# XuZhang1211/PVPUFormer

Hardware: AMD Instinct MI355X
Metric: 448x448 images/sec fwd+bwd, ViT-B VPUFormer (higher is better)
Workload: dtype bf16

## Files before the change

### include/vpu_hip.h

```cpp
#ifndef VPU_HIP_H
#define VPU_HIP_H
#include <stdint.h>

#ifdef __cplusplus
extern "C" {
#endif

#define VPU_BF16 0
#define VPU_F32 1

#define VPU_EPI_BIAS 1
#define VPU_EPI_PREACT 2
#define VPU_EPI_GELU 4
#define VPU_EPI_RELU 8
#define VPU_EPI_DGELU 16
#define VPU_EPI_DRELU 32
#define VPU_EPI_RESID 64
#define VPU_EPI_AFFINE 128
#define VPU_EPI_ACCUM 256
#define VPU_EPI_OUT_F32 512
#define VPU_EPI_SAVE_DGELU 1024
#define VPU_EPI_MULAUX 2048

typedef struct vpu_gemm_desc {
    const void* A;
    const void* B;
    void* C;
    const float* bias;
    const void* resid;
    const void* aux;
    void* preact;
    int32_t M, N, K;
    int32_t lda, ldb, ldc, ldr, ldaux;
    int32_t batch, inner;
    int64_t sAo, sAi, sBo, sBi, sCo, sCi, sRo, sRi;
    int32_t transA, transB;
    int32_t dtype, flags;
    int32_t resid_period;
    float alpha, post_mul, post_add;
    void* workspace;
    int64_t workspace_bytes;
    float* colsum;
    int32_t cs_tn, cs_t0;
    int64_t cs_ld;
} vpu_gemm_desc;

#define VPU_GEMM_GROUP_MAX 16
typedef struct vpu_gemm_group {
    int32_t n;
    int32_t start[VPU_GEMM_GROUP_MAX + 1];
    vpu_gemm_desc d[VPU_GEMM_GROUP_MAX];
} vpu_gemm_group;

const char* vpu_last_error(void);
int vpu_abi_version(void);

int vpu_gemm(const vpu_gemm_desc* d, void* stream);
int vpu_gemm_set_option(const char* name, int32_t value);
int vpu_gemm_get_option(const char* name, int32_t* value);
const char* vpu_gemm_last_kernel(void);
int vpu_gemm_grouped(const vpu_gemm_desc* d, int32_t n, void* stream);

int vpu_layernorm_fwd(const void* x, const float* w, const float* b, void* y, float* mean, float* rstd,
                      int64_t rows, int32_t C, float eps, int32_t dtype, void* stream);
int vpu_layernorm_bwd_nblk(int64_t rows);
int vpu_layernorm_bwd(const void* dy, const void* x, const float* w, const float* mean, const float* rstd,
                      const void* dres, void* dx, float* part, int64_t rows, int32_t C, int32_t dtype, void* stream);
int vpu_layernorm_fwd_pe(const void* x, const float* w, const float* b, void* y, float* mean, float* rstd,
                         int64_t rows, int32_t C, float eps, const void* pe, int64_t pe_rows, void* y2,
                         int32_t dtype, void* stream);
int vpu_layernorm_bwd2(const void* dy, const void* dy2, const void* x, const float* w, const float* mean,
                       const float* rstd, const void* dres, void* dx, float* part, int64_t rows, int32_t C,
                       int32_t dtype, void* stream);
#define VPU_COLSUM_BATCH_MAX 64
typedef struct vpu_colsum_job { const float* in; float* out; int32_t nrows, ncols, row_len, out_ld; } vpu_colsum_job;
typedef struct vpu_colsum_batch { vpu_colsum_job job[VPU_COLSUM_BATCH_MAX]; } vpu_colsum_batch;
int vpu_colsum_batched(const vpu_colsum_job* jobs, int32_t n, void* stream);
int vpu_colsum_f32(const float* in, float* out, int64_t rows, int32_t C, float beta, void* stream);
int vpu_colsum(const void* in, int32_t ld, float* out, float* part, int64_t rows, int32_t C, float beta,
               int32_t dtype, void* stream);
int vpu_softmax_fwd(const float* S, int32_t lds, void* P, int32_t ldp, int64_t rows, int32_t ncols,
                    int32_t dtype, void* stream);
int vpu_softmax_bwd(const void* P, int32_t ldp, const float* dP, int32_t lddp, void* dS, int64_t rows,
                    int32_t ncols, float scale, int32_t dtype, void* stream);
int vpu_l2norm_fwd(const void* x, void* y, float* inv, int64_t rows, int32_t C, int32_t dtype, void* stream);
int vpu_l2norm_bwd(const void* dy, const void* y, const float* inv, void* dx, int64_t rows, int32_t C,
                   int32_t dtype, void* stream);

int vpu_attn_fwd(const void* q, const void* k, const void* v, void* out, float* lse, int32_t nb, int32_t H, int32_t n,
                 int32_t hd, int32_t ld, int32_t ldo, float scale, void* stream);
int vpu_attn_bwd(const void* q, const void* k, const void* v, const void* o, const void* d_o, const float* lse,
                 float* delta, void* dq, void* dk, void* dv, int32_t nb, int32_t H, int32_t n, int32_t hd, int32_t ld,
                 int32_t ldo, int32_t ldg, float scale, void* stream);
int vpu_attn_set_option(const char* name, int32_t value);
const char* vpu_attn_last_kernel(void);
int vpu_xattn_fwd(const void* q, const void* k, const void* v, void* out, float* lse, int32_t nb, int32_t H, int32_t nq,
                  int32_t nk, int32_t hd, int32_t ldq, int32_t ldk, int32_t ldo, float scale, void* stream);
int vpu_xattn_bwd(const void* q, const void* k, const void* v, const void* o, const void* d_o, const float* lse,
                  float* delta, void* dq, void* dk, void* dv, int32_t nb, int32_t H, int32_t nq, int32_t nk, int32_t hd,
                  int32_t ldq, int32_t ldk, int32_t ldo, int32_t ldgq, int32_t ldgk, float scale, void* stream);
int vpu_xattn_fwd_split(const void* q, const void* k, const void* v, void* out, float* lse, int32_t nb, int32_t H, int32_t nq,
                        int32_t nk, int32_t hd, int32_t ldq, int32_t ldk, int32_t ldo, float scale, int32_t qdiv, int32_t kdiv,
                        void* stream);
int vpu_xattn_bwd_split(const void* q, const void* k, const void* v, const void* o, const void* d_o, const float* lse,
                        float* delta, void* dq, void* dk, void* dv, int32_t nb, int32_t H, int32_t nq, int32_t nk, int32_t hd,
                        int32_t ldq, int32_t ldk, int32_t ldo, int32_t ldgq, int32_t ldgk, float scale, int32_t qdiv, int32_t kdiv,
                        void* stream);
int vpu_attn_combine(const void* o_s, const float* lse_s, void* out, float* lse, int32_t nb, int32_t H, int32_t nq, int32_t hd,
                     int32_t S, int32_t ld_s, int32_t ldo, void* stream);
int vpu_sum_groups(const void* in, void* out, int64_t G, int32_t S, int64_t n, int32_t dtype, void* stream);

int vpu_add_bcast(const void* a, const void* b, void* out, int64_t n, int64_t period_b, int32_t dtype, void* stream);
int vpu_add4(const void* a, const void* b, const void* c, const void* d, void* out, int64_t n, int32_t dtype,
             void* stream);
int vpu_fanout_add(const void* src, void* const* dst, const int32_t* accum, int32_t ndst, int64_t n, int32_t dtype, void* stream);
int vpu_cast2d(const void* src, int32_t src_dtype, int64_t ld_src, void* dst, int32_t dst_dtype, int64_t ld_dst,
               int64_t rows, int32_t cols, int32_t cols_pad, void* stream);
typedef struct vpu_cast_job {
    const float* src;
    const float* src2;
    void* dst;
    int64_t ld_src, ld_dst, rows;
    int32_t cols, cols_pad, dst_dtype, perm_g, perm_wg;
} vpu_cast_job;
int vpu_cast2d_batched(const vpu_cast_job* jobs, int32_t n, void* stream);
int vpu_dropout_mask(float* out, int32_t n, float keep, uint64_t seed, uint64_t* state, void* stream);
int vpu_fill_f32(float* p, float v, int64_t n, void* stream);
int vpu_fill_ranges_f32(float* base, const int64_t* off, const int64_t* len, int32_t n, float v, void* stream);
int vpu_debug_spin(float* sink, int32_t wgs, int64_t cycles, void* stream);
int vpu_debug_gemm_times(void* dev_buf);
int vpu_sigmoid_to_channel(const float* logits, float* out, int32_t B, int64_t HW, int32_t channels, int32_t channel,
                           void* stream);
int vpu_act_bwd(const void* dy, int64_t ld_dy, const void* aux, int64_t ld_aux, void* dz, int64_t ld_dz, int64_t rows,
                int32_t cols, int32_t kind, int32_t dtype, void* stream);

int vpu_pue_encode(const float* points, const int32_t* boxes, const float* lut, void* out, double* out64,
                   int32_t B, int32_t n, int32_t num_max, int32_t img, int32_t ld, int32_t dtype, void* stream);
int vpu_pue_scribble_rows(const float* points, const double* vec, void* out, double* out64, int32_t B, int32_t n,
                          int32_t num_max, int32_t img, int32_t ld, int32_t dtype, void* stream);
int vpu_draw_polyline(const int32_t* curve, float* disks, int32_t B, int32_t P, int32_t H, int32_t W, void* stream);
int vpu_pue_encode_rows(const float* points, const int32_t* kinds, const int32_t* boxes, const double* vec, const float* lut,
                        void* out, double* out64, int32_t B, int32_t n, int32_t num_max, int32_t img, int32_t ld,
                        int32_t dtype, void* stream);
int vpu_draw_prompt_rows(const int32_t* kinds, const int32_t* boxes, const int32_t* curve, const int32_t* counts, float* disks,
                         int32_t B, int32_t Pmax, int32_t n, int32_t H, int32_t W, void* stream);
int vpu_edt(const uint8_t* mask, int32_t* scratch, float* dist, int32_t B, int32_t H, int32_t W, int32_t zero_border,
            void* stream);
int vpu_chamfer5(const uint8_t* mask, int32_t* scratch, float* dist, int32_t B, int32_t H, int32_t W, int32_t zero_border,
                 void* stream);
int vpu_mask_bbox(const float* prob, float thr, const int32_t* pos_clicks, int32_t nclicks, int32_t* out, int32_t B,
                  int32_t H, int32_t W, void* stream);
int vpu_error_masks(const uint8_t* pred, const uint8_t* gt, const uint8_t* valid, uint8_t* out, int32_t H, int32_t W,
                    void* stream);
int vpu_masked_argmax(const float* dist, const uint8_t* keep, uint64_t* out, int32_t planes, int32_t H, int32_t W,
                      void* stream);
typedef struct vpu_eval_obj {
    const float* image;
    const float* prev;
    float* canvas;
    uint8_t* mask;
    const uint8_t* gt;
    const uint8_t* valid;
    uint8_t* keep;
    int64_t* out;
    int32_t H, W, r0, r1, c0, c1, src, clear_at;
} vpu_eval_obj;
int vpu_roi_resize_batched(const vpu_eval_obj* objs, int32_t n, float* out, int32_t S_h, int32_t S_w, int32_t flip,
                           int32_t channels, void* stream);
int vpu_roi_paste_batched(const vpu_eval_obj* objs, int32_t n, const float* probs, int32_t S_h, int32_t S_w, float pred_thr,
                          float box_thr, int32_t max_hw, void* stream);
int vpu_click_keys_batched(const vpu_eval_obj* objs, int32_t n, uint8_t* err, int32_t* scratch, float* dist, int32_t Hm,
                           int32_t Wm, int32_t max_hw, void* stream);
typedef struct vpu_session_obj {
    float* canvas;
    uint64_t* bits;
    int32_t* rec;
    int32_t H, W, r0, r1, c0, c1, src, reserved;
} vpu_session_obj;
int vpu_session_paste_batched(const vpu_session_obj* objs, int32_t n, const float* probs, int32_t S_h, int32_t S_w,
                              float pred_thr, float box_thr, int32_t max_hw, int32_t form, void* stream);
typedef struct vpu_annot_obj {
    const float* add;
    float* total;
    uint16_t* labels;
    uint64_t* bits;
    int32_t* rec;
    int32_t H, W, label, mode;
} vpu_annot_obj;
int vpu_annot_compose_batched(const vpu_annot_obj* objs, int32_t n, float thr, int32_t max_hw, void* stream);
int vpu_label_extract(uint16_t* labels, float* out, int32_t* rec, int32_t H, int32_t W, int32_t label, void* stream);
typedef struct vpu_runs_obj {
    const void* src;
    int32_t H, W, kind;
    float thr;
} vpu_runs_obj;
#define VPU_RUNS_BAND_ROWS 64
#define VPU_RUNS_COLS 64
int vpu_runs_count_batched(const vpu_runs_obj* objs, const vpu_runs_obj* host_objs, int32_t n, int32_t* scratch,
                           int64_t scratch_len, int32_t* header, void* stream);
int vpu_runs_write_batched(const vpu_runs_obj* objs, const vpu_runs_obj* host_objs, int32_t n, const int32_t* scratch,
                           int64_t scratch_len, int32_t* entries, int32_t cap, void* stream);
typedef struct vpu_unrun_obj {
    void* dst;
    const int32_t* entries;
    int32_t H, W, n_runs, kind, label, pad;
} vpu_unrun_obj;
int vpu_runs_decode_batched(const vpu_unrun_obj* objs, const vpu_unrun_obj* host_objs, int32_t n, void* stream);
typedef struct vpu_box_row {
    const float* prev;
    const uint8_t* gt;
    const uint8_t* valid;
    int32_t H, W, r0, r1, c0, c1, mirror, n_obj;
} vpu_box_row;
int vpu_box_prompts_batched(const vpu_box_row* rows, int32_t n_rows, const float* points, int32_t n_batch, int32_t S_h,
                            int32_t S_w, float pred_thresh, uint8_t* masks, int32_t* counts, int32_t* roots, int32_t* slots,
                            int32_t* table, int32_t kmax, int32_t* boxes, int32_t* flag, void* stream);
#define VPU_CROPS_MAX_TILES_AXIS 64
int vpu_crops_gather(const float* in, float* out, const int32_t* y_offsets, const int32_t* x_offsets, int32_t ny, int32_t nx,
                     int32_t C, int32_t H, int32_t W, int32_t ch, int32_t cw, void* stream);
int vpu_crops_blend(const float* probs, float* out, const int32_t* y_offsets, const int32_t* x_offsets, int32_t ny, int32_t nx,
                    int32_t H, int32_t W, int32_t ch, int32_t cw, void* stream);
int vpu_cc_roots(const uint8_t* mask, int32_t* roots, int32_t B, int32_t H, int32_t W, void* stream);
int vpu_cc_table(const int32_t* roots, int32_t* slots, int32_t* table, int32_t kmax, int32_t B, int32_t H, int32_t W,
                 void* stream);

int vpu_disk_maps(const float* points, const int32_t* boxes, float* out, int32_t B, int32_t n, int32_t H, int32_t W,
                  float radius, void* stream);

int vpu_patch_im2col(const float* image4, const float* disks, void* cols, int32_t B, int32_t H, int32_t W, int32_t P,
                     int32_t win_tokens, int32_t dtype, void* stream);
int vpu_patch_im2col_prenorm(const float* image4, const float* disks, void* cols, int32_t B, int32_t H, int32_t W, int32_t P,
                             int32_t win_tokens, int32_t dtype, void* stream);
int vpu_patch_im2col_floor(const float* image4, const float* disks, void* cols, int32_t B, int32_t H, int32_t W, int32_t P,
                           int32_t wside, int32_t prenorm, int32_t dtype, void* stream);
int vpu_window_permute(const void* x, void* y, int32_t B, int32_t g, int32_t wg, int32_t C, int32_t dir, int32_t dtype,
                       void* stream);

int vpu_pixel_shuffle2(const void* in, void* out, const float* bias, int32_t B, int32_t h, int32_t w, int32_t C,
                       int32_t dir, int32_t dtype, void* stream);
int vpu_space_to_depth2_crop(const void* in, void* out, int32_t B, int32_t g, int32_t C, int32_t dir, int32_t dtype,
                             void* stream);
int vpu_pixel_shuffle2_gn_stats(const void* in, void* out, const float* bias, double* stats, int32_t B, int32_t h, int32_t w,
                                int32_t C, int32_t dtype, void* stream);
int vpu_groupnorm_apply(const void* x, const float* w, const float* b, void* y, float* mean, float* rstd, const double* stats,
                        int32_t B, int64_t HW, int32_t C, float eps, int32_t gelu, int32_t dtype, void* stream);
int vpu_pixel_unshuffle2_nblk(int32_t C);
int vpu_pixel_unshuffle2_sums(const void* in, void* out, float* part, int32_t B, int32_t h, int32_t w, int32_t C,
                              int32_t dtype, void* stream);
int vpu_groupnorm_nchunk(void);
int vpu_groupnorm_fwd(const void* x, const float* w, const float* b, void* y, float* mean, float* rstd, double* stats,
                      int32_t B, int64_t HW, int32_t C, float eps, int32_t gelu, int32_t dtype, void* stream);
int vpu_groupnorm_bwd(const void* dy, const void* x, const float* w, const float* b, const float* mean,
                      const float* rstd, void* dx, float* part, double* stats, int32_t B, int64_t HW, int32_t C,
                      int32_t gelu, int32_t dtype, void* stream);
int vpu_bilinear_cl_fwd(const void* in, int32_t ld_in, void* out, int32_t ld_out, int32_t B, int32_t h, int32_t w,
                        int32_t H, int32_t W, int32_t C, int32_t dtype, void* stream);
int vpu_bilinear_cl_bwd(const void* dout, int32_t ld_out, void* din, int32_t ld_in, int32_t B, int32_t h, int32_t w,
                        int32_t H, int32_t W, int32_t C, int32_t dtype, void* stream);
int vpu_upsum_relu(void* io, const void* const* z, const int32_t* h, const int32_t* w, int32_t n, int32_t B, int32_t H,
                   int32_t W, int32_t C, int32_t dtype, void* stream);
int vpu_head_grad_fused(const void* dfn, const void* y, const float* inv, const float* dout, const void* x, const float* w,
                        const float* mask, void* dx, float* part, float* part_b, int64_t rows, int64_t HW, int32_t C,
                        int32_t dtype, void* stream);
// ... 51 lines not shown
```

### pvpuformer_amd/_lib.py

```python
import ctypes as C
import os

_HERE = os.path.dirname(os.path.abspath(__file__))
LIB_PATH = os.path.join(_HERE, os.environ.get("VPU_LIB_FILE") or
                        ("libvpu_hip_diag.so" if os.environ.get("VPU_LIB_DIAG", "0") == "1" else "libvpu_hip.so"))

BF16, F32 = 0, 1

EPI_BIAS, EPI_PREACT, EPI_GELU, EPI_RELU, EPI_DGELU, EPI_DRELU = 1, 2, 4, 8, 16, 32
EPI_RESID, EPI_AFFINE, EPI_ACCUM, EPI_OUT_F32 = 64, 128, 256, 512
EPI_SAVE_DGELU, EPI_MULAUX = 1024, 2048


class GemmDesc(C.Structure):
    _fields_ = [
        ("A", C.c_void_p), ("B", C.c_void_p), ("C", C.c_void_p), ("bias", C.c_void_p), ("resid", C.c_void_p),
        ("aux", C.c_void_p), ("preact", C.c_void_p),
        ("M", C.c_int32), ("N", C.c_int32), ("K", C.c_int32),
        ("lda", C.c_int32), ("ldb", C.c_int32), ("ldc", C.c_int32), ("ldr", C.c_int32), ("ldaux", C.c_int32),
        ("batch", C.c_int32), ("inner", C.c_int32),
        ("sAo", C.c_int64), ("sAi", C.c_int64), ("sBo", C.c_int64), ("sBi", C.c_int64),
        ("sCo", C.c_int64), ("sCi", C.c_int64), ("sRo", C.c_int64), ("sRi", C.c_int64),
        ("transA", C.c_int32), ("transB", C.c_int32), ("dtype", C.c_int32), ("flags", C.c_int32),
        ("resid_period", C.c_int32),
        ("alpha", C.c_float), ("post_mul", C.c_float), ("post_add", C.c_float),
        ("workspace", C.c_void_p), ("workspace_bytes", C.c_int64), ("colsum", C.c_void_p),
        ("cs_tn", C.c_int32), ("cs_t0", C.c_int32), ("cs_ld", C.c_int64),
    ]


_P, _I, _L, _F = C.c_void_p, C.c_int32, C.c_int64, C.c_float

class ColsumJob(C.Structure):
    _fields_ = [("inp", C.c_void_p), ("out", C.c_void_p), ("nrows", C.c_int32), ("ncols", C.c_int32),
                ("row_len", C.c_int32), ("out_ld", C.c_int32)]


class CastJob(C.Structure):
    _fields_ = [("src", C.c_void_p), ("src2", C.c_void_p), ("dst", C.c_void_p), ("ld_src", C.c_int64), ("ld_dst", C.c_int64),
                ("rows", C.c_int64), ("cols", C.c_int32), ("cols_pad", C.c_int32), ("dst_dtype", C.c_int32),
                ("perm_g", C.c_int32), ("perm_wg", C.c_int32)]


class EvalObj(C.Structure):
    _fields_ = [("image", C.c_void_p), ("prev", C.c_void_p), ("canvas", C.c_void_p), ("mask", C.c_void_p),
                ("gt", C.c_void_p), ("valid", C.c_void_p), ("keep", C.c_void_p), ("out", C.c_void_p),
                ("H", C.c_int32), ("W", C.c_int32), ("r0", C.c_int32), ("r1", C.c_int32), ("c0", C.c_int32),
                ("c1", C.c_int32), ("src", C.c_int32), ("clear_at", C.c_int32)]


class BoxRow(C.Structure):
    _fields_ = [("prev", C.c_void_p), ("gt", C.c_void_p), ("valid", C.c_void_p),
                ("H", C.c_int32), ("W", C.c_int32), ("r0", C.c_int32), ("r1", C.c_int32), ("c0", C.c_int32),
                ("c1", C.c_int32), ("mirror", C.c_int32), ("n_obj", C.c_int32)]


class SessionObj(C.Structure):
    _fields_ = [("canvas", C.c_void_p), ("bits", C.c_void_p), ("rec", C.c_void_p),
                ("H", C.c_int32), ("W", C.c_int32), ("r0", C.c_int32), ("r1", C.c_int32), ("c0", C.c_int32),
                ("c1", C.c_int32), ("src", C.c_int32), ("reserved", C.c_int32)]


class AnnotObj(C.Structure):
    _fields_ = [("add", C.c_void_p), ("total", C.c_void_p), ("labels", C.c_void_p), ("bits", C.c_void_p), ("rec", C.c_void_p),
                ("H", C.c_int32), ("W", C.c_int32), ("label", C.c_int32), ("mode", C.c_int32)]


class RunsObj(C.Structure):
    _fields_ = [("src", C.c_void_p), ("H", C.c_int32), ("W", C.c_int32), ("kind", C.c_int32), ("thr", C.c_float)]


class UnrunObj(C.Structure):
    _fields_ = [("dst", C.c_void_p), ("entries", C.c_void_p), ("H", C.c_int32), ("W", C.c_int32), ("n_runs", C.c_int32),
                ("kind", C.c_int32), ("label", C.c_int32), ("pad", C.c_int32)]


SIGNATURES = {
    "vpu_gemm": [C.POINTER(GemmDesc), _P],
    "vpu_layernorm_fwd": [_P, _P, _P, _P, _P, _P, _L, _I, _F, _I, _P],
    "vpu_layernorm_bwd_nblk": [_L],
    "vpu_layernorm_bwd": [_P, _P, _P, _P, _P, _P, _P, _P, _L, _I, _I, _P],
    "vpu_layernorm_fwd_pe": [_P, _P, _P, _P, _P, _P, _L, _I, _F, _P, _L, _P, _I, _P],
    "vpu_layernorm_bwd2": [_P, _P, _P, _P, _P, _P, _P, _P, _P, _L, _I, _I, _P],
    "vpu_colsum_batched": [C.POINTER(ColsumJob), _I, _P],
    "vpu_colsum_f32": [_P, _P, _L, _I, _F, _P],
    "vpu_colsum": [_P, _I, _P, _P, _L, _I, _F, _I, _P],
    "vpu_softmax_fwd": [_P, _I, _P, _I, _L, _I, _I, _P],
    "vpu_softmax_bwd": [_P, _I, _P, _I, _P, _L, _I, _F, _I, _P],
    "vpu_l2norm_fwd": [_P, _P, _P, _L, _I, _I, _P],
    "vpu_l2norm_bwd": [_P, _P, _P, _P, _L, _I, _I, _P],
    "vpu_attn_fwd": [_P, _P, _P, _P, _P, _I, _I, _I, _I, _I, _I, _F, _P],
    "vpu_attn_bwd": [_P, _P, _P, _P, _P, _P, _P, _P, _P, _P, _I, _I, _I, _I, _I, _I, _I, _F, _P],
    "vpu_xattn_fwd": [_P, _P, _P, _P, _P, _I, _I, _I, _I, _I, _I, _I, _I, _F, _P],
    "vpu_xattn_bwd": [_P, _P, _P, _P, _P, _P, _P, _P, _P, _P, _I, _I, _I, _I, _I, _I, _I, _I, _I, _I, _F, _P],
    "vpu_xattn_fwd_split": [_P, _P, _P, _P, _P, _I, _I, _I, _I, _I, _I, _I, _I, _F, _I, _I, _P],
    "vpu_xattn_bwd_split": [_P, _P, _P, _P, _P, _P, _P, _P, _P, _P, _I, _I, _I, _I, _I, _I, _I, _I, _I, _I, _F, _I, _I, _P],
    "vpu_attn_combine": [_P, _P, _P, _P, _I, _I, _I, _I, _I, _I, _I, _P],
    "vpu_sum_groups": [_P, _P, _L, _I, _L, _I, _P],
    "vpu_add_bcast": [_P, _P, _P, _L, _L, _I, _P],
    "vpu_add4": [_P, _P, _P, _P, _P, _L, _I, _P],
    "vpu_cast2d": [_P, _I, _L, _P, _I, _L, _L, _I, _I, _P],
    "vpu_cast2d_batched": [C.POINTER(CastJob), _I, _P],
    "vpu_fanout_add": [_P, C.POINTER(C.c_void_p), C.POINTER(C.c_int32), _I, _L, _I, _P],
    "vpu_dropout_mask": [_P, _I, _F, C.c_uint64, _P, _P],
    "vpu_fill_f32": [_P, _F, _L, _P],
    "vpu_fill_ranges_f32": [_P, C.POINTER(C.c_int64), C.POINTER(C.c_int64), _I, _F, _P],
    "vpu_debug_spin": [_P, _I, _L, _P],
    "vpu_debug_gemm_times": [_P],
    "vpu_sigmoid_to_channel": [_P, _P, _I, _L, _I, _I, _P],
    "vpu_act_bwd": [_P, _L, _P, _L, _P, _L, _L, _I, _I, _I, _P],
    "vpu_pue_encode": [_P, _P, _P, _P, _P, _I, _I, _I, _I, _I, _I, _P],
    "vpu_cc_roots": [_P, _P, _I, _I, _I, _P],
    "vpu_cc_table": [_P, _P, _P, _I, _I, _I, _I, _P],
    "vpu_edt": [_P, _P, _P, _I, _I, _I, _I, _P],
    "vpu_chamfer5": [_P, _P, _P, _I, _I, _I, _I, _P],
    "vpu_pue_scribble_rows": [_P, _P, _P, _P, _I, _I, _I, _I, _I, _I, _P],
    "vpu_draw_polyline": [_P, _P, _I, _I, _I, _I, _P],
    "vpu_pue_encode_rows": [_P, _P, _P, _P, _P, _P, _P, _I, _I, _I, _I, _I, _I, _P],
    "vpu_draw_prompt_rows": [_P, _P, _P, _P, _P, _I, _I, _I, _I, _I, _P],
    "vpu_mask_bbox": [_P, _F, _P, _I, _P, _I, _I, _I, _P],
    "vpu_masked_argmax": [_P, _P, _P, _I, _I, _I, _P],
    "vpu_error_masks": [_P, _P, _P, _P, _I, _I, _P],
    "vpu_roi_resize_batched": [_P, _I, _P, _I, _I, _I, _I, _P],
    "vpu_roi_paste_batched": [_P, _I, _P, _I, _I, _F, _F, _I, _P],
    "vpu_session_paste_batched": [_P, _I, _P, _I, _I, _F, _F, _I, _I, _P],
    "vpu_annot_compose_batched": [_P, _I, _F, _I, _P],
    "vpu_label_extract": [_P, _P, _P, _I, _I, _I, _P],
    "vpu_runs_count_batched": [_P, _P, _I, _P, _L, _P, _P],
    "vpu_runs_write_batched": [_P, _P, _I, _P, _L, _P, _I, _P],
    "vpu_runs_decode_batched": [_P, _P, _I, _P],
    "vpu_click_keys_batched": [_P, _I, _P, _P, _P, _I, _I, _I, _P],
    "vpu_box_prompts_batched": [_P, _I, _P, _I, _I, _I, _F, _P, _P, _P, _P, _P, _I, _P, _P, _P],
    "vpu_crops_gather": [_P, _P, _P, _P, _I, _I, _I, _I, _I, _I, _I, _P],
    "vpu_crops_blend": [_P, _P, _P, _P, _I, _I, _I, _I, _I, _I, _P],
    "vpu_disk_maps": [_P, _P, _P, _I, _I, _I, _I, _F, _P],
    "vpu_patch_im2col": [_P, _P, _P, _I, _I, _I, _I, _I, _I, _P],
    "vpu_patch_im2col_prenorm": [_P, _P, _P, _I, _I, _I, _I, _I, _I, _P],
    "vpu_patch_im2col_floor": [_P, _P, _P, _I, _I, _I, _I, _I, _I, _I, _P],
    "vpu_window_permute": [_P, _P, _I, _I, _I, _I, _I, _I, _P],
    "vpu_space_to_depth2_crop": [_P, _P, _I, _I, _I, _I, _I, _P],
    "vpu_pixel_shuffle2": [_P, _P, _P, _I, _I, _I, _I, _I, _I, _P],
    "vpu_pixel_shuffle2_gn_stats": [_P, _P, _P, _P, _I, _I, _I, _I, _I, _P],
    "vpu_groupnorm_apply": [_P, _P, _P, _P, _P, _P, _P, _I, _L, _I, _F, _I, _I, _P],
    "vpu_pixel_unshuffle2_nblk": [_I],
    "vpu_pixel_unshuffle2_sums": [_P, _P, _P, _I, _I, _I, _I, _I, _P],
    "vpu_groupnorm_nchunk": [],
    "vpu_groupnorm_fwd": [_P, _P, _P, _P, _P, _P, _P, _I, _L, _I, _F, _I, _I, _P],
    "vpu_groupnorm_bwd": [_P, _P, _P, _P, _P, _P, _P, _P, _P, _I, _L, _I, _I, _I, _P],
    "vpu_bilinear_cl_fwd": [_P, _I, _P, _I, _I, _I, _I, _I, _I, _I, _I, _P],
    "vpu_bilinear_cl_bwd": [_P, _I, _P, _I, _I, _I, _I, _I, _I, _I, _I, _P],
    "vpu_head_grad_fused": [_P, _P, _P, _P, _P, _P, _P, _P, _P, _P, _L, _L, _I, _I, _P],
    "vpu_upsum_relu": [_P, C.POINTER(C.c_void_p), C.POINTER(C.c_int32), C.POINTER(C.c_int32), _I, _I, _I, _I, _I, _I, _P],
    "vpu_gate_stats": [_P, _P, _P, _P, _P, _P, _I, _I, _I, _I, _I, _P],
    "vpu_gate_apply": [_P, _P, _P, _P, _I, _I, _I, _I, _P],
    "vpu_gate_bwd": [_P, _P, _P, _P, _P, _P, _P, _I, _P, _P, _P, _I, _I, _I, _I, _I, _P],
    "vpu_gate_fwd_n": [C.POINTER(C.c_void_p), C.POINTER(C.c_void_p), _P, C.POINTER(C.c_void_p), _P, _P, _P, _P, _I, _I, _I, _I, _I, _I, _P],
    "vpu_gate_bwd_n": [C.POINTER(C.c_void_p), _P, _P, _P, _P, _P, _P, _I, C.POINTER(C.c_void_p), C.POINTER(C.c_void_p), _P, _I, _I, _I,
                       _I, _I, _I, _P],
    "vpu_convseg_fwd": [_P, _P, _P, _P, _P, _L, _L, _I, _I, _P],
    "vpu_convseg_bwd_nblk": [_L],
    "vpu_convseg_bwd": [_P, _P, _P, _P, _P, _I, _P, _P, _L, _L, _I, _I, _P],
    "vpu_upsample_ac_fwd": [_P, _P, _L, _I, _I, _I, _I, _P],
    "vpu_upsample_ac_bwd": [_P, _P, _L, _I, _I, _I, _I, _P],
    "vpu_p2cl_fwd_bwd": [_P, _P, _P, _P, _P, _P, _F, _I, _I, _I, _I, _P],
    "vpu_p2cl_up_nband": [_I, _I],
    "vpu_p2cl_up_fwd_bwd": [_P, _P, _P, _P, _P, _P, _F, _I, _I, _I, _I, _I, _I, _P],
    "vpu_nfl_dice_scratch_doubles": [_I],
    "vpu_nfl_dice_fwd_bwd": [_P, _P, _P, _P, _P, _F, _F, _I, _L, _P],
    "vpu_loss_finalize": [_P, _P, _I, _I, C.c_double, _F, _F, _F, _F, _P, _P],
    "vpu_adam_step": [_P, _P, _P, _P, _P, _L, _F, _F, _F, _F, _F, _I, _F, _P],
    "vpu_adam_step_groups": [_P, _P, _P, _P, _P, _L, _P, _P, _P, _I, _F, _F, _F, _I, _I, _F, _P],
    "vpu_adam_step_hyper": [_P, _P, _P, _P, _P, _L, _P, _P, _P, _P, _I, _F, _F, _F, _F, _I, _P],
    "vpu_gemm_set_option": [C.c_char_p, _I],
    "vpu_gemm_get_option": [C.c_char_p, C.POINTER(C.c_int32)],
    "vpu_gemm_last_kernel": [],
    "vpu_attn_last_kernel": [],
    "vpu_attn_set_option": [C.c_char_p, _I],
    "vpu_gemm_grouped": [C.POINTER(GemmDesc), _I, _P],
    "vpu_last_error": [],
    "vpu_abi_version": [],
}
_RET = {"vpu_last_error": C.c_char_p, "vpu_gemm_last_kernel": C.c_char_p, "vpu_attn_last_kernel": C.c_char_p}

_lib = None


class VpuError(RuntimeError):
    pass


def load():
    global _lib
    if _lib is not None:
        return _lib
    if not os.path.exists(LIB_PATH):
        raise VpuError(f"{LIB_PATH} not found: build it with pvpuformer_amd/csrc/build.sh "
                       f"(or `python -c 'import __graft_entry__ as g; g.build()'`). There is no CPU fallback.")
    import torch
    lib = C.CDLL(LIB_PATH)
    for name, argtypes in SIGNATURES.items():
        fn = getattr(lib, name)
        fn.argtypes = argtypes
        fn.restype = _RET.get(name, C.c_int)
    _lib = lib
    return lib


def call(name, *args):
    lib = load()
    rc = getattr(lib, name)(*args)
    if rc != 0:
        raise VpuError(f"{name} failed ({rc}): {lib.vpu_last_error().decode()}")
    return rc
```

### pvpuformer_amd/csrc/attention.hip

```cpp
#include <stdio.h>
#include <stdlib.h>
#include <string.h>
#include <atomic>
#include "vpu_common.h"
#include "../../include/vpu_hip.h"

namespace {

typedef __attribute__((address_space(3))) s16x4_t* lds_s16x4_ptr;
constexpr int CH = 32;

template <int HD> __device__ __forceinline__ int rc_off(int row, int chunk) {
    return row * (HD * 2) + ((chunk ^ ((row >> 1) & (HD / 8 - 1))) << 4);
}
template <int HD> __device__ __forceinline__ int tr_off(int row, int unit) {
    return row * (HD * 2) + ((unit ^ ((((row >> 1) & 3) << 2) & (HD / 4 - 1))) << 3);
}

template <int HD, int NS> struct RowChunk { uint4 v[(NS * CH * HD / 8 + 255) / 256]; };
template <int HD, int NS>
__device__ __forceinline__ void fetch_rows(const bf16_t* __restrict__ base, int ld, int r0, int n, int tid, int hd,
                                           RowChunk<HD, NS>& rc) {
    constexpr int CPR = HD / 8;
#pragma unroll
    for (int i = 0; i < (NS * CH * CPR + 255) / 256; ++i) {
        const int c = tid + i * 256;
        const int row = c / CPR, ch = c % CPR;
        uint4 v = make_uint4(0, 0, 0, 0);
        if (c < NS * CH * CPR && r0 + row < n && ch * 8 < hd)
            v = *reinterpret_cast<const uint4*>(base + (int64_t)(r0 + row) * ld + ch * 8);
        rc.v[i] = v;
    }
}
template <int HD, int NS, bool TR>
__device__ __forceinline__ void put_rows(char* lds, int tid, const RowChunk<HD, NS>& rc) {
    constexpr int CPR = HD / 8;
#pragma unroll
    for (int i = 0; i < (NS * CH * CPR + 255) / 256; ++i) {
        const int c = tid + i * 256;
        if (c < NS * CH * CPR) {
            const int row = c / CPR, ch = c % CPR;
            const int off = TR ? tr_off<HD>(row, ch * 2) : rc_off<HD>(row, ch);
            *reinterpret_cast<uint4*>(lds + off) = rc.v[i];
        }
    }
}

template <int HD> __device__ __forceinline__ bf16x8_t frag_rc(const char* lds, int row16, int ks, int lane) {
    const uint4 v = *reinterpret_cast<const uint4*>(lds + rc_off<HD>(row16 + (lane & 15), ks * 4 + (lane >> 4)));
    return __builtin_bit_cast(bf16x8_t, v);
}
template <int HD> __device__ __forceinline__ bf16x8_t frag_tr_perm(const char* lds, int dt, int lane) {
    const int g = lane >> 4, q = (lane & 15) >> 2, p = lane & 3;
    const int unit = dt * 4 + p;
    const s16x4_t lo = __builtin_amdgcn_ds_read_tr16_b64_v4i16((lds_s16x4_ptr)(lds + tr_off<HD>(4 * g + q, unit)));
    const s16x4_t hi = __builtin_amdgcn_ds_read_tr16_b64_v4i16((lds_s16x4_ptr)(lds + tr_off<HD>(16 + 4 * g + q, unit)));
    s16x8_t v;
    v[0] = lo[0]; v[1] = lo[1]; v[2] = lo[2]; v[3] = lo[3];
    v[4] = hi[0]; v[5] = hi[1]; v[6] = hi[2]; v[7] = hi[3];
    return __builtin_bit_cast(bf16x8_t, v);
}
template <int HD>
__device__ __forceinline__ void load_rows_as_b(const bf16_t* __restrict__ base, int ld, int row0, int n, int lane,
                                               bf16x8_t (&f)[HD / 32], int hd) {
    const int row = row0 + (lane & 15);
#pragma unroll
    for (int ks = 0; ks < HD / 32; ++ks) {
        uint4 v = make_uint4(0, 0, 0, 0);
        const int col = ks * 32 + (lane >> 4) * 8;
        if (row < n && col < hd) v = *reinterpret_cast<const uint4*>(base + (int64_t)row * ld + col);
        f[ks] = __builtin_bit_cast(bf16x8_t, v);
    }
}
template <int NK>
__device__ __forceinline__ void load_rows_as_bn(const bf16_t* __restrict__ base, int ld, int row0, int n, int lane,
                                                bf16x8_t (&f)[NK], int hd) {
    const int row = row0 + (lane & 15);
#pragma unroll
    for (int ks = 0; ks < NK; ++ks) {
        uint4 v = make_uint4(0, 0, 0, 0);
        const int col = ks * 32 + (lane >> 4) * 8;
        if (row < n && col < hd) v = *reinterpret_cast<const uint4*>(base + (int64_t)row * ld + col);
        f[ks] = __builtin_bit_cast(bf16x8_t, v);
    }
}
__device__ __forceinline__ bf16x8_t pack_pair(const f32x4_t& a, const f32x4_t& b) {
    bf16x8_t f;
#pragma unroll
    for (int j = 0; j < 4; ++j) { f[j] = (bf16_t)a[j]; f[4 + j] = (bf16_t)b[j]; }
    return f;
}

struct AttnArgs {
    const bf16_t *q, *k, *v;
    const bf16_t *o, *d_o;
    bf16_t *out, *dq, *dk, *dv;
    float *lse, *delta;
    int nq, nk, H, hd;
    int ldq, ldk, ldo;
    int ldgq, ldgk;
    float scale;
    int gx, nbh;
    int qdiv, kdiv;
};

template <int HD, int NS, int QT>
__global__ __launch_bounds__(256) void attn_fwd_kernel(const AttnArgs a) {
    __shared__ __attribute__((aligned(16))) char ldsK[NS * CH * HD * 2];
    __shared__ __attribute__((aligned(16))) char ldsV[NS * CH * HD * 2];
    const int tid = threadIdx.x, lane = tid & 63, wave = tid >> 6, g = lane >> 4, c = lane & 15;
    const int bh = blockIdx.y, bw = bh / a.H, h = bh % a.H, nq = a.nq, nk = a.nk, hd = a.hd;
    const int64_t rbq = (int64_t)bw * nq, rbk = (int64_t)bw * nk;
    const bf16_t* q = a.q + rbq * a.ldq + h * hd;
    const bf16_t* k = a.k + rbk * a.ldk + h * hd;
    const bf16_t* v = a.v + rbk * a.ldk + h * hd;
    const int q0 = blockIdx.x * (64 * QT) + wave * (16 * QT);
    const float sc2 = a.scale * 1.44269504089f;
    bf16x8_t qf[QT][HD / 32];
    float m[QT], l[QT];
    f32x4_t acc[QT][HD / 16];
#pragma unroll
    for (int u = 0; u < QT; ++u) {
        load_rows_as_b<HD>(q, a.ldq, q0 + 16 * u, nq, lane, qf[u], hd);
        m[u] = -INFINITY; l[u] = 0.f;
#pragma unroll
        for (int dt = 0; dt < HD / 16; ++dt) acc[u][dt] = (f32x4_t){0.f, 0.f, 0.f, 0.f};
    }
    RowChunk<HD, NS> pk, pv;
    fetch_rows<HD, NS>(k, a.ldk, 0, nk, tid, hd, pk);
    fetch_rows<HD, NS>(v, a.ldk, 0, nk, tid, hd, pv);
    for (int kb = 0; kb < nk; kb += NS * CH) {
        __syncthreads();
        put_rows<HD, NS, false>(ldsK, tid, pk);
        put_rows<HD, NS, true>(ldsV, tid, pv);
        __syncthreads();
        if (kb + NS * CH < nk) {
            fetch_rows<HD, NS>(k, a.ldk, kb + NS * CH, nk, tid, hd, pk);
            fetch_rows<HD, NS>(v, a.ldk, kb + NS * CH, nk, tid, hd, pv);
        }
        for (int sub = 0; sub < NS && kb + sub * CH < nk; ++sub) {
        const int kc = kb + sub * CH;
        const char* sK = ldsK + sub * (CH * HD * 2);
        const char* sV = ldsV + sub * (CH * HD * 2);
        f32x4_t s[QT][2];
#pragma unroll
        for (int u = 0; u < QT; ++u)
#pragma unroll
            for (int t = 0; t < 2; ++t) s[u][t] = (f32x4_t){0.f, 0.f, 0.f, 0.f};
#pragma unroll
        for (int t = 0; t < 2; ++t)
#pragma unroll
            for (int ks = 0; ks < HD / 32; ++ks) {
                const bf16x8_t kfr = frag_rc<HD>(sK, 16 * t, ks, lane);
#pragma unroll
                for (int u = 0; u < QT; ++u)
                    s[u][t] = __builtin_amdgcn_mfma_f32_16x16x32_bf16(kfr, qf[u][ks], s[u][t], 0, 0, 0);
            }
        bf16x8_t pf[QT];
        float ar[QT][4];
        const bool tail = kc + CH > nk;
#pragma unroll
        for (int u = 0; u < QT; ++u) {
            float mx = m[u];
#pragma unroll
            for (int t = 0; t < 2; ++t)
#pragma unroll
                for (int r = 0; r < 4; ++r) {
                    float x = s[u][t][r] * sc2;
                    if (tail) x = (kc + 16 * t + 4 * g + r < nk) ? x : -INFINITY;
                    s[u][t][r] = x;
                    mx = fmaxf(mx, x);
                }
            mx = fmaxf(mx, __shfl_xor(mx, 16, 64));
            mx = fmaxf(mx, __shfl_xor(mx, 32, 64));
            const float alpha = __builtin_amdgcn_exp2f(m[u] - mx);
            float ps = 0.f;
#pragma unroll
            for (int t = 0; t < 2; ++t)
#pragma unroll
                for (int r = 0; r < 4; ++r) { s[u][t][r] = __builtin_amdgcn_exp2f(s[u][t][r] - mx); ps += s[u][t][r]; }
            ps += __shfl_xor(ps, 16, 64);
            ps += __shfl_xor(ps, 32, 64);
            l[u] = l[u] * alpha + ps;
            m[u] = mx;
#pragma unroll
            for (int r = 0; r < 4; ++r) ar[u][r] = __shfl(alpha, 4 * g + r, 64);
            pf[u] = pack_pair(s[u][0], s[u][1]);
        }
#pragma unroll
        for (int dt = 0; dt < HD / 16; ++dt) {
            const bf16x8_t vfr = frag_tr_perm<HD>(sV, dt, lane);
#pragma unroll
            for (int u = 0; u < QT; ++u) {
#pragma unroll
                for (int r = 0; r < 4; ++r) acc[u][dt][r] *= ar[u][r];
                acc[u][dt] = __builtin_amdgcn_mfma_f32_16x16x32_bf16(pf[u], vfr, acc[u][dt], 0, 0, 0);
            }
        }
        }
    }
#pragma unroll
    for (int u = 0; u < QT; ++u) {
        const int qu = q0 + 16 * u;
        const float il = 1.0f / l[u];
        if (g == 0 && qu + c < nq) a.lse[(int64_t)bh * nq + qu + c] = (m[u] + __builtin_amdgcn_logf(l[u])) * 0.69314718056f;
#pragma unroll
        for (int r = 0; r < 4; ++r) {
            const float s1 = __shfl(il, 4 * g + r, 64);
            const int qq = qu + 4 * g + r;
            if (qq < nq) {
                bf16_t* orow = a.out + (rbq + qq) * a.ldo + h * hd;
#pragma unroll
                for (int dt = 0; dt < HD / 16; ++dt)
                    if (dt * 16 < hd) orow[dt * 16 + c] = (bf16_t)(acc[u][dt][r] * s1);
            }
        }
    }
}

template <int HD, int NS>
__global__ __launch_bounds__(256) void attn_bwd_dkdv_kernel(const AttnArgs a) {
    __shared__ __attribute__((aligned(16))) char ldsQr[NS * CH * HD * 2], ldsQt[NS * CH * HD * 2];
    __shared__ __attribute__((aligned(16))) char ldsOr[NS * CH * HD * 2], ldsOt[NS * CH * HD * 2];
    const int tid = threadIdx.x, lane = tid & 63, wave = tid >> 6, g = lane >> 4, c = lane & 15;
    const int bh = blockIdx.y, bw = bh / a.H, h = bh % a.H, nq = a.nq, nk = a.nk, hd = a.hd;
    const int64_t rbq = (int64_t)bw * nq, rbk = (int64_t)bw * nk;
    const bf16_t* q = a.q + rbq * a.ldq + h * hd;
    const bf16_t* k = a.k + rbk * a.ldk + h * hd;
    const bf16_t* v = a.v + rbk * a.ldk + h * hd;
    const bf16_t* d_o = a.d_o + rbq * a.ldo + h * hd;
    const float* lse = a.lse + (int64_t)bh * nq;
    const float* dl = a.delta + (int64_t)bh * nq;
    const int key0 = blockIdx.x * 64 + wave * 16;
    const bool key_ok = key0 + c < nk;
    bf16x8_t kf[HD / 32], vf[HD / 32];
    load_rows_as_b<HD>(k, a.ldk, key0, nk, lane, kf, hd);
    load_rows_as_b<HD>(v, a.ldk, key0, nk, lane, vf, hd);
    f32x4_t adk[HD / 16], adv[HD / 16];
#pragma unroll
    for (int dt = 0; dt < HD / 16; ++dt) { adk[dt] = (f32x4_t){0.f, 0.f, 0.f, 0.f}; adv[dt] = adk[dt]; }
    RowChunk<HD, NS> pq, po;
    fetch_rows<HD, NS>(q, a.ldq, 0, nq, tid, hd, pq);
    fetch_rows<HD, NS>(d_o, a.ldo, 0, nq, tid, hd, po);
    for (int qb = 0; qb < nq; qb += NS * CH) {
        __syncthreads();
        put_rows<HD, NS, false>(ldsQr, tid, pq);
        put_rows<HD, NS, true>(ldsQt, tid, pq);
        put_rows<HD, NS, false>(ldsOr, tid, po);
        put_rows<HD, NS, true>(ldsOt, tid, po);
        __syncthreads();
        if (qb + NS * CH < nq) {
            fetch_rows<HD, NS>(q, a.ldq, qb + NS * CH, nq, tid, hd, pq);
            fetch_rows<HD, NS>(d_o, a.ldo, qb + NS * CH, nq, tid, hd, po);
        }
        for (int sub = 0; sub < NS && qb + sub * CH < nq; ++sub) {
        const int qc = qb + sub * CH;
// ... 54 lines not shown
                    vr[dt * 16 + c] = (bf16_t)adv[dt][r];
                }
        }
    }
}

template <int HD, int NS>
__global__ __launch_bounds__(256) void attn_bwd_dq_kernel(const AttnArgs a) {
    __shared__ __attribute__((aligned(16))) char ldsKr[NS * CH * HD * 2], ldsKt[NS * CH * HD * 2], ldsVr[NS * CH * HD * 2];
    const int tid = threadIdx.x, lane = tid & 63, wave = tid >> 6, g = lane >> 4, c = lane & 15;
    const int bh = blockIdx.y, bw = bh / a.H, h = bh % a.H, nq = a.nq, nk = a.nk, hd = a.hd;
    const int64_t rbq = (int64_t)bw * nq, rbk = (int64_t)bw * nk;
    const bf16_t* q = a.q + rbq * a.ldq + h * hd;
    const bf16_t* k = a.k + rbk * a.ldk + h * hd;
    const bf16_t* v = a.v + rbk * a.ldk + h * hd;
    const bf16_t* d_o = a.d_o + rbq * a.ldo + h * hd;
    const int q0 = blockIdx.x * 64 + wave * 16;
    const bool q_ok = q0 + c < nq;
    const float lse_q = q_ok ? a.lse[(int64_t)bh * nq + q0 + c] : 0.f;
    bf16x8_t qf[HD / 32], dof[HD / 32];
    load_rows_as_b<HD>(q, a.ldq, q0, nq, lane, qf, hd);
    load_rows_as_b<HD>(d_o, a.ldo, q0, nq, lane, dof, hd);
    float dl_q = 0.f;
    {
        bf16x8_t of[HD / 32];
        load_rows_as_b<HD>(a.o + rbq * a.ldo + h * hd, a.ldo, q0, nq, lane, of, hd);
#pragma unroll
        for (int ks = 0; ks < HD / 32; ++ks)
#pragma unroll
            for (int j = 0; j < 8; ++j) dl_q += (float)dof[ks][j] * (float)of[ks][j];
        dl_q += __shfl_xor(dl_q, 16, 64);
        dl_q += __shfl_xor(dl_q, 32, 64);
        if (blockIdx.x * 64 + wave * 16 + c < nq && g == 0) a.delta[(int64_t)bh * nq + q0 + c] = dl_q;
    }
    f32x4_t adq[HD / 16];
#pragma unroll
    for (int dt = 0; dt < HD / 16; ++dt) adq[dt] = (f32x4_t){0.f, 0.f, 0.f, 0.f};
    RowChunk<HD, NS> pk, pv;
    fetch_rows<HD, NS>(k, a.ldk, 0, nk, tid, hd, pk);
    fetch_rows<HD, NS>(v, a.ldk, 0, nk, tid, hd, pv);
    for (int kb = 0; kb < nk; kb += NS * CH) {
        __syncthreads();
        put_rows<HD, NS, false>(ldsKr, tid, pk);
        put_rows<HD, NS, true>(ldsKt, tid, pk);
        put_rows<HD, NS, false>(ldsVr, tid, pv);
        __syncthreads();
        if (kb + NS * CH < nk) {
            fetch_rows<HD, NS>(k, a.ldk, kb + NS * CH, nk, tid, hd, pk);
            fetch_rows<HD, NS>(v, a.ldk, kb + NS * CH, nk, tid, hd, pv);
        }
        for (int sub = 0; sub < NS && kb + sub * CH < nk; ++sub) {
        const int kc = kb + sub * CH;
        const int so = sub * (CH * HD * 2);
        f32x4_t dS[2];
#pragma unroll
        for (int t = 0; t < 2; ++t) {
            f32x4_t s = (f32x4_t){0.f, 0.f, 0.f, 0.f}, dp = s;
#pragma unroll
            for (int ks = 0; ks < HD / 32; ++ks) {
                s = __builtin_amdgcn_mfma_f32_16x16x32_bf16(frag_rc<HD>(ldsKr + so, 16 * t, ks, lane), qf[ks], s, 0, 0, 0);
                dp = __builtin_amdgcn_mfma_f32_16x16x32_bf16(frag_rc<HD>(ldsVr + so, 16 * t, ks, lane), dof[ks], dp, 0, 0, 0);
            }
#pragma unroll
            for (int r = 0; r < 4; ++r) {
                float ds = 0.f;
                if (q_ok && kc + 16 * t + 4 * g + r < nk)
                    ds = __expf(s[r] * a.scale - lse_q) * (dp[r] - dl_q) * a.scale;
                dS[t][r] = ds;
            }
        }
        const bf16x8_t dsf = pack_pair(dS[0], dS[1]);
#pragma unroll
        for (int dt = 0; dt < HD / 16; ++dt)
            adq[dt] = __builtin_amdgcn_mfma_f32_16x16x32_bf16(dsf, frag_tr_perm<HD>(ldsKt + so, dt, lane), adq[dt], 0, 0, 0);
        }
    }
#pragma unroll
    for (int r = 0; r < 4; ++r) {
        const int qq = q0 + 4 * g + r;
        if (qq < nq) {
            bf16_t* qr = a.dq + (rbq + qq) * a.ldgq + h * hd;
#pragma unroll
            for (int dt = 0; dt < HD / 16; ++dt)
                if (dt * 16 < hd) qr[dt * 16 + c] = (bf16_t)adq[dt][r];
        }
    }
}

constexpr float LOG2E = 1.44269504089f, LN2 = 0.69314718056f;
typedef unsigned u32x4v __attribute__((ext_vector_type(4)));

__device__ __forceinline__ __amdgpu_buffer_rsrc_t rows_rsrc(const void* base, int n, int ld, int cols, int elem) {
    return __builtin_amdgcn_make_buffer_rsrc(const_cast<void*>(base), 0, ((n - 1) * ld + cols) * elem, 0x00020000);
}

template <int HD> struct Stg {
    static constexpr int CPR = HD / 8, NCH = CH * CPR, NI = (NCH + 255) / 256;
    int lrc[NI], ltr[NI];
    bool live[NI];
    __device__ __forceinline__ void init(int tid) {
#pragma unroll
        for (int i = 0; i < NI; ++i) {
            const int c = tid + i * 256, row = c / CPR, ch = c % CPR;
            live[i] = c < NCH;
            lrc[i] = rc_off<HD>(row, ch);
            ltr[i] = tr_off<HD>(row, ch * 2);
        }
    }
    __device__ __forceinline__ void offsets(int tid, int ld, int hd, int (&voff)[NI]) const {
#pragma unroll
        for (int i = 0; i < NI; ++i) {
            const int c = tid + i * 256, row = c / CPR, ch = c % CPR;
            voff[i] = (live[i] && ch * 8 < hd) ? (row * ld + ch * 8) * 2 : 0x40000000;
        }
    }
    __device__ __forceinline__ static void fetch(const __amdgpu_buffer_rsrc_t rs, const int (&voff)[NI], int base, u32x4v (&v)[NI]) {
#pragma unroll
        for (int i = 0; i < NI; ++i) v[i] = __builtin_amdgcn_raw_buffer_load_b128(rs, voff[i] + base, 0, 0);
    }
    __device__ __forceinline__ void put_rc(char* lds, const u32x4v (&v)[NI]) const {
#pragma unroll
        for (int i = 0; i < NI; ++i)
            if (live[i]) *reinterpret_cast<u32x4v*>(lds + lrc[i]) = v[i];
    }
    __device__ __forceinline__ void put_tr(char* lds, const u32x4v (&v)[NI]) const {
#pragma unroll
        for (int i = 0; i < NI; ++i)
            if (live[i]) *reinterpret_cast<u32x4v*>(lds + ltr[i]) = v[i];
    }
};

__device__ __forceinline__ float max8(const f32x4_t& a, const f32x4_t& b) {
    float d, t0, t1;
    asm volatile("s_nop 15\n\ts_nop 3\n\t"
                 "v_max3_f32 %0, %3, %4, %5\n\t"
                 "v_max3_f32 %1, %6, %7, %8\n\t"
                 "v_max3_f32 %2, %9, %10, %10\n\t"
                 "v_max3_f32 %0, %0, %1, %2"
                 : "=&v"(d), "=&v"(t0), "=&v"(t1)
                 : "v"(a[0]), "v"(a[1]), "v"(a[2]), "v"(a[3]), "v"(b[0]), "v"(b[1]), "v"(b[2]), "v"(b[3]));
    return d;
}

__device__ __forceinline__ void wg_problem(int gx, int nbh, int& bh, int& xb) {
    if (gx == 0) { bh = blockIdx.y; xb = blockIdx.x; return; }
    const int id = blockIdx.x, per = 8 * gx, grp = id / per, r = id - grp * per;
    const int cnt = min(8, nbh - grp * 8);
    bh = grp * 8 + r % cnt;
    xb = r / cnt;
}

constexpr float RESCALE_TH = 8.0f;

template <int HD, int QT, int HC>
#ifndef VPU_ATTN_FWD_OCC
#define VPU_ATTN_FWD_OCC 4
#endif
__global__ __launch_bounds__(256, (HD == 64 && QT == 2) ? VPU_ATTN_FWD_OCC : 1) void attn_fwd_lean_kernel(const AttnArgs a) {
    constexpr int KS = HC / 32, DT = HC / 16;
    using S = Stg<HD>;
    __shared__ __attribute__((aligned(16))) char ldsK[2][CH * HD * 2];
    __shared__ __attribute__((aligned(16))) char ldsV[2][CH * HD * 2];
    const int tid = threadIdx.x, lane = tid & 63, wave = tid >> 6, g = lane >> 4, c = lane & 15;
    int bh, xb;
    wg_problem(a.gx, a.nbh, bh, xb);
    const int bw = bh / a.H, h = bh % a.H, nq = a.nq, nk = a.nk, hd = a.hd;
    const int bwq = bw / max(a.qdiv, 1), bwk = bw / max(a.kdiv, 1);
    const int64_t rbq = (int64_t)bwq * nq, rbk = (int64_t)bwk * nk, rbqo = (int64_t)bw * nq, rbko = (int64_t)bw * nk;
    const int bhq = bwq * a.H + h;
    const bf16_t* q = a.q + rbq * a.ldq + h * hd;
    const bf16_t* k = a.k + rbk * a.ldk + h * hd;
    const bf16_t* v = a.v + rbk * a.ldk + h * hd;
    const int q0 = xb * (64 * QT) + wave * (16 * QT);
    const float sc2 = a.scale * LOG2E;
    bf16x8_t qf[QT][KS];
    float mref[QT];
    f32x4_t acc[QT][DT], accl[QT];
#pragma unroll
    for (int u = 0; u < QT; ++u) {
        load_rows_as_bn<KS>(q, a.ldq, q0 + 16 * u, nq, lane, qf[u], hd);
        mref[u] = -INFINITY;
        accl[u] = (f32x4_t){0.f, 0.f, 0.f, 0.f};
#pragma unroll
        for (int dt = 0; dt < DT; ++dt) acc[u][dt] = (f32x4_t){0.f, 0.f, 0.f, 0.f};
    }
    bf16x8_t ones;
#pragma unroll
    for (int j = 0; j < 8; ++j) ones[j] = (bf16_t)1.0f;
    S st;
    st.init(tid);
    int voff[S::NI];
    st.offsets(tid, a.ldk, hd, voff);
    const __amdgpu_buffer_rsrc_t rsK = rows_rsrc(k, nk, a.ldk, hd, 2), rsV = rows_rsrc(v, nk, a.ldk, hd, 2);
    const int nch = (nk + CH - 1) / CH, cstep = CH * a.ldk * 2;
    u32x4v pk[S::NI], pv[S::NI];
    S::fetch(rsK, voff, 0, pk);
    S::fetch(rsV, voff, 0, pv);
    st.put_rc(ldsK[0], pk);
    st.put_tr(ldsV[0], pv);
    if (nch > 1) { S::fetch(rsK, voff, cstep, pk); S::fetch(rsV, voff, cstep, pv); }
    f32x4_t s[QT][2];
    float lm[QT];
    auto stage = [&](int i) {
        __syncthreads();
        if (i + 1 < nch) { st.put_rc(ldsK[(i + 1) & 1], pk); st.put_tr(ldsV[(i + 1) & 1], pv); }
        if (i + 2 < nch) { S::fetch(rsK, voff, (i + 2) * cstep, pk); S::fetch(rsV, voff, (i + 2) * cstep, pv); }
    };
    auto scores = [&](int i) {
        const char* sK = ldsK[i & 1];
        const int kc = i * CH;
#pragma unroll
        for (int u = 0; u < QT; ++u)
#pragma unroll
            for (int t = 0; t < 2; ++t) s[u][t] = (f32x4_t){0.f, 0.f, 0.f, 0.f};
#pragma unroll
        for (int t = 0; t < 2; ++t)
#pragma unroll
            for (int ks = 0; ks < KS; ++ks) {
                const bf16x8_t kfr = frag_rc<HD>(sK, 16 * t, ks, lane);
#pragma unroll
                for (int u = 0; u < QT; ++u)
                    s[u][t] = __builtin_amdgcn_mfma_f32_16x16x32_bf16(kfr, qf[u][ks], s[u][t], 0, 0, 0);
            }
        if (kc + CH > nk) {
#pragma unroll
            for (int t = 0; t < 2; ++t)
#pragma unroll
                for (int r = 0; r < 4; ++r)
                    if (kc + 16 * t + 4 * g + r >= nk) {
#pragma unroll
                        for (int u = 0; u < QT; ++u) s[u][t][r] = -INFINITY;
                    }
        }
#pragma unroll
        for (int u = 0; u < QT; ++u) lm[u] = max8(s[u][0], s[u][1]) * sc2;
    };
    auto outgrown = [&]() {
        bool need = false;
#pragma unroll
        for (int u = 0; u < QT; ++u) need = need || (lm[u] > mref[u] + RESCALE_TH);
        return __builtin_amdgcn_ballot_w64(need) != 0;
    };
    auto raise = [&]() {
#pragma unroll
        for (int u = 0; u < QT; ++u) {
            float xm = lm[u];
            xm = fmaxf(xm, __shfl_xor(xm, 16, 64));
            xm = fmaxf(xm, __shfl_xor(xm, 32, 64));
            const float mnew = (xm > mref[u] + RESCALE_TH) ? xm : mref[u];
            const float alpha = __builtin_amdgcn_exp2f(mref[u] - mnew);
            mref[u] = mnew;
#pragma unroll
            for (int r = 0; r < 4; ++r) {
                accl[u][r] *= alpha;
#pragma unroll
                for (int dt = 0; dt < DT; ++dt) acc[u][dt][r] *= alpha;
            }
        }
    };
    auto probs_pv = [&](int i) {
        const char* sV = ldsV[i & 1];
        bf16x8_t pf[QT];
#pragma unroll
        for (int u = 0; u < QT; ++u) {
            const float nm = -mref[u];
#pragma unroll
            for (int t = 0; t < 2; ++t)
#pragma unroll
                for (int r = 0; r < 4; ++r) s[u][t][r] = __builtin_amdgcn_exp2f(__builtin_fmaf(s[u][t][r], sc2, nm));
            pf[u] = pack_pair(s[u][0], s[u][1]);
            accl[u] = __builtin_amdgcn_mfma_f32_16x16x32_bf16(ones, pf[u], accl[u], 0, 0, 0);
        }
#pragma unroll
        for (int dt = 0; dt < DT; ++dt) {
            const bf16x8_t vfr = frag_tr_perm<HD>(sV, dt, lane);
#pragma unroll
            for (int u = 0; u < QT; ++u) acc[u][dt] = __builtin_amdgcn_mfma_f32_16x16x32_bf16(vfr, pf[u], acc[u][dt], 0, 0, 0);
        }
    };
    stage(0); scores(0); raise();
    int i = 0;
    bool go;
    do {
        probs_pv(i);
        ++i;
        go = i < nch;
        if (go) { stage(i); scores(i); go = !outgrown(); }
    } while (go);
    while (i < nch) {
        raise(); probs_pv(i);
        ++i;
        if (i < nch) { stage(i); scores(i); }
    }
    __syncthreads();
    {
        typedef __bf16 bf16x4o_t __attribute__((ext_vector_type(4)));
        constexpr int RB = HD * 2, NCHK = HD / 8, SW = NCHK >= 8 ? 7 : NCHK - 1;
        char* const stg = (wave < 2 ? &ldsK[0][0] : &ldsV[0][0]) + (wave & 1) * (CH * HD * 2);
#pragma unroll
        for (int u = 0; u < QT; ++u) {
            const float l = accl[u][0], il = __builtin_amdgcn_rcpf(l);
            const int qq = q0 + 16 * u + c;
            if (g == 0 && qq < nq) a.lse[(int64_t)bh * nq + qq] = (mref[u] + __builtin_amdgcn_logf(l)) * LN2;
            const int row = 16 * u + c;
#pragma unroll
            for (int dt = 0; dt < DT; ++dt) {
                bf16x4o_t w4;
#pragma unroll
                for (int r = 0; r < 4; ++r) w4[r] = (bf16_t)(acc[u][dt][r] * il);
                const int chk = (2 * dt + (g >> 1)) ^ (row & SW);
                *reinterpret_cast<bf16x4o_t*>(stg + row * RB + chk * 16 + (g & 1) * 8) = w4;
            }
        }
#pragma unroll
        for (int i = 0; i < 16 * QT * NCHK / 64; ++i) {
            const int idx = i * 64 + lane, row = idx / NCHK, ch = idx % NCHK;
            const u32x4v v16 = *reinterpret_cast<const u32x4v*>(stg + row * RB + ((ch ^ (row & SW)) * 16));
            const int qq = q0 + row;
            if (qq < nq && ch * 8 < hd) *reinterpret_cast<u32x4v*>(a.out + (rbqo + qq) * a.ldo + h * hd + ch * 8) = v16;
        }
    }
}

template <int HD, int QT, int HC>
__global__ __launch_bounds__(256) void attn_bwd_dq_lean_kernel(const AttnArgs a) {
    constexpr int KS = HC / 32, DT = HC / 16;
    using S = Stg<HD>;
    __shared__ __attribute__((aligned(16))) char ldsKr[2][CH * HD * 2], ldsKt[2][CH * HD * 2], ldsVr[2][CH * HD * 2];
    const int tid = threadIdx.x, lane = tid & 63, wave = tid >> 6, g = lane >> 4, c = lane & 15;
    int bh, xb;
    wg_problem(a.gx, a.nbh, bh, xb);
    const int bw = bh / a.H, h = bh % a.H, nq = a.nq, nk = a.nk, hd = a.hd;
    const int bwq = bw / max(a.qdiv, 1), bwk = bw / max(a.kdiv, 1);
    const int64_t rbq = (int64_t)bwq * nq, rbk = (int64_t)bwk * nk, rbqo = (int64_t)bw * nq, rbko = (int64_t)bw * nk;
    const int bhq = bwq * a.H + h;
    const bf16_t* q = a.q + rbq * a.ldq + h * hd;
    const bf16_t* k = a.k + rbk * a.ldk + h * hd;
    const bf16_t* v = a.v + rbk * a.ldk + h * hd;
    const bf16_t* d_o = a.d_o + rbq * a.ldo + h * hd;
    const int q0 = xb * (64 * QT) + wave * (16 * QT);
    const float sc2 = a.scale * LOG2E;
    bf16x8_t qf[QT][KS], dof[QT][KS];
    float nl2[QT], nds[QT];
    f32x4_t adq[QT][DT];
#pragma unroll
    for (int u = 0; u < QT; ++u) {
        const int qu = q0 + 16 * u;
        const bool q_ok = qu + c < nq;
        nl2[u] = q_ok ? -a.lse[(int64_t)bhq * nq + qu + c] * LOG2E : 0.f;
        load_rows_as_bn<KS>(q, a.ldq, qu, nq, lane, qf[u], hd);
        load_rows_as_bn<KS>(d_o, a.ldo, qu, nq, lane, dof[u], hd);
        bf16x8_t of[KS];
        load_rows_as_bn<KS>(a.o + rbq * a.ldo + h * hd, a.ldo, qu, nq, lane, of, hd);
        float dl = 0.f;
#pragma unroll
        for (int ks = 0; ks < KS; ++ks)
#pragma unroll
            for (int j = 0; j < 8; ++j) dl += (float)dof[u][ks][j] * (float)of[ks][j];
        dl += __shfl_xor(dl, 16, 64);
        dl += __shfl_xor(dl, 32, 64);
        if (q_ok && g == 0) a.delta[(int64_t)bhq * nq + qu + c] = dl;
        nds[u] = -dl * a.scale;
#pragma unroll
        for (int dt = 0; dt < DT; ++dt) adq[u][dt] = (f32x4_t){0.f, 0.f, 0.f, 0.f};
    }
    S st;
    st.init(tid);
    int voff[S::NI];
    st.offsets(tid, a.ldk, hd, voff);
    const __amdgpu_buffer_rsrc_t rsK = rows_rsrc(k, nk, a.ldk, hd, 2), rsV = rows_rsrc(v, nk, a.ldk, hd, 2);
    const int nch = (nk + CH - 1) / CH, cstep = CH * a.ldk * 2;
    u32x4v pk[S::NI], pv[S::NI];
    S::fetch(rsK, voff, 0, pk);
    S::fetch(rsV, voff, 0, pv);
    st.put_rc(ldsKr[0], pk); st.put_tr(ldsKt[0], pk); st.put_rc(ldsVr[0], pv);
    if (nch > 1) { S::fetch(rsK, voff, cstep, pk); S::fetch(rsV, voff, cstep, pv); }
    for (int i = 0; i < nch; ++i) {
        __syncthreads();
        if (i + 1 < nch) {
            const int nb = (i + 1) & 1;
            st.put_rc(ldsKr[nb], pk); st.put_tr(ldsKt[nb], pk); st.put_rc(ldsVr[nb], pv);
        }
        if (i + 2 < nch) { S::fetch(rsK, voff, (i + 2) * cstep, pk); S::fetch(rsV, voff, (i + 2) * cstep, pv); }
        const char* sKr = ldsKr[i & 1];
        const char* sKt = ldsKt[i & 1];
        const char* sVr = ldsVr[i & 1];
        const int kc = i * CH;
        f32x4_t dS[QT][2];
#pragma unroll
        for (int t = 0; t < 2; ++t) {
            f32x4_t s[QT], dp[QT];
#pragma unroll
            for (int u = 0; u < QT; ++u) { s[u] = (f32x4_t){0.f, 0.f, 0.f, 0.f}; dp[u] = s[u]; }
#pragma unroll
            for (int ks = 0; ks < KS; ++ks) {
                const bf16x8_t kfr = frag_rc<HD>(sKr, 16 * t, ks, lane), vfr = frag_rc<HD>(sVr, 16 * t, ks, lane);
#pragma unroll
                for (int u = 0; u < QT; ++u) {
                    s[u] = __builtin_amdgcn_mfma_f32_16x16x32_bf16(kfr, qf[u][ks], s[u], 0, 0, 0);
                    dp[u] = __builtin_amdgcn_mfma_f32_16x16x32_bf16(vfr, dof[u][ks], dp[u], 0, 0, 0);
                }
            }
#pragma unroll
            for (int u = 0; u < QT; ++u)
#pragma unroll
                for (int r = 0; r < 4; ++r)
                    dS[u][t][r] = __builtin_amdgcn_exp2f(__builtin_fmaf(s[u][r], sc2, nl2[u])) * __builtin_fmaf(dp[u][r], a.scale, nds[u]);
        }
        if (kc + CH > nk) {
#pragma unroll
            for (int t = 0; t < 2; ++t)
#pragma unroll
                for (int r = 0; r < 4; ++r)
                    if (kc + 16 * t + 4 * g + r >= nk) {
#pragma unroll
                        for (int u = 0; u < QT; ++u) dS[u][t][r] = 0.f;
                    }
        }
        bf16x8_t dsf[QT];
#pragma unroll
        for (int u = 0; u < QT; ++u) dsf[u] = pack_pair(dS[u][0], dS[u][1]);
#pragma unroll
        for (int dt = 0; dt < DT; ++dt) {
            const bf16x8_t ktf = frag_tr_perm<HD>(sKt, dt, lane);
#pragma unroll
            for (int u = 0; u < QT; ++u) adq[u][dt] = __builtin_amdgcn_mfma_f32_16x16x32_bf16(dsf[u], ktf, adq[u][dt], 0, 0, 0);
        }
    }
#pragma unroll
    for (int u = 0; u < QT; ++u)
#pragma unroll
        for (int r = 0; r < 4; ++r) {
            const int qq = q0 + 16 * u + 4 * g + r;
            if (qq < nq) {
                bf16_t* qr = a.dq + (rbqo + qq) * a.ldgq + h * hd + c;
                if (hd == HC) {
#pragma unroll
                    for (int dt = 0; dt < DT; ++dt) qr[dt * 16] = (bf16_t)adq[u][dt][r];
                } else {
#pragma unroll
                    for (int dt = 0; dt < DT; ++dt)
                        if (dt * 16 < hd) qr[dt * 16] = (bf16_t)adq[u][dt][r];
                }
            }
        }
}

template <int HD, int KT, int HC>
__global__ __launch_bounds__(256, 3) void attn_bwd_dkdv_lean_kernel(const AttnArgs a) {
    constexpr int KS = HC / 32, DT = HC / 16;
    using S = Stg<HD>;
    __shared__ __attribute__((aligned(16))) char ldsQr[2][CH * HD * 2], ldsQt[2][CH * HD * 2];
    __shared__ __attribute__((aligned(16))) char ldsOr[2][CH * HD * 2], ldsOt[2][CH * HD * 2];
    const int tid = threadIdx.x, lane = tid & 63, wave = tid >> 6, g = lane >> 4, c = lane & 15;
    int bh, xb;
    wg_problem(a.gx, a.nbh, bh, xb);
    const int bw = bh / a.H, h = bh % a.H, nq = a.nq, nk = a.nk, hd = a.hd;
    const int bwq = bw / max(a.qdiv, 1), bwk = bw / max(a.kdiv, 1);
    const int64_t rbq = (int64_t)bwq * nq, rbk = (int64_t)bwk * nk, rbqo = (int64_t)bw * nq, rbko = (int64_t)bw * nk;
    const int bhq = bwq * a.H + h;
    const bf16_t* q = a.q + rbq * a.ldq + h * hd;
    const bf16_t* k = a.k + rbk * a.ldk + h * hd;
    const bf16_t* v = a.v + rbk * a.ldk + h * hd;
    const bf16_t* d_o = a.d_o + rbq * a.ldo + h * hd;
    const int key0 = xb * (64 * KT) + wave * (16 * KT);
    const float sc2 = a.scale * LOG2E;
    bf16x8_t kf[KT][KS], vf[KT][KS];
    f32x4_t adk[KT][DT], adv[KT][DT];
#pragma unroll
    for (int u = 0; u < KT; ++u) {
        load_rows_as_bn<KS>(k, a.ldk, key0 + 16 * u, nk, lane, kf[u], hd);
        load_rows_as_bn<KS>(v, a.ldk, key0 + 16 * u, nk, lane, vf[u], hd);
#pragma unroll
        for (int dt = 0; dt < DT; ++dt) { adk[u][dt] = (f32x4_t){0.f, 0.f, 0.f, 0.f}; adv[u][dt] = adk[u][dt]; }
    }
    S st;
    st.init(tid);
    int voq[S::NI], voo[S::NI];
    st.offsets(tid, a.ldq, hd, voq);
    st.offsets(tid, a.ldo, hd, voo);
    const __amdgpu_buffer_rsrc_t rsQ = rows_rsrc(q, nq, a.ldq, hd, 2), rsO = rows_rsrc(d_o, nq, a.ldo, hd, 2);
    const __amdgpu_buffer_rsrc_t rsL = rows_rsrc(reinterpret_cast<const char*>(a.lse + (int64_t)bhq * nq), 1, 0, nq, 4);
    const __amdgpu_buffer_rsrc_t rsD = rows_rsrc(reinterpret_cast<const char*>(a.delta + (int64_t)bhq * nq), 1, 0, nq, 4);
    const int nch = (nq + CH - 1) / CH, qstep = CH * a.ldq * 2, ostep = CH * a.ldo * 2;
    u32x4v pq[S::NI], po[S::NI];
    S::fetch(rsQ, voq, 0, pq);
    S::fetch(rsO, voo, 0, po);
    st.put_rc(ldsQr[0], pq); st.put_tr(ldsQt[0], pq); st.put_rc(ldsOr[0], po); st.put_tr(ldsOt[0], po);
    if (nch > 1) { S::fetch(rsQ, voq, qstep, pq); S::fetch(rsO, voo, ostep, po); }
    for (int i = 0; i < nch; ++i) {
        __syncthreads();
        if (i + 1 < nch) {
            const int nb = (i + 1) & 1;
            st.put_rc(ldsQr[nb], pq); st.put_tr(ldsQt[nb], pq); st.put_rc(ldsOr[nb], po); st.put_tr(ldsOt[nb], po);
        }
        if (i + 2 < nch) { S::fetch(rsQ, voq, (i + 2) * qstep, pq); S::fetch(rsO, voo, (i + 2) * ostep, po); }
        const int b = i & 1, qc = i * CH;
        f32x4_t nl2[2], nds[2];
#pragma unroll
        for (int t = 0; t < 2; ++t) {
            const int off = (qc + 16 * t + 4 * g) * 4;
            const f32x4_t lv = __builtin_bit_cast(f32x4_t, __builtin_amdgcn_raw_buffer_load_b128(rsL, off, 0, 0));
            const f32x4_t dv = __builtin_bit_cast(f32x4_t, __builtin_amdgcn_raw_buffer_load_b128(rsD, off, 0, 0));
            nl2[t] = lv * (-LOG2E);
            nds[t] = dv * (-a.scale);
        }
        f32x4_t P[KT][2], dS[KT][2];
#pragma unroll
        for (int t = 0; t < 2; ++t) {
            f32x4_t s[KT], dp[KT];
#pragma unroll
            for (int u = 0; u < KT; ++u) { s[u] = (f32x4_t){0.f, 0.f, 0.f, 0.f}; dp[u] = s[u]; }
#pragma unroll
            for (int ks = 0; ks < KS; ++ks) {
                const bf16x8_t qfr = frag_rc<HD>(ldsQr[b], 16 * t, ks, lane), ofr = frag_rc<HD>(ldsOr[b], 16 * t, ks, lane);
#pragma unroll
                for (int u = 0; u < KT; ++u) {
                    s[u] = __builtin_amdgcn_mfma_f32_16x16x32_bf16(qfr, kf[u][ks], s[u], 0, 0, 0);
                    dp[u] = __builtin_amdgcn_mfma_f32_16x16x32_bf16(ofr, vf[u][ks], dp[u], 0, 0, 0);
                }
            }
#pragma unroll
            for (int u = 0; u < KT; ++u)
#pragma unroll
                for (int r = 0; r < 4; ++r) {
                    const float p = __builtin_amdgcn_exp2f(__builtin_fmaf(s[u][r], sc2, nl2[t][r]));
                    P[u][t][r] = p;
                    dS[u][t][r] = p * __builtin_fmaf(dp[u][r], a.scale, nds[t][r]);
                }
        }
        bf16x8_t pf[KT], dsf[KT];
#pragma unroll
        for (int u = 0; u < KT; ++u) { pf[u] = pack_pair(P[u][0], P[u][1]); dsf[u] = pack_pair(dS[u][0], dS[u][1]); }
#pragma unroll
        for (int dt = 0; dt < DT; ++dt) {
            const bf16x8_t otf = frag_tr_perm<HD>(ldsOt[b], dt, lane), qtf = frag_tr_perm<HD>(ldsQt[b], dt, lane);
#pragma unroll
            for (int u = 0; u < KT; ++u) {
                adv[u][dt] = __builtin_amdgcn_mfma_f32_16x16x32_bf16(pf[u], otf, adv[u][dt], 0, 0, 0);
                adk[u][dt] = __builtin_amdgcn_mfma_f32_16x16x32_bf16(dsf[u], qtf, adk[u][dt], 0, 0, 0);
            }
        }
    }
#pragma unroll
    for (int u = 0; u < KT; ++u)
#pragma unroll
        for (int r = 0; r < 4; ++r) {
            const int kk = key0 + 16 * u + 4 * g + r;
            if (kk < nk) {
                bf16_t* kr = a.dk + (rbko + kk) * a.ldgk + h * hd + c;
                bf16_t* vr = a.dv + (rbko + kk) * a.ldgk + h * hd + c;
                if (hd == HC) {
#pragma unroll
                    for (int dt = 0; dt < DT; ++dt) {
                        kr[dt * 16] = (bf16_t)adk[u][dt][r];
                        vr[dt * 16] = (bf16_t)adv[u][dt][r];
                    }
                } else {
#pragma unroll
                    for (int dt = 0; dt < DT; ++dt)
                        if (dt * 16 < hd) {
                            kr[dt * 16] = (bf16_t)adk[u][dt][r];
                            vr[dt * 16] = (bf16_t)adv[u][dt][r];
                        }
                }
            }
        }
}

constexpr int WIN_MAX_KB = 8;
constexpr int WIN_ROWS = WIN_MAX_KB * 32;
constexpr int win_lds(int nkb) { return 3 * (32 * nkb * 64 * 2) + 2 * ((32 * nkb + 16) * 64) + 2 * (32 * nkb) * 4; }

__device__ __forceinline__ int ds_swz(int row) { return (((row >> 2) & 1) << 2) | (((row >> 3) & 1) << 1) | ((row >> 1) & 1); }
__device__ __forceinline__ bf16x8_t frag_ds(const char* lds, int t, int lane) {
    const int g = lane >> 4, q = (lane & 15) >> 2, p = lane & 3;
    const int r0 = 4 * g + q, u = ((t * 4 + p) ^ ds_swz(r0)) << 3;
    const s16x4_t lo = __builtin_amdgcn_ds_read_tr16_b64_v4i16((lds_s16x4_ptr)(lds + r0 * 64 + u));
    const s16x4_t hi = __builtin_amdgcn_ds_read_tr16_b64_v4i16((lds_s16x4_ptr)(lds + (16 + r0) * 64 + u));
    s16x8_t v;
    v[0] = lo[0]; v[1] = lo[1]; v[2] = lo[2]; v[3] = lo[3];
    v[4] = hi[0]; v[5] = hi[1]; v[6] = hi[2]; v[7] = hi[3];
    return __builtin_bit_cast(bf16x8_t, v);
}
template <int HD> __device__ __forceinline__ bf16x8_t frag_rc_tr(const char* lds, int row16, int ks, int lane) {
    const uint4 v = *reinterpret_cast<const uint4*>(lds + tr_off<HD>(row16 + (lane & 15), 2 * (ks * 4 + (lane >> 4))));
    return __builtin_bit_cast(bf16x8_t, v);
}
__device__ __forceinline__ bf16x8_t frag_rc_trv(const char* lds, int row16, int ks, int lane) {
    const u32x4v v = *reinterpret_cast<const u32x4v*>(lds + tr_off<64>(row16 + (lane & 15), 2 * (ks * 4 + (lane >> 4))));
    return __builtin_bit_cast(bf16x8_t, v);
}
typedef __attribute__((address_space(3))) void* lds_vptr3;
typedef __bf16 bf16x4w_t __attribute__((ext_vector_type(4)));
typedef unsigned u32x2w __attribute__((ext_vector_type(2)));
__device__ __forceinline__ bf16x4w_t pack4(const f32x4_t& a) {
    bf16x4w_t w;
#pragma unroll
    for (int r = 0; r < 4; ++r) w[r] = (bf16_t)a[r];
    return w;
}

template <int NKB>
__global__ __launch_bounds__(512) void attn_bwd_win_kernel(const AttnArgs a) {
    constexpr int HD = 64, KS = 2, DT = 4, ROWS = 32 * NKB, NP = (NKB + 1) / 2;
    constexpr int LDS_M = ROWS * HD * 2, LDS_S1 = (ROWS + 16) * 64;
    extern __shared__ __attribute__((aligned(16))) char wlds[];
    char* const ldsQ = wlds;
    char* const ldsO = wlds + LDS_M;
    char* const ldsK = wlds + 2 * LDS_M;
    char* const ldsS = wlds + 3 * LDS_M;
    float* const ldsD = reinterpret_cast<float*>(ldsS + 2 * LDS_S1);
    float* const ldsL = ldsD + ROWS;
    const int tid = threadIdx.x, lane = tid & 63, wave = tid >> 6, g = lane >> 4, c = lane & 15;
    const int bh = blockIdx.x, bw = bh / a.H, h = bh % a.H, n = a.nq;
    const int64_t rb = (int64_t)bw * n;
    const bf16_t* q = a.q + rb * a.ldq + h * HD;
    const bf16_t* k = a.k + rb * a.ldk + h * HD;
    const bf16_t* v = a.v + rb * a.ldk + h * HD;
    const bf16_t* o = a.o + rb * a.ldo + h * HD;
    const bf16_t* d_o = a.d_o + rb * a.ldo + h * HD;
    const float sc2 = a.scale * LOG2E;
    const int NT = (n + 15) >> 4;
    const int base = NT >> 3, rem = NT & 7;
    const int nu = base + (wave < rem ? 1 : 0), tile0 = wave * base + (wave < rem ? wave : rem);
    const int my_t = wave >> 2, my_dt = wave & 3;
#ifdef VPU_WIN_STAMPS
    const unsigned t_start = (unsigned)__builtin_amdgcn_s_memtime();
#endif
    bf16x8_t kf[2][KS], vf[2][KS];
#pragma unroll
    for (int u = 0; u < 2; ++u) {
        const int key0 = (u < nu) ? (tile0 + u) * 16 : n;
        load_rows_as_bn<KS>(k, a.ldk, key0, n, lane, kf[u], HD);
        load_rows_as_bn<KS>(v, a.ldk, key0, n, lane, vf[u], HD);
    }
    {
        const __amdgpu_buffer_rsrc_t rsQ = rows_rsrc(q, n, a.ldq, HD, 2), rsK = rows_rsrc(k, n, a.ldk, HD, 2);
        const __amdgpu_buffer_rsrc_t rsG = rows_rsrc(d_o, n, a.ldo, HD, 2), rsO = rows_rsrc(o, n, a.ldo, HD, 2);
        const __amdgpu_buffer_rsrc_t rsL = rows_rsrc(reinterpret_cast<const char*>(a.lse + (int64_t)bh * n), 1, 0, n, 4);
        u32x4v pq[NP], pk[NP], pg[NP], po[NP];
        const int ch = tid & 7, row0 = tid >> 3;
#pragma unroll
        for (int i = 0; i < NP; ++i) {
            const int row = row0 + 64 * i;
            const bool live = row < ROWS;
            pq[i] = __builtin_amdgcn_raw_buffer_load_b128(rsQ, live ? (row * a.ldq + ch * 8) * 2 : 0x40000000, 0, 0);
            pk[i] = __builtin_amdgcn_raw_buffer_load_b128(rsK, live ? (row * a.ldk + ch * 8) * 2 : 0x40000000, 0, 0);
            pg[i] = __builtin_amdgcn_raw_buffer_load_b128(rsG, live ? (row * a.ldo + ch * 8) * 2 : 0x40000000, 0, 0);
            po[i] = __builtin_amdgcn_raw_buffer_load_b128(rsO, live ? (row * a.ldo + ch * 8) * 2 : 0x40000000, 0, 0);
        }
        const float pl = __builtin_bit_cast(float, __builtin_amdgcn_raw_buffer_load_b32(rsL, tid < ROWS ? tid * 4 : 0x40000000, 0, 0));
        if ((NT & 1) && tid < 128)
            *reinterpret_cast<u32x4v*>(ldsS + (tid >> 6) * LDS_S1 + NT * 16 * 64 + (tid & 63) * 16) = (u32x4v){0u, 0u, 0u, 0u};
        if (tid < ROWS) ldsL[tid] = -pl * LOG2E;
#pragma unroll
        for (int i = 0; i < NP; ++i) {
            const int row = row0 + 64 * i;
            if (row < ROWS) {
                const int off = tr_off<HD>(row, ch * 2);
                *reinterpret_cast<u32x4v*>(ldsQ + off) = pq[i];
                *reinterpret_cast<u32x4v*>(ldsK + off) = pk[i];
                *reinterpret_cast<u32x4v*>(ldsO + off) = pg[i];
                const bf16x8_t x = __builtin_bit_cast(bf16x8_t, pg[i]), y = __builtin_bit_cast(bf16x8_t, po[i]);
                float dl = 0.f;
#pragma unroll
                for (int j = 0; j < 8; ++j) dl += (float)x[j] * (float)y[j];
                dl += __shfl_xor(dl, 1, 64);
                dl += __shfl_xor(dl, 2, 64);
                dl += __shfl_xor(dl, 4, 64);
                if (ch == 0) ldsD[row] = -dl * a.scale;
            }
        }
    }
    int srow[2], smask[2];
#pragma unroll
    for (int u = 0; u < 2; ++u) {
        const int krow = (u < nu ? (tile0 + u) * 16 : ROWS) + c;
        srow[u] = krow * 64;
        smask[u] = ds_swz(krow);
    }
    f32x4_t adk[2][DT], adv[2][DT];
#pragma unroll
    for (int u = 0; u < 2; ++u)
#pragma unroll
        for (int dt = 0; dt < DT; ++dt) { adk[u][dt] = (f32x4_t){0.f, 0.f, 0.f, 0.f}; adv[u][dt] = adk[u][dt]; }
    __syncthreads();
    bf16x8_t ktf[NKB];
#pragma unroll
    for (int kb = 0; kb < NKB; ++kb) ktf[kb] = frag_tr_perm<HD>(ldsK + kb * 32 * HD * 2, my_dt, lane);
    auto scores = [&](int i, bf16x8_t (&pf)[2], bf16x8_t (&dsf)[2]) {
        const int qc = i * CH;
        const char* sQ = ldsQ + qc * HD * 2;
        const char* sO = ldsO + qc * HD * 2;
        char* const sS = ldsS + (i & 1) * LDS_S1;
// ... 655 lines not shown
    const int64_t total = (int64_t)nb * nq * H * cpr;
    for (int64_t i = (int64_t)blockIdx.x * 256 + threadIdx.x; i < total; i += (int64_t)gridDim.x * 256) {
        const int ck = (int)(i % cpr);
        const int h = (int)((i / cpr) % H);
        const int qq = (int)((i / ((int64_t)cpr * H)) % nq);
        const int b = (int)(i / ((int64_t)cpr * H * nq));
        float ls[8], m = -INFINITY;
        for (int sp = 0; sp < S; ++sp) {
            ls[sp] = lse_s[((int64_t)(b * S + sp) * H + h) * nq + qq];
            m = fmaxf(m, ls[sp]);
        }
        float tot = 0.f, acc[8] = {0.f, 0.f, 0.f, 0.f, 0.f, 0.f, 0.f, 0.f};
        for (int sp = 0; sp < S; ++sp) {
            const float w = __expf(ls[sp] - m);
            tot += w;
            float v[8];
            load8(o_s + ((int64_t)(b * S + sp) * nq + qq) * ld_s + h * hd + ck * 8, v);
#pragma unroll
            for (int j = 0; j < 8; ++j) acc[j] += w * v[j];
        }
        const float inv = 1.f / tot;
#pragma unroll
        for (int j = 0; j < 8; ++j) acc[j] *= inv;
        store8(out + ((int64_t)b * nq + qq) * ldo + h * hd + ck * 8, acc);
        if (ck == 0) lse[((int64_t)b * H + h) * nq + qq] = m + __logf(tot);
    }
}

std::atomic<int> g_opt_lean{-1}, g_opt_onepass{-1};
inline bool xcd_map_enabled() {
    static const int e0 = [] { const char* e = vpu_lab_getenv("VPU_ATTN_XCDMAP"); return e ? atoi(e) : 1; }();
    return e0 != 0;
}
inline int onepass_enabled() {
    static const int e0 = [] { const char* e = getenv("VPU_ATTN_ONEPASS"); return e ? atoi(e) : 3; }();
    const int v = g_opt_onepass.load(std::memory_order_relaxed);
    return v >= 0 ? v : e0;
}
inline bool wide_two() {
    static const int e0 = [] { const char* e = vpu_lab_getenv("VPU_ATTN_WIDE2"); return e ? atoi(e) : 1; }();
    return e0 != 0;
}
inline bool lean_enabled() {
    static const int e0 = [] { const char* e = getenv("VPU_ATTN_LEAN"); return e ? atoi(e) : 1; }();
    const int v = g_opt_lean.load(std::memory_order_relaxed);
    return (v >= 0 ? v : e0) != 0;
}

inline bool ok16(const void* p) { return (reinterpret_cast<uintptr_t>(p) & 15) == 0; }

int hd_image(int hd) { return hd <= 32 ? 32 : (hd <= 64 ? 64 : 128); }
int hd_computed(int hd) { return hd_image(hd) == 128 && hd <= 96 ? 96 : hd_image(hd); }

thread_local char g_last_attn[192] = "";

}

extern "C" const char* vpu_attn_last_kernel(void) { return g_last_attn; }

extern "C" int vpu_attn_set_option(const char* name, int32_t value) {
    vpu_clear_stale_error();
    if (name && !strcmp(name, "lean") && value >= -1 && value <= 1) {
        g_opt_lean.store(value, std::memory_order_relaxed);
        return VPU_OK;
    }
    if (name && !strcmp(name, "onepass") && value >= -1 && value <= 3) {
        g_opt_onepass.store(value, std::memory_order_relaxed);
        return VPU_OK;
    }
    vpu_set_error("vpu_attn_set_option: known options: lean (-1 environment default VPU_ATTN_LEAN, 0 round-1 step kernels, 1 lean kernels), "
                  "onepass (-1 environment default VPU_ATTN_ONEPASS, 0 two-kernel backward, 1 one-pass backward for window-sized problems with one workgroup per problem, 2 in key passes with three workgroups per CU, 3 persistent workgroups that fetch the next problem while they compute (65 <= n <= 224; 1 elsewhere))");
    return VPU_ERR_ARG;
}

static int xattn_fwd_impl(const void* q, const void* k, const void* v, void* out, float* lse, int32_t nb, int32_t H,
                          int32_t nq, int32_t nk, int32_t hd, int32_t ldq, int32_t ldk, int32_t ldo, float scale, int32_t qdiv,
                          int32_t kdiv, void* stream) {
    vpu_clear_stale_error();
    if (qdiv < 1 || kdiv < 1 || (qdiv > 1 && kdiv > 1) || nb % (qdiv * kdiv) || ((qdiv > 1 || kdiv > 1) && !lean_enabled())) {
        vpu_set_error("xattn_fwd_split: qdiv, kdiv >= 1, one of them 1, nb a multiple of the other; the lean kernels only");
        return VPU_ERR_ARG;
    }
    if (hd <= 0 || hd > 128 || hd % 16 || ldq % 8 || ldk % 8 || ldo % 8 || !ok16(q) || !ok16(k) || !ok16(v) || !ok16(out) || nb <= 0 ||
        H <= 0 || nq <= 0 || nk <= 0 || (int64_t)nk * ldk >= (1 << 29)) {
        vpu_set_error("xattn_fwd: head dim a multiple of 16 up to 128, 16-byte aligned slices (q, k, v, out), row strides % 8 == 0, one batch entry of k/v below 1 GiB");
        return VPU_ERR_ARG;
    }
    AttnArgs a{};
    a.q = (const bf16_t*)q; a.k = (const bf16_t*)k; a.v = (const bf16_t*)v; a.out = (bf16_t*)out; a.lse = lse;
    a.nq = nq; a.nk = nk; a.H = H; a.hd = hd; a.ldq = ldq; a.ldk = ldk; a.ldo = ldo; a.scale = scale;
    a.qdiv = qdiv; a.kdiv = kdiv;
    hipStream_t s = reinterpret_cast<hipStream_t>(stream);
    if (lean_enabled()) {
        const bool two = nq > 64 && (hd_image(hd) <= 64 || wide_two());
        dim3 grid(two ? (nq + 127) / 128 : (nq + 63) / 64, nb * H);
        if (xcd_map_enabled() && grid.x > 1) { a.gx = grid.x; a.nbh = nb * H; grid = dim3(grid.x * grid.y); }
        snprintf(g_last_attn, sizeof(g_last_attn), "attn_fwd_lean_kernel<%d, %d, %d>", hd_image(hd), two ? 2 : 1, hd_computed(hd));
        switch (hd_image(hd) * 4 + (two ? 2 : 1)) {
            case 128 * 4 + 2:
                if (hd <= 96) attn_fwd_lean_kernel<128, 2, 96><<<grid, 256, 0, s>>>(a);
                else attn_fwd_lean_kernel<128, 2, 128><<<grid, 256, 0, s>>>(a);
                break;
            case 32 * 4 + 2: attn_fwd_lean_kernel<32, 2, 32><<<grid, 256, 0, s>>>(a); break;
            case 32 * 4 + 1: attn_fwd_lean_kernel<32, 1, 32><<<grid, 256, 0, s>>>(a); break;
            case 64 * 4 + 2: attn_fwd_lean_kernel<64, 2, 64><<<grid, 256, 0, s>>>(a); break;
            case 64 * 4 + 1: attn_fwd_lean_kernel<64, 1, 64><<<grid, 256, 0, s>>>(a); break;
            default:
                if (hd <= 96) attn_fwd_lean_kernel<128, 1, 96><<<grid, 256, 0, s>>>(a);
                else attn_fwd_lean_kernel<128, 1, 128><<<grid, 256, 0, s>>>(a);
                break;
        }
        return vpu_check_launch("vpu_xattn_fwd");
    }
    static const int qt2 = [] { const char* e = vpu_lab_getenv("VPU_ATTN_QT"); return e ? atoi(e) : 2; }();
    const bool two = qt2 == 2 && nq > 64 && nk <= 256 && hd_image(hd) <= 64;
    dim3 grid(two ? (nq + 127) / 128 : (nq + 63) / 64, nb * H);
    snprintf(g_last_attn, sizeof(g_last_attn), "attn_fwd_kernel<%d, 1, %d>", hd_image(hd), two ? 2 : 1);
    if (two) {
        if (hd_image(hd) == 32) attn_fwd_kernel<32, 1, 2><<<grid, 256, 0, s>>>(a);
        else attn_fwd_kernel<64, 1, 2><<<grid, 256, 0, s>>>(a);
        return vpu_check_launch("vpu_xattn_fwd");
    }
    switch (hd_image(hd)) {
        case 32: attn_fwd_kernel<32, 1, 1><<<grid, 256, 0, s>>>(a); break;
        case 64: attn_fwd_kernel<64, 1, 1><<<grid, 256, 0, s>>>(a); break;
        default: attn_fwd_kernel<128, 1, 1><<<grid, 256, 0, s>>>(a); break;
    }
    return vpu_check_launch("vpu_xattn_fwd");
}

extern "C" int vpu_xattn_fwd(const void* q, const void* k, const void* v, void* out, float* lse, int32_t nb, int32_t H,
                             int32_t nq, int32_t nk, int32_t hd, int32_t ldq, int32_t ldk, int32_t ldo, float scale,
                             void* stream) {
    return xattn_fwd_impl(q, k, v, out, lse, nb, H, nq, nk, hd, ldq, ldk, ldo, scale, 1, 1, stream);
}
extern "C" int vpu_xattn_fwd_split(const void* q, const void* k, const void* v, void* out, float* lse, int32_t nb, int32_t H,
                                   int32_t nq, int32_t nk, int32_t hd, int32_t ldq, int32_t ldk, int32_t ldo, float scale,
                                   int32_t qdiv, int32_t kdiv, void* stream) {
    return xattn_fwd_impl(q, k, v, out, lse, nb, H, nq, nk, hd, ldq, ldk, ldo, scale, qdiv, kdiv, stream);
}
extern "C" int vpu_attn_combine(const void* o_s, const float* lse_s, void* out, float* lse, int32_t nb, int32_t H, int32_t nq,
                                int32_t hd, int32_t S, int32_t ld_s, int32_t ldo, void* stream) {
    vpu_clear_stale_error();
    if (!o_s || !lse_s || !out || !lse || nb < 1 || H < 1 || nq < 1 || hd < 8 || hd % 8 || S < 1 || S > 8 || ld_s % 8 || ldo % 8) {
        vpu_set_error("attn_combine: non-null operands, head dim and row strides multiples of 8, 1 <= S <= 8");
        return VPU_ERR_ARG;
    }
    const int64_t total = (int64_t)nb * nq * H * (hd / 8);
    attn_combine_kernel<<<vpu_grid_for(total, 256, 4096), 256, 0, reinterpret_cast<hipStream_t>(stream)>>>(
        (const bf16_t*)o_s, lse_s, (bf16_t*)out, lse, nb, H, nq, hd, S, ld_s, ldo);
    return vpu_check_launch("vpu_attn_combine");
}

static int xattn_bwd_impl(const void* q, const void* k, const void* v, const void* o, const void* d_o,
                          const float* lse, float* delta, void* dq, void* dk, void* dv, int32_t nb, int32_t H,
                          int32_t nq, int32_t nk, int32_t hd, int32_t ldq, int32_t ldk, int32_t ldo, int32_t ldgq,
                          int32_t ldgk, float scale, int32_t qdiv, int32_t kdiv, void* stream) {
    vpu_clear_stale_error();
    const bool split = qdiv > 1 || kdiv > 1;
    if (qdiv < 1 || kdiv < 1 || (qdiv > 1 && kdiv > 1) || nb % (qdiv * kdiv) || (split && (!lean_enabled() || nq % 4))) {
        vpu_set_error("xattn_bwd_split: qdiv, kdiv >= 1, one of them 1, nb a multiple of the other; the lean kernels only (nq % 4 == 0)");
        return VPU_ERR_ARG;
    }
    if (hd <= 0 || hd > 128 || hd % 16 || ldq % 8 || ldk % 8 || ldo % 8 || !ok16(q) || !ok16(k) || !ok16(v) || !ok16(o) ||
        !ok16(d_o) || nb <= 0 || H <= 0 || nq <= 0 || nk <= 0 || (int64_t)nk * ldk >= (1 << 29) ||
        (int64_t)nq * ldq >= (1 << 29) || (int64_t)nq * ldo >= (1 << 29)) {
        vpu_set_error("xattn_bwd: head dim a multiple of 16 up to 128, 16-byte aligned slices, row strides % 8 == 0, one batch entry per matrix below 1 GiB");
        return VPU_ERR_ARG;
    }
    AttnArgs a{};
    a.q = (const bf16_t*)q; a.k = (const bf16_t*)k; a.v = (const bf16_t*)v; a.o = (const bf16_t*)o;
    a.d_o = (const bf16_t*)d_o; a.lse = const_cast<float*>(lse); a.delta = delta;
    a.dq = (bf16_t*)dq; a.dk = (bf16_t*)dk; a.dv = (bf16_t*)dv;
    a.nq = nq; a.nk = nk; a.H = H; a.hd = hd; a.ldq = ldq; a.ldk = ldk; a.ldo = ldo; a.ldgq = ldgq; a.ldgk = ldgk;
    a.scale = scale; a.qdiv = qdiv; a.kdiv = kdiv;
    hipStream_t s = reinterpret_cast<hipStream_t>(stream);
    if (!split && lean_enabled() && onepass_enabled() == 2 && hd == 64 && nq == nk && nq <= 32 * WIN_MAX_KB && ldgq % 4 == 0 && ldgk % 4 == 0 &&
        (reinterpret_cast<uintptr_t>(dq) & 7) == 0 && (reinterpret_cast<uintptr_t>(dk) & 7) == 0 && (reinterpret_cast<uintptr_t>(dv) & 7) == 0) {
        static VpuDevOnce attrp;
        if (auto todo_ = attrp.pending()) {
            VPU_SET_LDS(WpCfg<1>::LDS, attn_bwd_winp_kernel<1>);
        }
        snprintf(g_last_attn, sizeof(g_last_attn), "attn_bwd_winp_kernel<1>");
        attn_bwd_winp_kernel<1><<<dim3(nb * H), 256, WpCfg<1>::LDS, s>>>(a);
        return vpu_check_launch("vpu_xattn_bwd");
    }
    const bool win_ok = !split && lean_enabled() && hd == 64 && nq == nk && nq <= 32 * WIN_MAX_KB && ldgq % 4 == 0 && ldgk % 4 == 0 &&
        (reinterpret_cast<uintptr_t>(dq) & 7) == 0 && (reinterpret_cast<uintptr_t>(dk) & 7) == 0 && (reinterpret_cast<uintptr_t>(dv) & 7) == 0;
    {
        const int64_t trows = (int64_t)nb * nq, lim = (int64_t)1 << 30;
        const int nkb = (nq + 31) / 32;
        if (win_ok && onepass_enabled() == 3 && nkb >= 3 && nkb <= 7 && trows * ldq < lim && trows * ldk < lim && trows * ldo < lim &&
            trows * ldgq < lim && trows * ldgk < lim && (int64_t)nb * H * nq < lim / 2) {
            const int ncu = vpu_cu_budget();
            a.nbh = nb * H;
            const int grid = a.nbh < ncu ? a.nbh : ncu;
            snprintf(g_last_attn, sizeof(g_last_attn), "attn_bwd_winx_kernel");
#define WINX_CASE(NKB_)                                                                               \
            case NKB_: {                                                                              \
                static VpuDevOnce attr;                                                               \
                if (auto todo_ = attr.pending()) { VPU_SET_LDS(WxCfg<NKB_>::LDS, attn_bwd_winx_kernel<NKB_>); } \
                attn_bwd_winx_kernel<NKB_><<<dim3(grid), 512, WxCfg<NKB_>::LDS, s>>>(a);              \
            } break;
            switch (nkb) { WINX_CASE(3) WINX_CASE(4) WINX_CASE(5) WINX_CASE(6) WINX_CASE(7) }
#undef WINX_CASE
            return vpu_check_launch("vpu_xattn_bwd");
        }
    }
    if (win_ok && onepass_enabled()) {
        snprintf(g_last_attn, sizeof(g_last_attn), "attn_bwd_win_kernel");
#define WIN_CASE(NKB_)                                                                           \
        case NKB_: {                                                                             \
            static VpuDevOnce attr;                                                              \
            if (auto todo_ = attr.pending()) { VPU_SET_LDS(win_lds(NKB_), attn_bwd_win_kernel<NKB_>); } \
            attn_bwd_win_kernel<NKB_><<<dim3(nb * H), 512, win_lds(NKB_), s>>>(a);               \
        } break;
        switch ((nq + 31) / 32) {
            WIN_CASE(1) WIN_CASE(2) WIN_CASE(3) WIN_CASE(4) WIN_CASE(5) WIN_CASE(6) WIN_CASE(7) WIN_CASE(8)
        }
#undef WIN_CASE
        return vpu_check_launch("vpu_xattn_bwd");
    }
    if (lean_enabled() && nq % 4 == 0) {
        const bool q2 = nq > 64 && (hd_image(hd) <= 64 || wide_two()), k2 = nk > 64 && hd_image(hd) <= 64;
        dim3 gq(q2 ? (nq + 127) / 128 : (nq + 63) / 64, nb * H), gk(k2 ? (nk + 127) / 128 : (nk + 63) / 64, nb * H);
        AttnArgs ak = a;
        if (xcd_map_enabled() && gq.x > 1) { a.gx = gq.x; a.nbh = nb * H; gq = dim3(gq.x * gq.y); }
        if (xcd_map_enabled() && gk.x > 1) { ak.gx = gk.x; ak.nbh = nb * H; gk = dim3(gk.x * gk.y); }
        snprintf(g_last_attn, sizeof(g_last_attn), "attn_bwd_dq_lean_kernel<%d, %d, %d> attn_bwd_dkdv_lean_kernel<%d, %d, %d>",
                 hd_image(hd), q2 ? 2 : 1, hd_computed(hd), hd_image(hd), k2 ? 2 : 1, hd_computed(hd));
        switch (hd_image(hd) * 4 + (q2 ? 2 : 1)) {
            case 128 * 4 + 2:
                if (hd <= 96) attn_bwd_dq_lean_kernel<128, 2, 96><<<gq, 256, 0, s>>>(a);
                else attn_bwd_dq_lean_kernel<128, 2, 128><<<gq, 256, 0, s>>>(a);
                break;
            case 32 * 4 + 2: attn_bwd_dq_lean_kernel<32, 2, 32><<<gq, 256, 0, s>>>(a); break;
            case 32 * 4 + 1: attn_bwd_dq_lean_kernel<32, 1, 32><<<gq, 256, 0, s>>>(a); break;
            case 64 * 4 + 2: attn_bwd_dq_lean_kernel<64, 2, 64><<<gq, 256, 0, s>>>(a); break;
            case 64 * 4 + 1: attn_bwd_dq_lean_kernel<64, 1, 64><<<gq, 256, 0, s>>>(a); break;
            default:
                if (hd <= 96) attn_bwd_dq_lean_kernel<128, 1, 96><<<gq, 256, 0, s>>>(a);
                else attn_bwd_dq_lean_kernel<128, 1, 128><<<gq, 256, 0, s>>>(a);
                break;
        }
        switch (hd_image(hd) * 4 + (k2 ? 2 : 1)) {
            case 32 * 4 + 2: attn_bwd_dkdv_lean_kernel<32, 2, 32><<<gk, 256, 0, s>>>(ak); break;
            case 32 * 4 + 1: attn_bwd_dkdv_lean_kernel<32, 1, 32><<<gk, 256, 0, s>>>(ak); break;
            case 64 * 4 + 2: attn_bwd_dkdv_lean_kernel<64, 2, 64><<<gk, 256, 0, s>>>(ak); break;
            case 64 * 4 + 1: attn_bwd_dkdv_lean_kernel<64, 1, 64><<<gk, 256, 0, s>>>(ak); break;
            default:
                if (hd <= 96) attn_bwd_dkdv_lean_kernel<128, 1, 96><<<gk, 256, 0, s>>>(ak);
                else attn_bwd_dkdv_lean_kernel<128, 1, 128><<<gk, 256, 0, s>>>(ak);
                break;
        }
        return vpu_check_launch("vpu_xattn_bwd");
    }
    dim3 gk((nk + 63) / 64, nb * H), gq((nq + 63) / 64, nb * H);
    snprintf(g_last_attn, sizeof(g_last_attn), "attn_bwd_dq_kernel<%d, 1> attn_bwd_dkdv_kernel<%d, 1>", hd_image(hd), hd_image(hd));
    switch (hd_image(hd)) {
        case 32:
            attn_bwd_dq_kernel<32, 1><<<gq, 256, 0, s>>>(a);
            attn_bwd_dkdv_kernel<32, 1><<<gk, 256, 0, s>>>(a);
            break;
        case 64:
            attn_bwd_dq_kernel<64, 1><<<gq, 256, 0, s>>>(a);
            attn_bwd_dkdv_kernel<64, 1><<<gk, 256, 0, s>>>(a);
            break;
        default:
            attn_bwd_dq_kernel<128, 1><<<gq, 256, 0, s>>>(a);
            attn_bwd_dkdv_kernel<128, 1><<<gk, 256, 0, s>>>(a);
            break;
    }
    return vpu_check_launch("vpu_xattn_bwd");
}

extern "C" int vpu_xattn_bwd(const void* q, const void* k, const void* v, const void* o, const void* d_o,
                             const float* lse, float* delta, void* dq, void* dk, void* dv, int32_t nb, int32_t H,
                             int32_t nq, int32_t nk, int32_t hd, int32_t ldq, int32_t ldk, int32_t ldo, int32_t ldgq,
                             int32_t ldgk, float scale, void* stream) {
    return xattn_bwd_impl(q, k, v, o, d_o, lse, delta, dq, dk, dv, nb, H, nq, nk, hd, ldq, ldk, ldo, ldgq, ldgk, scale, 1, 1, stream);
}
extern "C" int vpu_xattn_bwd_split(const void* q, const void* k, const void* v, const void* o, const void* d_o,
                                   const float* lse, float* delta, void* dq, void* dk, void* dv, int32_t nb, int32_t H,
                                   int32_t nq, int32_t nk, int32_t hd, int32_t ldq, int32_t ldk, int32_t ldo, int32_t ldgq,
                                   int32_t ldgk, float scale, int32_t qdiv, int32_t kdiv, void* stream) {
    return xattn_bwd_impl(q, k, v, o, d_o, lse, delta, dq, dk, dv, nb, H, nq, nk, hd, ldq, ldk, ldo, ldgq, ldgk, scale, qdiv, kdiv, stream);
}

extern "C" int vpu_attn_fwd(const void* q, const void* k, const void* v, void* out, float* lse, int32_t nb, int32_t H,
                            int32_t n, int32_t hd, int32_t ld, int32_t ldo, float scale, void* stream) {
    return vpu_xattn_fwd(q, k, v, out, lse, nb, H, n, n, hd, ld, ld, ldo, scale, stream);
}

extern "C" int vpu_attn_bwd(const void* q, const void* k, const void* v, const void* o, const void* d_o,
                            const float* lse, float* delta, void* dq, void* dk, void* dv, int32_t nb, int32_t H,
                            int32_t n, int32_t hd, int32_t ld, int32_t ldo, int32_t ldg, float scale, void* stream) {
    return vpu_xattn_bwd(q, k, v, o, d_o, lse, delta, dq, dk, dv, nb, H, n, n, hd, ld, ld, ldo, ldg, ldg, scale, stream);
}
```

### pvpuformer_amd/csrc/gemm.hip

```cpp
#include <stdio.h>
#include <stdlib.h>
#include <string.h>
#include <atomic>
#include "vpu_common.h"
#include "../../include/vpu_hip.h"
#include "gemm_tiles.h"

int vpu_k5_option();
void vpu_k5_set_option(int v);
void vpu_k5_set_grid(int v);
void vpu_k5_set_split(int v);
void vpu_k5_set_noepi(int v);
int vpu_k5_launch(const vpu_gemm_desc* d, int rb, int ncu, int vec, void* stream, char* name, size_t name_len);
#ifdef VPU_DIAG
void vpu_k5_set_dbg(unsigned long long* p);
#endif

namespace {


template <typename T>
__device__ __forceinline__ void epilogue_store(const vpu_gemm_desc& p, int64_t coff, int64_t roff, int m, int n,
                                               float acc) {
    const int flags = p.flags;
// ... 1947 lines not shown
            float v[8] = {0.f, 0.f, 0.f, 0.f, 0.f, 0.f, 0.f, 0.f};
            for (int s = 0; s < splitk; ++s) {
                float t[8];
                load8(w + s * mn + i * 8, t);
#pragma unroll
                for (int j = 0; j < 8; ++j) v[j] += t[j];
            }
            EpiPre e;
            e.has_pre = false; e.has_bias = false; e.pre = make_uint4(0, 0, 0, 0);
            epilogue_store8(p, p.flags, coff, roff, m, n, v, e);
        }
    } else
    for (int64_t i = (int64_t)blockIdx.x * 256 + threadIdx.x; i < mn; i += (int64_t)gridDim.x * 256) {
        float v = 0.f;
        for (int s = 0; s < splitk; ++s) v += w[s * mn + i];
        epilogue_store<T>(p, coff, roff, (int)(i / p.N), (int)(i % p.N), v);
    }
    if (p.colsum != nullptr && z == 0) {
        __shared__ float redc[32][8];
        const float* wb = ws + (int64_t)gridDim.z * splitk * mn;
        const int mi = threadIdx.x & 7, sl = threadIdx.x >> 3;
        for (int mb = blockIdx.x * 8; mb < p.M; mb += gridDim.x * 8) {
            const int m = mb + mi;
            float t = 0.f;
            if (m < p.M)
                for (int s = sl; s < splitk; s += 32) t += wb[(int64_t)s * p.M + m];
            __syncthreads();
            redc[sl][mi] = t;
            __syncthreads();
            if (sl == 0 && m < p.M) {
                for (int q = 1; q < 32; ++q) t += redc[q][mi];
                p.colsum[m] += t;
            }
        }
    }
}

constexpr int FM = 64, FN = 64, FK = 16, FLD = 68;

template <int TRANS>
__device__ __forceinline__ void f32_stage(const float* base, int ld, int x0, int X, int k0, int K, float* lds,
                                          int tid) {
    if (TRANS == 0) {
        const int row = tid >> 2, kc = (tid & 3) * 4;
        float4 v = make_float4(0.f, 0.f, 0.f, 0.f);
        const int gx = x0 + row, gk = k0 + kc;
        if (gx < X && gk < K) v = *reinterpret_cast<const float4*>(base + (int64_t)gx * ld + gk);
        lds[(kc + 0) * FLD + row] = v.x;
        lds[(kc + 1) * FLD + row] = v.y;
        lds[(kc + 2) * FLD + row] = v.z;
        lds[(kc + 3) * FLD + row] = v.w;
    } else {
        const int k = tid >> 4, cc = (tid & 15) * 4;
        float4 v = make_float4(0.f, 0.f, 0.f, 0.f);
        const int gk = k0 + k, gx = x0 + cc;
        if (gk < K && gx < X) v = *reinterpret_cast<const float4*>(base + (int64_t)gk * ld + gx);
        *reinterpret_cast<float4*>(&lds[k * FLD + cc]) = v;
    }
}

template <int TA, int TB>
__global__ __launch_bounds__(256) void gemm_f32_kernel(const vpu_gemm_desc p, const int tiles_n) {
    __shared__ __attribute__((aligned(16))) float ldsA[FK * FLD];
    __shared__ __attribute__((aligned(16))) float ldsB[FK * FLD];
    const int tid = threadIdx.x, lane = tid & 63, wave = tid >> 6;
    const int wm = wave >> 1, wn = wave & 1;
    const int tile_m = blockIdx.x / tiles_n, tile_n = blockIdx.x % tiles_n;
    const int m0 = tile_m * FM, n0 = tile_n * FN;
    const int z = blockIdx.z, zo = z / p.inner, zi = z % p.inner;
    const float* A = reinterpret_cast<const float*>(p.A) + zo * p.sAo + zi * p.sAi;
    const float* B = reinterpret_cast<const float*>(p.B) + zo * p.sBo + zi * p.sBi;
    const int64_t coff = zo * p.sCo + zi * p.sCi;
    const int64_t roff = zo * p.sRo + zi * p.sRi;

    f32x4_t acc[2][2];
#pragma unroll
    for (int i = 0; i < 2; ++i)
#pragma unroll
        for (int j = 0; j < 2; ++j) acc[i][j] = (f32x4_t){0.f, 0.f, 0.f, 0.f};
    const int fr = lane & 15, fq = lane >> 4;
    const int nk = (p.K + FK - 1) / FK;
    for (int kt = 0; kt < nk; ++kt) {
        f32_stage<TA>(A, p.lda, m0, p.M, kt * FK, p.K, ldsA, tid);
        f32_stage<TB>(B, p.ldb, n0, p.N, kt * FK, p.K, ldsB, tid);
        __syncthreads();
#pragma unroll
        for (int ks = 0; ks < 4; ++ks) {
            const int k = ks * 4 + fq;
            float a[2], b[2];
#pragma unroll
            for (int i = 0; i < 2; ++i) a[i] = ldsA[k * FLD + wm * 32 + i * 16 + fr];
#pragma unroll
            for (int j = 0; j < 2; ++j) b[j] = ldsB[k * FLD + wn * 32 + j * 16 + fr];
#pragma unroll
            for (int i = 0; i < 2; ++i)
#pragma unroll
                for (int j = 0; j < 2; ++j)
                    acc[i][j] = __builtin_amdgcn_mfma_f32_16x16x4f32(a[i], b[j], acc[i][j], 0, 0, 0);
        }
        __syncthreads();
    }
#pragma unroll
    for (int i = 0; i < 2; ++i)
#pragma unroll
        for (int r = 0; r < 4; ++r) {
            const int m = m0 + wm * 32 + i * 16 + fq * 4 + r;
            if (m >= p.M) continue;
#pragma unroll
            for (int j = 0; j < 2; ++j) {
                const int n = n0 + wn * 32 + j * 16 + fr;
                if (n < p.N) epilogue_store<float>(p, coff, roff, m, n, acc[i][j][r]);
            }
        }
}

inline bool aligned_to(const void* p, size_t a) { return (reinterpret_cast<uintptr_t>(p) % a) == 0; }

thread_local char g_last_kernel[160] = "";
#define NOTE_KERNEL(...) snprintf(g_last_kernel, sizeof(g_last_kernel), __VA_ARGS__)
std::atomic<int> g_opt_ring{-1};
std::atomic<int> g_opt_inlaunch{-1};
std::atomic<int> g_opt_skinny{-1};
std::atomic<int> g_opt_skinny_group{-1};
std::atomic<int> g_opt_k2{-1};
std::atomic<int> g_opt_k3{-1};
inline int k3_env0() {
    static const int v = [] { const char* e = getenv("VPU_GEMM_K3"); return e ? atoi(e) : 28; }();
    return v;
}
inline int k3_opt() {
    int v = g_opt_k3.load(std::memory_order_relaxed);
    v = v >= 0 ? v : k3_env0();
#ifndef VPU_LAB
    v &= ~3;
    if (v & 8) v |= 16;
#endif
    return v;
}
inline int k2_env0() {
    static const int v = [] { const char* e = getenv("VPU_GEMM_K2"); return e ? atoi(e) : 2; }();
    return v;
}
inline int k2_opt() { const int v = g_opt_k2.load(std::memory_order_relaxed); return v >= 0 ? v : k2_env0(); }
std::atomic<int> g_opt_reserve{0};
#ifdef VPU_DIAG
std::atomic<unsigned long long*> g_dbg_times{nullptr};
#endif
inline int cu_count() {
    static const int v = [] { int dev = 0, n = 0; (void)hipGetDevice(&dev); (void)hipDeviceGetAttribute(&n, hipDeviceAttributeMultiprocessorCount, dev); return n > 0 ? n : 256; }();
    const int r = g_opt_reserve.load(std::memory_order_relaxed);
    const int left = (v - r) & ~7;
    return left >= 64 ? left : v;
}
inline int inlaunch_env0() {
    static const int v = [] { const char* e = vpu_lab_getenv("VPU_GEMM_INLAUNCH"); return e ? atoi(e) : 0; }();
    return v;
}
constexpr int64_t CNT_BYTES = 256 << 10;
inline int ring_env0() {
    static const int v = [] { const char* e = vpu_lab_getenv("VPU_GEMM_RING"); return e ? atoi(e) : 0; }();
    return v;
}

}

extern "C" int vpu_gemm(const vpu_gemm_desc* d, void* stream) {
    vpu_clear_stale_error();
    if (!d || !d->A || !d->B || !d->C) { vpu_set_error("vpu_gemm: null operand"); return VPU_ERR_ARG; }
    if (d->M <= 0 || d->N <= 0 || d->K <= 0 || d->batch <= 0 || d->inner <= 0 || d->batch % d->inner) {
        vpu_set_error("vpu_gemm: bad sizes (M,N,K,batch > 0; batch % inner == 0)");
        return VPU_ERR_ARG;
    }
    if (d->colsum && d->cs_tn > 1) {
        vpu_set_error("vpu_gemm: cs_tn > 1 (distributed column sums) is a vpu_gemm_grouped form");
        return VPU_ERR_ARG;
    }
    const int f = d->flags;
    if (((f & VPU_EPI_BIAS) && !d->bias) || ((f & VPU_EPI_RESID) && !d->resid) ||
        ((f & (VPU_EPI_DGELU | VPU_EPI_DRELU | VPU_EPI_MULAUX)) && !d->aux) ||
        ((f & (VPU_EPI_PREACT | VPU_EPI_SAVE_DGELU)) && !d->preact) ||
        ((f & VPU_EPI_SAVE_DGELU) && (!(f & VPU_EPI_GELU) || (f & VPU_EPI_PREACT)))) {
        vpu_set_error("vpu_gemm: epilogue flag set but its pointer is null");
        return VPU_ERR_ARG;
    }
    const bool bf = d->dtype == VPU_BF16;
    if (!bf && d->dtype != VPU_F32) { vpu_set_error("vpu_gemm: dtype"); return VPU_ERR_ARG; }
    if (d->colsum && (!bf || !d->transA || d->batch != 1)) {
        vpu_set_error("vpu_gemm: colsum needs the bf16 path, transA=1 and batch=1");
        return VPU_ERR_ARG;
    }
    const int64_t q = bf ? 8 : 4;
    const bool strides_ok = d->lda % q == 0 && d->ldb % q == 0 && d->sAo % q == 0 && d->sAi % q == 0 &&
                            d->sBo % q == 0 && d->sBi % q == 0;
    if (!strides_ok || !aligned_to(d->A, 16) || !aligned_to(d->B, 16)) {
        vpu_set_error("vpu_gemm: A/B base, leading dimensions and batch strides must be 16-byte multiples");
        return VPU_ERR_ALIGN;
    }
    if (bf) {
        const int64_t ea = d->transA ? (int64_t)d->K * d->lda : (int64_t)d->M * d->lda;
        const int64_t eb = d->transB ? (int64_t)d->K * d->ldb : (int64_t)d->N * d->ldb;
        if (ea * 2 >= 0x7FFFFFF0LL || eb * 2 >= 0x7FFFFFF0LL) {
            vpu_set_error("vpu_gemm: an operand spans more than 2 GiB per batch entry");
            return VPU_ERR_ARG;
        }
    }
    hipStream_t s = reinterpret_cast<hipStream_t>(stream);
    static const int force_big = [] { const char* e = vpu_lab_getenv("VPU_GEMM_BIG"); return e ? (e[0] == '1' ? 1 : 0) : -1; }();
#ifdef VPU_LAB
    const bool big = bf && force_big == 1 && d->M >= 1024 && d->N >= 128 && d->K >= 256;
#else
    const bool big = false;
    (void)force_big;
#endif
    const int tm = bf ? (big ? BM2 : BM) : FM, tn = bf ? BN : FN;
    const int tiles_m = (d->M + tm - 1) / tm, tiles_n = (d->N + tn - 1) / tn;
    const int key = (d->transA ? 2 : 0) | (d->transB ? 1 : 0);
    if (bf) {
        const size_t cbytes = (f & VPU_EPI_OUT_F32) ? 32 : 16;
        bool vec = d->ldc % 8 == 0 && d->sCo % 8 == 0 && d->sCi % 8 == 0 && aligned_to(d->C, cbytes);
        if (f & VPU_EPI_BIAS) vec = vec && aligned_to(d->bias, 32);
        if (f & (VPU_EPI_PREACT | VPU_EPI_SAVE_DGELU)) vec = vec && aligned_to(d->preact, 16);
        if (f & (VPU_EPI_DGELU | VPU_EPI_DRELU | VPU_EPI_MULAUX)) vec = vec && d->ldaux % 8 == 0 && aligned_to(d->aux, 16);
        if (f & VPU_EPI_RESID)
            vec = vec && d->ldr % 8 == 0 && d->sRo % 8 == 0 && d->sRi % 8 == 0 && aligned_to(d->resid, 16);
        const int64_t tiles = (int64_t)tiles_m * tiles_n * d->batch;
        int splitk = 1, kchunk = (d->K + BK - 1) / BK * BK;
        const int ring_env = g_opt_ring.load(std::memory_order_relaxed) >= 0 ? g_opt_ring.load(std::memory_order_relaxed) : ring_env0();
        static const int ring_min = [] { const char* e = vpu_lab_getenv("VPU_GEMM_RING_MIN"); return e ? atoi(e) : 96; }();
#ifdef VPU_LAB
        const bool ring = !big && (ring_env == 2 || (ring_env == 1 && tiles >= ring_min && tiles <= 256 && d->K <= 24 * BK && d->K > 2 * BK));
#else
        const bool ring = false;
        (void)ring_env; (void)ring_min;
#endif
        if (!ring && d->workspace && (tiles < 192 || (tiles <= 256 && d->K >= 32 * BK)) && d->K >= 8 * BK) {
            int64_t want = (384 + tiles - 1) / tiles;
            const int64_t max_by_k = d->K / (4 * BK);
            const int64_t max_by_ws = (d->workspace_bytes - CNT_BYTES) / ((int64_t)d->batch * d->M * (d->N + 1) * 4);
            if (want > max_by_k) want = max_by_k;
            if (want > max_by_ws) want = max_by_ws;
            if (want > 128) want = 128;
            if (want > 1) {
                kchunk = (int)(((d->K + want - 1) / want + BK - 1) / BK * BK);
                splitk = (d->K + kchunk - 1) / kchunk;
            }
        }
#ifdef VPU_LAB
        static const int forms3 = [] { const char* e = vpu_lab_getenv("VPU_GEMM_K3_FORMS"); return e ? atoi(e) : 0; }();
        if (((k3_opt() & 2) || forms3) && !big && d->batch == 1 && !d->colsum && vec && d->N % 8 == 0 && d->K % K3_BK == 0 && d->K >= 256 &&
            !d->transA && d->alpha == 1.0f && (int64_t)d->M * d->ldc * 2 < 0x7FFFFFF0LL &&
            (int64_t)d->M * (d->ldr > d->ldaux ? d->ldr : d->ldaux) * 2 < 0x7FFFFFF0LL) {
            static const bool noepi3 = [] { const char* e = vpu_lab_getenv("VPU_GEMM_NOEPI"); return e && e[0] == '1'; }();
            static const int rb3_env = [] { const char* e = vpu_lab_getenv("VPU_GEMM_K2_RB"); return e ? atoi(e) : 0; }();
            constexpr int F_B = VPU_EPI_BIAS, F_BR = VPU_EPI_BIAS | VPU_EPI_RESID,
                          F_G = VPU_EPI_BIAS | VPU_EPI_GELU | VPU_EPI_SAVE_DGELU, F_M = VPU_EPI_MULAUX;
            const int tn3 = (d->N + 127) / 128;
            const int64_t t256 = (int64_t)((d->M + 255) / 256) * tn3, t224 = (int64_t)((d->M + 223) / 224) * tn3;
            const bool short3 = rb3_env != 8 && (rb3_env == 7 || t224 * 224 < t256 * 256);
            const int64_t tot3 = short3 ? t224 : t256;
            const int cap3 = 2 * cu_count();
            bool done3 = tot3 > cu_count();
            static const int stag3 = [] { const char* e = vpu_lab_getenv("VPU_GEMM_K3_STAGGER"); return e ? atoi(e) : 0; }();
            const int vec3 = (noepi3 ? 9 : 1) | (stag3 << 8);
#define VPU_LAUNCH_K3_RB(TA_, TB_, FL_, RB_)                                                                         \
    do {                                                                                                             \
        static VpuDevOnce attr_;                                                                                   \
        auto kern_ = gemm_bf16_k3_kernel<TA_, TB_, FL_, RB_>;                                                         \
        if (auto todo_ = attr_.pending()) {                                                                                                \
            VPU_SET_LDS(K3_LDS, kern_); \
        }                                                                                                            \
        const int tm_ = (d->M + 32 * RB_ - 1) / (32 * RB_);                                                           \
        const int tot_ = tm_ * tn3;                                                                                  \
        NOTE_KERNEL("gemm_bf16_k3_kernel<%d, %d, %d, %d>", TA_, TB_, FL_, RB_);                                        \
        kern_<<<dim3((unsigned)(tot_ < cap3 ? tot_ : cap3)), dim3(256), K3_LDS, s>>>(*d, tm_, tn3, vec3);              \
    } while (0)
#define VPU_LAUNCH_K3(TA_, TB_, FL_) do { if (short3) VPU_LAUNCH_K3_RB(TA_, TB_, FL_, 7); else VPU_LAUNCH_K3_RB(TA_, TB_, FL_, 8); } while (0)
            const bool all3 = (k3_opt() & 2) != 0;
            if (!done3) {}
            else if (key == 0 && f == F_B && (all3 || (forms3 & 1))) VPU_LAUNCH_K3(0, 0, F_B);
            else if (key == 0 && f == F_BR && (all3 || (forms3 & 2))) VPU_LAUNCH_K3(0, 0, F_BR);
            else if (key == 0 && f == F_G && (all3 || (forms3 & 4))) VPU_LAUNCH_K3(0, 0, F_G);
            else if (key == 1 && f == 0 && (all3 || (forms3 & 8))) VPU_LAUNCH_K3(0, 1, 0);
            else if (key == 1 && f == F_M && (all3 || (forms3 & 16))) VPU_LAUNCH_K3(0, 1, F_M);
            else done3 = false;
#undef VPU_LAUNCH_K3
#undef VPU_LAUNCH_K3_RB
            if (done3) return vpu_check_launch("vpu_gemm");
        }
#endif
        {
            static const bool noepi2 = [] { const char* e = vpu_lab_getenv("VPU_GEMM_NOEPI"); return e && e[0] == '1'; }();
            const int k2 = k2_opt();
            static const int k2_min_tiles = [] { const char* e = vpu_lab_getenv("VPU_GEMM_K2_MIN_TILES"); return e ? atoi(e) : 120; }();
            const int tm2 = (d->M + K2_BM - 1) / K2_BM, tn2 = (d->N + 127) / 128;
            const int ncu_k2 = cu_count();
            auto k2_cost = [&](int bm, int bn) {
                const int64_t t = (int64_t)((d->M + bm - 1) / bm) * ((d->N + bn - 1) / bn);
                return ((t + ncu_k2 - 1) / ncu_k2) * bm;
            };
            int rbn = 8;
            {
                static const int rb_min = [] { const char* e = vpu_lab_getenv("VPU_GEMM_K2_RBMIN"); const int v = e ? atoi(e) : 6; return v < 5 ? 5 : (v > 8 ? 8 : v); }();
                int64_t best = k2_cost(256, 128);
                for (int rb = 7; rb >= rb_min; --rb) {
                    const int64_t c = k2_cost(32 * rb, 128);
                    if (c < best) { best = c; rbn = rb; }
                }
                if ((int64_t)((d->M + 32 * rbn - 1) / (32 * rbn)) * tn2 < k2_min_tiles && (int64_t)((d->M + 159) / 160) * tn2 >= k2_min_tiles) rbn = 5;
// ... 616 lines not shown
```

### pvpuformer_amd/engine.py

```python
import contextlib
import math
import os
from collections import OrderedDict
from types import SimpleNamespace

import numpy as np
import torch

from . import ops
from ._lib import (BF16, F32, EPI_BIAS, EPI_PREACT, EPI_GELU, EPI_RELU, EPI_DGELU, EPI_DRELU, EPI_RESID, EPI_AFFINE,
                   EPI_ACCUM, EPI_OUT_F32, EPI_SAVE_DGELU, EPI_MULAUX)


class Tape:
    __slots__ = ("fns", "out_grads", "done", "sim_low", "lane")

    def __init__(self):
        self.fns = []
        self.out_grads = [None, None, None]
        self.done = False
        self.sim_low = None
        self.lane = None

    def append(self, fn):
        s = self.lane
        if s is not None:
            inner = fn

            def fn():
                with torch.cuda.stream(s):
                    inner()
        self.fns.append(fn)

    def __len__(self):
        return len(self.fns)


class Var:
    __slots__ = ("t", "g", "gn_stats")

    def __init__(self, t):
        self.t = t
        self.g = None
        self.gn_stats = None


def _rup(x, m):
    return (x + m - 1) // m * m


def click_lut():
    t = np.arange(0, 19, 1, np.float32)
    lut = np.exp(-((t - 9) ** 2) / (2 * 3 ** 2))
    lut[9] += 1
    return lut


def pos2d_table(d_model, height, width):
    pe = torch.zeros(d_model, height, width)
    half = d_model // 2
    div = torch.exp(torch.arange(0., half, 2) * -(math.log(10000.0) / half))
    pw = torch.arange(0., width).unsqueeze(1) * div
    ph = torch.arange(0., height).unsqueeze(1) * div
    pe[0:half:2] = torch.sin(pw).t().unsqueeze(1).expand(-1, height, -1)
    pe[1:half:2] = torch.cos(pw).t().unsqueeze(1).expand(-1, height, -1)
    pe[half::2] = torch.sin(ph).t().unsqueeze(2).expand(-1, -1, width)
    pe[half + 1::2] = torch.cos(ph).t().unsqueeze(2).expand(-1, -1, width)
    return pe.reshape(d_model, height * width).t().contiguous()


def window_geometry(S, P):
    S, P = int(S), int(P)
    wg = 224 // P
    g = S // P if P > 0 else 0
    if P < 1 or wg < 1 or g < wg:
        raise ValueError(f"input side {S} with patch {P}: the token grid S // P = {g} must hold at least one "
                         f"{wg}-token window (S >= {wg * P})")
    nwin = g // wg
    if g % nwin:
        raise ValueError(f"input side {S} with patch {P}: the token grid g = S // P = {g} must split into nwin = g // {wg} = "
                         f"{nwin} equal windows per side (g % nwin == 0), as the reference's patchify requires")
    return g, nwin, g // nwin


def check_square(H, W):
    if H != W:
        raise ValueError(f"input {H}x{W}: only square inputs are supported (the reference's neck takes h = w = sqrt(HW))")


class Engine:
    def __init__(self, cfg, dtype="bf16", device="cuda"):
        self.cfg = dict(cfg)
        self.dt = BF16 if dtype in ("bf16", BF16) else F32
        self.td = torch.bfloat16 if self.dt == BF16 else torch.float32
        self.dev = torch.device(device)
        c = self.cfg
        self.D, self.P, self.img = c["embed_dim"], c["patch"], c["img"]
        self.g, _, self.wside = window_geometry(self.img, self.P)
        self.NT = self.g * self.g
        self.heads = c["num_heads"]
        self.depth = c["depth"]
        self.group = 6 if self.depth == 12 else self.depth // 4
        self.nmax = c["num_max_points"]
        self.E = 2 * self.img + 3
        self.Epad = _rup(self.E, 8)
        self.C = c["head_channels"]
        self.out_dims = tuple(c["out_dims"])
        self.names = None
        self.tape = Tape()
        self.last_tape = None
        self.params = []
        self.norm_radius = float(c.get("norm_radius", 5))
        self.training = False
        self.shadow_valid = False
        self._const_ready = False
        self.use_flash = True
        self.use_side = os.environ.get("VPU_WGRAD_STREAM", "0") == "1"
        self.side = None
        self.fuse_ln_pe = True
        self.group_wgrad = True
        self.ride_wgrad = True
        self.wgrad_fill = 0.8
        hid = self.D * c["mlp_ratio"]
        blk = sum(((n + 255) // 256) * ((k + 127) // 128) for n, k in ((3 * self.D, self.D), (self.D, self.D), (hid, self.D), (self.D, hid)))
        pk = os.environ.get("VPU_WGRAD_PACK", "")
        k3 = ops.gemm_get_option("k3")
        k4_default = (k3 & 8) != 0
        self.pack_wgrad = pk == "1" or (pk != "0" and (blk < 0.95 * 256 or k4_default))
        self.k3_wgrad = (k3 & 1) != 0
        self.k4_wgrad = (k3 & 8) != 0
        self.wgrad_round = 256 if (self.k4_wgrad or not self.k3_wgrad) else 512
        self.wgrad_tn = 256 if self.k4_wgrad else 128
        self.unify_wgrad = True
        self.lazy_zero = True
        self.xattn_split = max(1, int(os.environ.get("VPU_XATTN_SPLIT", "1")))
        self.neck_lanes = int(os.environ.get("VPU_NECK_LANES", "0"))
        self._tok_stream = None
        self._in_lanes = False
        self.dist_colsum = True
        self._pack_seen, self._pack_total = {}, {}
        self._pending_reports, self._reporting = [], False
        self.group_tiles = 256
        self.split_wgrad = True
        self._wq = []
        self._csq = []
        self._gq = []
        self._gq_out = set()
        self._frozen = set()
        self._token_rows = 0
        self.grad_ready_hook = None
        self.report_lag = max(1, int(os.environ.get("VPU_DIST_REPORT_LAG", "2")))

    def bind(self, named_params):
        self.names = OrderedDict()
        off = 0
        for n, p in named_params.items():
            self.names[n] = (off, tuple(p.shape), p.numel())
            off = _rup(off + p.numel(), 8)
        self.total = off
        self.flat = torch.zeros(off, device=self.dev, dtype=torch.float32)
        self.gflat = torch.zeros(off, device=self.dev, dtype=torch.float32)
        self.params = []
        for n, p in named_params.items():
            o, shape, numel = self.names[n]
            view = self.flat[o:o + numel].view(shape)
            view.copy_(p.data)
            p.data = view
            p.grad = self.gflat[o:o + numel].view(shape)
            self.params.append((p, o, shape, numel))
        self.shadow = torch.zeros(off, device=self.dev, dtype=torch.bfloat16) if self.dt == BF16 else None
        self._lazy = set()
        self._lazy_names, self._lazy_ranges = self._lazy_plan()
        D, P = self.D, self.P
        self.k3p = _rup(3 * P * P, 8)
        self.w_patch = torch.zeros(D, 2 * self.k3p, device=self.dev, dtype=self.td)
        self.b_patch = torch.zeros(D, device=self.dev, dtype=torch.float32)
        self.w_lin1p = torch.zeros(2048, self.Epad, device=self.dev, dtype=self.td)
        self.pos_win = torch.zeros(self.NT, D, device=self.dev, dtype=self.td)
        self._pos_cache, self._kpe_cache, self._regrid_cache = {}, {}, {}
        self.shadow_valid = False
        if not self._const_ready:
            self.kpe = pos2d_table(D, self.g, self.g).to(self.dev).to(self.td)
            self.lut = torch.from_numpy(click_lut()).to(self.dev)
            self._const_ready = True

    def W(self, name):
        o = self.names[name][0]
        return (self.shadow, o) if self.dt == BF16 else (self.flat, o)

    def Pm(self, name):
        return (self.flat, self.names[name][0])

    def G(self, name):
        return (self.gflat, self.names[name][0])

    def refresh_weights(self, shadow_is_fresh=False):
        D, P = self.D, self.P
        if self.dt == BF16 and not shadow_is_fresh:
            ops.cast2d(self.flat, self.total, self.shadow, self.total, 1, self.total)
        k3 = 3 * P * P
        po = self.names["backbone.pos_embed"][0]
        ops.cast2d_batched([
            dict(src=self.Pm("backbone.patch_embed.proj.weight"), dst=(self.w_patch, 0), ld_src=k3, ld_dst=2 * self.k3p, rows=D, cols=k3),
            dict(src=self.Pm("patch_embed_coords.proj.weight"), dst=(self.w_patch, self.k3p), ld_src=k3, ld_dst=2 * self.k3p, rows=D,
                 cols=k3),
            dict(src=self.Pm("backbone.patch_embed.proj.bias"), src2=self.Pm("patch_embed_coords.proj.bias"), dst=self.b_patch,
                 ld_src=D, ld_dst=D, rows=1, cols=D),
            dict(src=self.Pm("neck.ffn_layer.lin1.weight"), dst=self.w_lin1p, ld_src=self.E, ld_dst=self.Epad, rows=2048, cols=self.E,
                 cols_pad=self.Epad),
            dict(src=(self.flat, po + D), dst=self.pos_win, ld_src=D, ld_dst=D, rows=self.NT, cols=D, perm=(self.g, self.wside)),
        ])
        self._pos_cache = {(self.g, self.wside): self.pos_win}
        self.shadow_valid = True

    def _regrid_adjoint(self, g):
        Rt = self._regrid_cache.get(g)
        if Rt is None:
            import torch.nn.functional as F
            g0 = self.g
            basis = torch.eye(g0 * g0, dtype=torch.float32).view(1, g0 * g0, g0, g0)
            Rt = F.interpolate(basis, size=(g, g), mode="bicubic", align_corners=False).reshape(g0 * g0, g * g)
            Rt = Rt.contiguous().to(self.dev)
            self._regrid_cache[g] = Rt
        return Rt

    def _pos_for(self, g, wside):
        pw = self._pos_cache.get((g, wside))
        if pw is None:
            import torch.nn.functional as F
            D, g0 = self.D, self.g
            po = self.names["backbone.pos_embed"][0]
            grid = self.flat[po + D: po + D + g0 * g0 * D].view(1, g0, g0, D).permute(0, 3, 1, 2)
            new = F.interpolate(grid, size=(g, g), mode="bicubic", align_corners=False).permute(0, 2, 3, 1)
            tmp = new.reshape(g * g, D).to(self.td).contiguous()
            pw = torch.empty(g * g, D, device=self.dev, dtype=self.td)
            ops.window_permute(tmp, pw, 1, g, wside, D, to_raster=False)
            self._pos_cache[(g, wside)] = pw
        return pw

    def _kpe_for(self, g):
        k = self._kpe_cache.get(g)
        if k is None:
            k = self.kpe if g == self.g else pos2d_table(self.D, g, g).to(self.dev).to(self.td)
            self._kpe_cache[g] = k
        return k

    def zero_grad(self, lazy=False):
        self._lazy = set()
        if (lazy and self.lazy_zero and self.group_wgrad and self.dt == BF16 and not self.use_side and self.pack_wgrad
                and self._lazy_ranges is not None):
            ops.zero_ranges_(self.gflat, self._lazy_ranges)
            self._lazy = set(self._lazy_names)
        else:
            ops.zero_(self.gflat)

    def _lazy_plan(self):
        names = [n for n in self.names if n.startswith("backbone.blocks.") and
                 n.endswith((".attn.qkv.weight", ".attn.proj.weight", ".mlp.fc1.weight", ".mlp.fc2.weight"))]
        ranges, pos = [], 0
        for n in names:
            o, _, numel = self.names[n]
            if o % 4 or numel % 4:
                return [], None
            if o > pos:
                ranges.append((pos, o - pos))
            pos = o + numel
        if self.total > pos:
            ranges.append((pos, self.total - pos))
        return names, (ranges if names else None)

    def _lazy_finish(self):
        if self._lazy:
            ops.zero_ranges_(self.gflat, [(self.names[n][0], self.names[n][2]) for n in sorted(self._lazy, key=lambda k: self.names[k][0])])
            self._lazy = set()

    def attach_grads(self):
        if not self.params:
            return
        def ok(e):
            p, o, shape, numel = e
            return p.grad is not None and p.grad.data_ptr() == self.gflat.data_ptr() + 4 * o
        if ok(self.params[0]) and ok(self.params[-1]):
            return
        for e in self.params:
            p, o, shape, numel = e
            if ok(e):
                continue
            seg = self.gflat[o:o + numel]
# ... 191 lines not shown
                h["bev"].record(self._cur(dst))
            self.tape.fns.append(bwd)

    def linear(self, x, wname, bname, M, N, K, act=None, resid=None, out=None, x_grad=True, group=False, pre_masked=None):
        assert not (act and resid is not None)
        if out is None:
            y = Var(self._new(M, N))
            yt, yoff, ldc = y.t, 0, N
        else:
            y, yoff, ldc = out
            yt = y.t
        flags = EPI_BIAS | (EPI_RELU if act == "relu" else 0) | (EPI_RESID if resid is not None else 0)
        group = group and self.dt == BF16 and act is None and resid is None and out is None
        g_args = (x.t, self.W(wname), (yt, yoff), M, N, K, K, K, ldc, self.dt)
        g_kw = dict(flags=flags, bias=self.Pm(bname), resid=None if resid is None else resid.t, ldr=N)
        if group:
            self._gemm_deferred(yt.data_ptr(), g_args, g_kw)
        else:
            ops.gemm(*g_args, **g_kw)
        if self.training:
            def bwd():
                if y.g is None:
                    return
                dy = (y.g, yoff)
                if resid is not None:
                    assert out is None
                    self.acc(resid, y.g, take=True)
                if act == "relu" and not (pre_masked is not None and pre_masked[0]):
                    dz = self._new(M, N)
                    ops.act_bwd(dy, ldc, (yt, yoff), ldc, dz, N, M, N, 0, self.dt)
                    dy, ld = dz, N
                else:
                    ld = ldc
                self._wgrad(dy, ld, x.t, K, wname, N, K, M, bias=bname)
                if x_grad:
                    self._dgrad(dy, ld, self.W(wname), K, x, M, K, N, defer=group)
            self.tape.append(bwd)
        return y

    def mlp(self, x, p1, p2, M, K, Hd, N, act, resid=None, w1=None, k_grad=None, x_grad=True):
        Kp = K
        h = self._new(M, Hd)
        if act == "gelu":
            pre = self._new(M, Hd)
            ops.gemm(x.t, self.W(p1 + ".weight") if w1 is None else w1, h, M, Hd, Kp, Kp, Kp, Hd, self.dt,
                     flags=EPI_BIAS | EPI_SAVE_DGELU | EPI_GELU, bias=self.Pm(p1 + ".bias"), preact=pre)
        else:
            pre = None
            ops.gemm(x.t, self.W(p1 + ".weight") if w1 is None else w1, h, M, Hd, Kp, Kp, Kp, Hd, self.dt,
                     flags=EPI_BIAS | EPI_RELU, bias=self.Pm(p1 + ".bias"))
        y = Var(self._new(M, N))
        ops.gemm(h, self.W(p2 + ".weight"), y.t, M, N, Hd, Hd, Hd, N, self.dt,
                 flags=EPI_BIAS | (EPI_RESID if resid is not None else 0), bias=self.Pm(p2 + ".bias"),
                 resid=None if resid is None else resid.t, ldr=N)
        if self.training:
            def bwd():
                dy = y.g
                if dy is None:
                    return
                if resid is not None:
                    self.acc(resid, dy, take=True)
                self._wgrad(dy, N, h, Hd, p2 + ".weight", N, Hd, M, bias=p2 + ".bias")
                dpre = self._new(M, Hd)
                ops.gemm(dy, self.W(p2 + ".weight"), dpre, M, Hd, N, N, Hd, Hd, self.dt, transB=True,
                         flags=EPI_MULAUX if act == "gelu" else EPI_DRELU, aux=pre if act == "gelu" else h, ldaux=Hd)
                kg = K if k_grad is None else k_grad
                self._wgrad(dpre, Hd, x.t, Kp, p1 + ".weight", Hd, kg, M, bias=p1 + ".bias")
                if x_grad:
                    self._dgrad(dpre, Hd, self.W(p1 + ".weight") if w1 is None else w1, Kp, x, M, Kp, Hd)
            self.tape.append(bwd)
        return y

    def layernorm(self, x, prefix, rows, Cdim, eps, pe=None, pe_rows=0, pe_var=None):
        if pe is not None and not self.fuse_ln_pe:
            y = self.layernorm(x, prefix, rows, Cdim, eps)
            return y, self.add_pe(y, pe, rows * Cdim, pe_rows * Cdim, pe_var=pe_var)
        y = Var(self._new(rows, Cdim))
        yy = Var(self._new(rows, Cdim)) if pe is not None else None
        mean, rstd = self._new(rows, dtype=torch.float32), self._new(rows, dtype=torch.float32)
        if pe is None:
            ops.layernorm_fwd(x.t, self.Pm(prefix + ".weight"), self.Pm(prefix + ".bias"), y.t, mean, rstd, rows, Cdim, eps)
        else:
            ops.layernorm_fwd_pe(x.t, self.Pm(prefix + ".weight"), self.Pm(prefix + ".bias"), y.t, mean, rstd, rows, Cdim,
                                 eps, pe, pe_rows, yy.t)
        if self.training:
            def bwd():
                dy, dy2 = y.g, (yy.g if yy is not None else None)
                if dy is None and dy2 is None:
                    return
                if dy2 is not None and pe_var is not None:
                    self.acc(pe_var, dy2)
                if dy is None:
                    dy, dy2 = dy2, None
                nblk = ops.layernorm_bwd_nblk(rows)
                part = self._new(nblk, 2, Cdim, dtype=torch.float32)
                dres = x.g
                if x.g is None or x.g.data_ptr() in self._frozen:
                    x.g = torch.empty_like(x.t)
                ops.layernorm_bwd(dy, x.t, self.Pm(prefix + ".weight"), mean, rstd, dres, x.g, part, rows, Cdim, dy2=dy2)
                self._reduce_wb(part, nblk, prefix, Cdim)
            self.tape.append(bwd)
        return y if pe is None else (y, yy)

    def sdpa(self, q, k, v, o, nb, H, nq, nk, hd, scale):
        (qv, qo, qld, qrows), (kv, ko, kld, krows), (vv, vo, vld, vrows), (ov, oo, old, orows) = q, k, v, o
        ldS = _rup(nk, 8)
        S = self._new(nb * H, nq, ldS, dtype=torch.float32)
        sS = (H * nq * ldS, nq * ldS)
        ops.gemm((qv.t, qo), (kv.t, ko), S, nq, nk, hd, qld, kld, ldS, self.dt, flags=EPI_OUT_F32, alpha=scale,
                 batch=nb * H, inner=H, sA=(qrows * qld, hd), sB=(krows * kld, hd), sC=sS)
        Pm = self._new(nb * H, nq, ldS)
        ops.softmax_fwd(S, ldS, Pm, ldS, nb * H * nq, nk)
        del S
        ops.gemm(Pm, (vv.t, vo), (ov.t, oo), nq, hd, nk, ldS, vld, old, self.dt, transB=True, batch=nb * H, inner=H,
                 sA=sS, sB=(vrows * vld, hd), sC=(orows * old, hd))
        if self.training:
            def bwd():
                if ov.g is None:
                    return
                for var in {id(qv): qv, id(kv): kv, id(vv): vv}.values():
                    assert var.g is None, "sdpa inputs must be single-use projections"
                    var.g = torch.empty_like(var.t)
                dO = (ov.g, oo)
                dP = self._new(nb * H, nq, ldS, dtype=torch.float32)
                ops.gemm(dO, (vv.t, vo), dP, nq, nk, hd, old, vld, ldS, self.dt, flags=EPI_OUT_F32, batch=nb * H,
                         inner=H, sA=(orows * old, hd), sB=(vrows * vld, hd), sC=sS)
                ops.gemm(Pm, dO, (vv.g, vo), nk, hd, nq, ldS, old, vld, self.dt, transA=True, transB=True, batch=nb * H,
                         inner=H, sA=sS, sB=(orows * old, hd), sC=(vrows * vld, hd))
                dS = self._new(nb * H, nq, ldS)
                ops.softmax_bwd(Pm, ldS, dP, ldS, dS, nb * H * nq, nk, scale)
                del dP
                ops.gemm(dS, (kv.t, ko), (qv.g, qo), nq, hd, nk, ldS, kld, qld, self.dt, transB=True, batch=nb * H,
                         inner=H, sA=sS, sB=(krows * kld, hd), sC=(qrows * qld, hd))
                ops.gemm(dS, (qv.t, qo), (kv.g, ko), nk, hd, nq, ldS, qld, kld, self.dt, transA=True, transB=True,
                         batch=nb * H, inner=H, sA=sS, sB=(qrows * qld, hd), sC=(krows * kld, hd))
            self.tape.append(bwd)

    def flash_attention(self, qkv, O, nb, H, n, hd, D, scale):
        lse = self._new(nb * H, n, dtype=torch.float32)
        ops.attn_fwd((qkv.t, 0), (qkv.t, D), (qkv.t, 2 * D), O.t, lse, nb, H, n, hd, 3 * D, D, scale)
        if self.training:
            def bwd():
                if O.g is None:
                    return
                assert qkv.g is None
                qkv.g = torch.empty_like(qkv.t)
                delta = self._new(nb * H, n, dtype=torch.float32)
                ops.attn_bwd((qkv.t, 0), (qkv.t, D), (qkv.t, 2 * D), O.t, O.g, lse, delta, (qkv.g, 0), (qkv.g, D),
                             (qkv.g, 2 * D), nb, H, n, hd, 3 * D, D, 3 * D, scale)
            self.tape.append(bwd)

    def cross_attention(self, Qp, Kp, Vp, O, nb, H, nq, nk, hd, ld, scale):
        S = self.xattn_split
        long_q = S > 1 and nq >= 4 * nk and nq % (4 * S) == 0 and nq // S >= 64
        long_k = S > 1 and not long_q and nk >= 4 * nq and nk % S == 0 and nk // S >= 64 and nq % 4 == 0
        if long_q:
            lse = self._new(nb * S * H, nq // S, dtype=torch.float32)
            ops.xattn_fwd_split(Qp.t, Kp.t, Vp.t, O.t, lse, nb * S, H, nq // S, nk, hd, ld, ld, ld, scale, 1, S)
        elif long_k:
            lse = self._new(nb * H, nq, dtype=torch.float32)
            o_s, lse_s = self._new(nb * S * nq, ld), self._new(nb * S * H, nq, dtype=torch.float32)
            ops.xattn_fwd_split(Qp.t, Kp.t, Vp.t, o_s, lse_s, nb * S, H, nq, nk // S, hd, ld, ld, ld, scale, S, 1)
            ops.attn_combine(o_s, lse_s, O.t, lse, nb, H, nq, hd, S, ld, ld)
        else:
            lse = self._new(nb * H, nq, dtype=torch.float32)
            ops.xattn_fwd(Qp.t, Kp.t, Vp.t, O.t, lse, nb, H, nq, nk, hd, ld, ld, ld, scale)
        if self.training:
            def bwd():
                if O.g is None:
                    return
                for var in {id(Qp): Qp, id(Kp): Kp, id(Vp): Vp}.values():
                    assert var.g is None, "attention inputs must be single-use projections"
                    var.g = torch.empty_like(var.t)
                if long_q:
                    delta = self._new(nb * S * H, nq // S, dtype=torch.float32)
                    dkp, dvp = self._new(nb * S * nk, ld), self._new(nb * S * nk, ld)
                    ops.xattn_bwd_split(Qp.t, Kp.t, Vp.t, O.t, O.g, lse, delta, Qp.g, dkp, dvp, nb * S, H, nq // S, nk, hd, ld, ld,
                                        ld, ld, ld, scale, 1, S)
                    ops.sum_groups(dkp, Kp.g, nb, S, nk * ld)
                    ops.sum_groups(dvp, Vp.g, nb, S, nk * ld)
                elif long_k:
                    delta = self._new(nb * H, nq, dtype=torch.float32)
                    dqp = self._new(nb * S * nq, ld)
                    ops.xattn_bwd_split(Qp.t, Kp.t, Vp.t, O.t, O.g, lse, delta, dqp, Kp.g, Vp.g, nb * S, H, nq, nk // S, hd, ld, ld,
                                        ld, ld, ld, scale, S, 1)
                    ops.sum_groups(dqp, Qp.g, nb, S, nq * ld)
                else:
                    delta = self._new(nb * H, nq, dtype=torch.float32)
                    ops.xattn_bwd(Qp.t, Kp.t, Vp.t, O.t, O.g, lse, delta, Qp.g, Kp.g, Vp.g, nb, H, nq, nk, hd, ld, ld, ld,
                                  ld, ld, scale)
            self.tape.append(bwd)

    def add_pe(self, x, pe, n, period, pe_var=None):
        y = Var(torch.empty_like(x.t))
        ops.add_bcast(x.t, pe, y.t, n, period)
        if self.training:
            def bwd():
                if y.g is None:
                    return
                if pe_var is not None:
                    self.acc(pe_var, y.g)
                self.acc(x, y.g, take=True)
            self.tape.append(bwd)
        return y

    def _group(self, fn):
        if self.training:
            self.tape.append(self.flush_group)
        r = fn()
        self.flush_group()
        return r

    def _proj(self, prefix, which, x, rows, width):
        return self.linear(x, f"{prefix}.{which}_proj.weight", f"{prefix}.{which}_proj.bias", rows, width, self.D, group=True)

    def _attend(self, B, prefix, Qp, Kp, Vp, nq, nk, width, resid):
        H, hd = 8, width // 8
        O = Var(self._new(B * nq, width))
        if self.dt == BF16 and self.use_flash and hd % 16 == 0 and hd <= 128:
            self.cross_attention(Qp, Kp, Vp, O, B, H, nq, nk, hd, width, 1.0 / math.sqrt(hd))
        else:
            self.sdpa((Qp, 0, width, nq), (Kp, 0, width, nk), (Vp, 0, width, nk), (O, 0, width, nq), B, H, nq, nk, hd,
                      1.0 / math.sqrt(hd))
        return self.linear(O, prefix + ".out_proj.weight", prefix + ".out_proj.bias", B * nq, self.D, width, resid=resid)

    def mha(self, prefix, xq, xk, xv, B, nq, nk, internal, resid=None):
        Qp, Kp, Vp = self._group(lambda: (self._proj(prefix, "q", xq, B * nq, internal), self._proj(prefix, "k", xk, B * nk, internal),
                                          self._proj(prefix, "v", xv, B * nk, internal)))
        return self._attend(B, prefix, Qp, Kp, Vp, nq, nk, internal, resid)

    def groupnorm(self, x, prefix, B, HW, Cdim, gelu):
        y = Var(torch.empty_like(x.t))
        nch = ops.groupnorm_nchunk()
        mean, rstd = self._new(B, dtype=torch.float32), self._new(B, dtype=torch.float32)
        stats = getattr(x, "gn_stats", None)
        if stats is not None:
            ops.groupnorm_apply(x.t, self.Pm(prefix + ".weight"), self.Pm(prefix + ".bias"), y.t, mean, rstd, stats, B, HW,
                                Cdim, 1e-5, gelu)
        else:
            stats = self._new(B, nch, 2, dtype=torch.float64)
            ops.groupnorm_fwd(x.t, self.Pm(prefix + ".weight"), self.Pm(prefix + ".bias"), y.t, mean, rstd, stats, B, HW,
                              Cdim, 1e-5, gelu)
        if self.training:
            def bwd():
                if y.g is None:
                    return
                assert x.g is None
                x.g = torch.empty_like(x.t)
                part = self._new(B * nch, 2, Cdim, dtype=torch.float32)
                ops.groupnorm_bwd(y.g, x.t, self.Pm(prefix + ".weight"), self.Pm(prefix + ".bias"), mean, rstd, x.g,
                                  part, stats, B, HW, Cdim, gelu)
                self._reduce_wb(part, B * nch, prefix, Cdim)
            self.tape.append(bwd)
        return y

    def conv_t2(self, x, prefix, B, h, w, Cin, Cout, gn_next=False):
        M = B * h * w
        t = self._new(M, 4 * Cout)
        ops.gemm(x.t, self.W(prefix + ".weight"), t, M, 4 * Cout, Cin, Cin, 4 * Cout, 4 * Cout, self.dt, transB=True)
        y = Var(self._new(B * 4 * h * w, Cout))
        if gn_next and Cout % 8 == 0:
            y.gn_stats = self._new(B, ops.groupnorm_nchunk(), 2, dtype=torch.float64)
            ops.pixel_shuffle2_gn_stats(t, y.t, self.Pm(prefix + ".bias"), y.gn_stats, B, h, w, Cout)
        else:
            ops.pixel_shuffle2(t, y.t, self.Pm(prefix + ".bias"), B, h, w, Cout)
        del t
        if self.training:
            def bwd():
                if y.g is None:
                    return
                dt = self._new(M, 4 * Cout)
                if Cout % 8 == 0 and Cout <= 2048:
                    part, nb = ops.pixel_unshuffle2_sums(y.g, dt, B, h, w, Cout)
                    self._csq.append((part, self.G(prefix + ".bias"), nb, Cout))
                else:
                    ops.pixel_shuffle2(y.g, dt, None, B, h, w, Cout, inverse=True)
                    self._colsum_to(y.g, Cout, prefix + ".bias", B * 4 * h * w, Cout)
                if self.unify_wgrad and self.pack_wgrad and self.dt == BF16 and self.group_wgrad and not self.use_side:
                    self._wgrad(x.t, Cin, dt, 4 * Cout, prefix + ".weight", Cin, 4 * Cout, M)
                else:
                    ops.gemm(x.t, dt, self.G(prefix + ".weight"), Cin, 4 * Cout, M, Cin, 4 * Cout, 4 * Cout, self.dt,
                             transA=True, transB=True, flags=EPI_OUT_F32 | EPI_ACCUM)
                f = 0
                if x.g is None:
                    x.g = torch.empty_like(x.t)
                else:
                    self._writable(x.g)
                    f = EPI_ACCUM
                ops.gemm(dt, self.W(prefix + ".weight"), x.g, M, Cin, 4 * Cout, 4 * Cout, 4 * Cout, Cin, self.dt, flags=f)
            self.tape.append(bwd)
        return y

    def conv_s2(self, x, prefix, B, h, w, Cin, Cout, g=None):
        odd = g is not None and g % 2 == 1
        assert g is None or (h == w == g // 2)
        M = B * h * w
        s2d = self._new(M, 4 * Cin)
        if odd:
            ops.space_to_depth2_crop(x.t, s2d, B, g, Cin)
        else:
            ops.pixel_shuffle2(x.t, s2d, None, B, h, w, Cin, inverse=True)
        y = Var(self._new(M, Cout))
        ops.gemm(s2d, self.W(prefix + ".weight"), y.t, M, Cout, 4 * Cin, 4 * Cin, 4 * Cin, Cout, self.dt,
                 flags=EPI_BIAS, bias=self.Pm(prefix + ".bias"))
        if self.training:
            def bwd():
                if y.g is None:
                    return
                self._wgrad(y.g, Cout, s2d, 4 * Cin, prefix + ".weight", Cout, 4 * Cin, M, bias=prefix + ".bias")
                ds = self._new(M, 4 * Cin)
                ops.gemm(y.g, self.W(prefix + ".weight"), ds, M, 4 * Cin, Cout, Cout, 4 * Cin, 4 * Cin, self.dt,
                         transB=True)
                if odd:
                    dx = self._new(B * g * g, Cin)
                    ops.space_to_depth2_crop(ds, dx, B, g, Cin, inverse=True)
                else:
                    dx = self._new(B * 4 * h * w, Cin)
                    ops.pixel_shuffle2(ds, dx, None, B, h, w, Cin)
                self.acc(x, dx, take=True)
            self.tape.append(bwd)
        return y

    def forward(self, image4, points, boxes=None, prompt_type=0, drop_mask=None, training=False, taps=None,
                materialize_aux=True, scribble=None, coord_override=None, prenorm=False, kinds=None):
        assert image4.is_cuda and image4.dtype == torch.float32 and image4.is_contiguous()
        if not self.shadow_valid:
            self.refresh_weights()
        self.training = training
        self.tape = Tape()
        B, H, W_ = image4.shape[0], image4.shape[2], image4.shape[3]
        D = self.D
        check_square(H, W_)
        g, nw_side, wside = window_geometry(H, self.P)
        NT = g * g
        pos_win, kpe_tab = self._pos_for(g, wside), self._kpe_for(g)
        self._token_rows = B * NT
        n = points.shape[1] // 2
        points = self._upload(points, torch.float32)
        boxes = self._upload(boxes, torch.int32) if prompt_type in (1, 3) else None
        curve = prof = rows = None
        if prompt_type == 2:
            curve = self._upload(scribble[0], torch.int32)
            prof = self._upload(scribble[1], torch.float64)
            assert curve.shape[0] == B and tuple(prof.shape) == (B, 2 * self.img)
# ... 514 lines not shown
            c = cols * tn
            head = ((dy, x, g, N, c, M, ld_dy, ld_x, ldc, dt), hkw, t128(N, c), red)
            tkw = dict(kw, cs_t0=kw["cs_t0"] + c // 256) if kw.get("cs_tn", 0) > 1 else dict(kw, colsum=None)
            tail = ((dy, adv(x, c), adv(g, c), N, K - c, M, ld_dy, ld_x, ldc, dt), tkw, t128(N, K - c), red)
        return head, tail

    def flush_wgrads(self, only_kind=None, ride=False, keep_riders=False, touching=None, budget=None, entries=None):
        kind_of = lambda e: 0 if e[3] <= 2048 else e[3]
        q = [e for e in self._wq if only_kind is None or kind_of(e) == only_kind]
        if entries is not None:
            ids = set(id(e) for e in entries)
            q = [e for e in self._wq if id(e) in ids]
        if touching is not None:
            ptr_of = lambda t: (t[0] if isinstance(t, tuple) else t).data_ptr()
            q = [e for e in q if touching in (ptr_of(e[0][0]), ptr_of(e[0][1]))]
        if ride and budget is not None:
            smalls = [e for e in q if self._pack_small(e)][:9]
            take, room = [], budget
            for e in smalls:
                t = self._k2_tiles(e)
                if t <= room:
                    take.append(e); room -= t
            nbig = 0
            for e in [e for e in q if not self._pack_small(e)]:
                t = self._k2_tiles(e)
                if t <= room and len(take) < 16:
                    take.append(e); room -= t; nbig += 1
                    continue
                cut = self._split_entry(e, room) if len(take) < 16 else None
                if cut is not None:
                    head, tail = cut
                    self._wq[[id(w) for w in self._wq].index(id(e))] = tail
                    self._wq.insert(0, head)
                    take.append(head); room -= self._k2_tiles(head)
                break
            if room > 0:
                for e in [e for e in q if self._pack_small(e)][9:]:
                    t = self._k2_tiles(e)
                    if len(take) >= 16:
                        break
                    if t <= room:
                        take.append(e); room -= t
            q = take
        elif ride:
            anchors = [e for e in q if not self._is_rider(e)]
            T = sum(self._k2_tiles(e) for e in anchors)
            room, slots, take = 256 * ((T + 255) // 256) - T, 16 - len(anchors), []
            for e in q:
                if self._is_rider(e) and slots > 0 and self._k2_tiles(e) <= room:
                    take.append(e); slots -= 1; room -= self._k2_tiles(e)
            q = anchors + take
        elif keep_riders:
            q = [e for e in q if not self._is_rider(e)]
        if not q:
            return
        chosen = set(id(e) for e in q)
        self._wq = [e for e in self._wq if id(e) not in chosen]
        parts = {}
        for e in q:
            parts.setdefault(kind_of(e), []).append(e)
        for red, part in parts.items():
            nk = (red + 63) // 64
            tiles = sum(e[2] for e in part)
            elig = [e for e in part if e[0][8] == e[0][4] and e[1].get("batch", 1) == 1 and not e[1].get("cs_tn")
                    and (e[1].get("flags", 0) & EPI_ACCUM)]
            etiles = sum(e[2] for e in elig)
            if self.split_wgrad and 2048 < red <= 16384 and len(elig) >= 2 and etiles < 200:
                self._wgrad_sliced(elig, red, etiles)
                taken = set(id(e) for e in elig)
                part = [e for e in part if id(e) not in taken]
                tiles -= etiles
            if not part:
                pass
            elif len(part) >= 2 and (red == 0 or tiles >= 200 or nk * 0.6 < len(part) * 35.0):
                for i in range(0, len(part), 16):
                    chunk = part[i:i + 16]
                    if len(chunk) == 1 and chunk[0][1].get("batch", 1) == 1 and not chunk[0][1].get("cs_tn"):
                        ops.gemm(*chunk[0][0], **self._pub(chunk[0][1]))
                    else:
                        ops.gemm_grouped([(e[0], self._pub(e[1])) for e in chunk])
            else:
                for args, kw, _, _ in part:
                    if kw.get("batch", 1) > 1 or kw.get("cs_tn"):
                        ops.gemm_grouped([(args, self._pub(kw))])
                    else:
                        ops.gemm(*args, **self._pub(kw))
            for e in part:
                self._csq.extend(e[1].get("_post", ()))
        if not self.use_side:
            self._frozen = set()
            for args, _, _, _ in self._wq:
                for t in (args[0], args[1]):
                    self._frozen.add((t[0] if isinstance(t, tuple) else t).data_ptr())
        if self._pending_reports and not self._reporting:
            self._reporting = True
            try:
                self._report_ready()
            finally:
                self._reporting = False

    @staticmethod
    def _pub(kw):
        return {k: v for k, v in kw.items() if not k.startswith("_")} if any(k.startswith("_") for k in kw) else kw

    @staticmethod
    def _targets(e):
        args, kw = e[0], e[1]
        if "_target" in kw:
            return list(kw["_target"])
        out = [args[2]]
        if kw.get("colsum") is not None:
            out.append(kw["colsum"])
        return out

    def _wgrad_sliced(self, part, red, tiles):
        S = max(2, min(8, 288 // tiles, 16 // len(part)))
        kchunk = ((red + S - 1) // S + 63) // 64 * 64
        S = (red + kchunk - 1) // kchunk
        slab = self._new(sum(S * e[0][3] * e[0][4] for e in part), dtype=torch.float32)
        nb = sum(S * e[0][3] for e in part if e[1].get("colsum") is not None)
        bslab = ops.zero_(torch.empty(max(nb, 1), device=self.dev, dtype=torch.float32))
        sub, jobs, so, bo = [], [], 0, 0
        adv = lambda t, n: (t[0], t[1] + n) if isinstance(t, tuple) else (t, n)
        for args, kw, _, _ in part:
            dy, x, g, N, K, M, ld_dy, ld_x, ldc, dt = args
            cs = kw.get("colsum")
            for s in range(S):
                k0 = s * kchunk
                k1 = min(red, k0 + kchunk)
                kw_s = dict(kw, flags=EPI_OUT_F32, colsum=None if cs is None else (bslab, bo + s * N))
                sub.append(((adv(dy, k0 * ld_dy), adv(x, k0 * ld_x), (slab, so + s * N * K), N, K, k1 - k0, ld_dy, ld_x, K, dt), kw_s))
            jobs.append(((slab, so), g, S, N * K))
            so += S * N * K
            if cs is not None:
                jobs.append(((bslab, bo), cs, S, N))
                bo += S * N
        for i in range(0, len(sub), 16):
            ops.gemm_grouped(sub[i:i + 16])
        ops.colsum_batched(jobs)

    def flush_colsums(self):
        q, self._csq = self._csq, []
        if q:
            ops.colsum_batched(q)

    def join_side(self):
        self.flush_wgrads()
        if self.side is not None:
            torch.cuda.current_stream(self.dev).wait_stream(self.side)
        self._frozen.clear()

    def abort_pass(self):
        self._wq, self._csq, self._gq = [], [], []
        self._lazy_finish()
        self._gq_out, self._frozen = set(), set()
        self._pending_reports, self._reporting = [], False
        self._pack_seen = {}
        self._in_lanes = False
        self.tape = Tape()
        self.last_tape = None

    def _writable(self, t):
        if t is not None and t.data_ptr() in self._frozen:
            if self.use_side:
                self.join_side()
            else:
                self.flush_wgrads(touching=t.data_ptr())

    def backward(self, d_inst, d_aux, d_sim_low=None, tape=None):
        tape = self.last_tape if tape is None else tape
        if tape is None or tape.done or len(tape) == 0:
            raise RuntimeError("Engine.backward: no pending training-mode forward to back-propagate (its tape was "
                               "already run, or forward ran with training=False)")
        self.attach_grads()
        tape.out_grads[:] = [None if d_inst is None else d_inst.contiguous(), None if d_aux is None else d_aux.contiguous(),
                             None if d_sim_low is None else d_sim_low.contiguous()]
        self._pack_seen = {}
        for fn in reversed(tape.fns):
            fn()
        self._pack_total = self._pack_seen
        tape.fns = []
        tape.done = True
        if tape is self.last_tape:
            self.last_tape = None
        self.tape = Tape()
        self.join_side()
        self.flush_colsums()
        self._lazy_finish()
        self._report_ready(final=True)
        if self.grad_ready_hook is not None:
            self.grad_ready_hook(0, self.names["backbone.blocks.0.norm1.weight"][0])
```

### pvpuformer_amd/ops.py

```python
import ctypes as C

import torch

from . import _lib
from ._lib import (BF16, F32, EPI_BIAS, EPI_PREACT, EPI_GELU, EPI_RELU, EPI_DGELU, EPI_DRELU, EPI_RESID, EPI_AFFINE,
                   EPI_ACCUM, EPI_OUT_F32, EPI_SAVE_DGELU, EPI_MULAUX, GemmDesc)

TORCH_DTYPE = {BF16: torch.bfloat16, F32: torch.float32}


def code_of(t):
    if isinstance(t, tuple):
        t = t[0]
    if t.dtype == torch.bfloat16:
        return BF16
    if t.dtype == torch.float32:
        return F32
    raise TypeError(f"unsupported dtype {t.dtype}")


_raw_stream = getattr(torch._C, "_cuda_getCurrentRawStream", None)
_cur_device = getattr(torch._C, "_cuda_getDevice", None)


# ... 68 lines not shown
        kw["workspace"] = None
        _fill_desc(d, *args, **kw)
    _lib.call("vpu_gemm_grouped", arr, n, _stream())


def gemm_last_kernel():
    return _lib.load().vpu_gemm_last_kernel().decode()


def attn_last_kernel():
    return _lib.load().vpu_attn_last_kernel().decode()


def attn_set_option(name, value):
    _lib.call("vpu_attn_set_option", name.encode(), int(value))


def gemm_set_option(name, value):
    _lib.call("vpu_gemm_set_option", name.encode(), int(value))


def gemm_get_option(name):
    import ctypes
    v = ctypes.c_int32(0)
    _lib.call("vpu_gemm_get_option", name.encode(), ctypes.byref(v))
    return int(v.value)


def layernorm_fwd(x, w, b, y, mean, rstd, rows, Cdim, eps):
    _lib.call("vpu_layernorm_fwd", ptr(x), ptr(w), ptr(b), ptr(y), ptr(mean), ptr(rstd), rows, Cdim, eps, code_of(x),
              _stream())


def layernorm_fwd_pe(x, w, b, y, mean, rstd, rows, Cdim, eps, pe, pe_rows, y2):
    _lib.call("vpu_layernorm_fwd_pe", ptr(x), ptr(w), ptr(b), ptr(y), ptr(mean), ptr(rstd), rows, Cdim, eps, ptr(pe),
              int(pe_rows), ptr(y2), code_of(x), _stream())


def layernorm_bwd_nblk(rows):
    return _lib.load().vpu_layernorm_bwd_nblk(rows)


def layernorm_bwd(dy, x, w, mean, rstd, dres, dx, part, rows, Cdim, dy2=None):
    if dy2 is None:
        _lib.call("vpu_layernorm_bwd", ptr(dy), ptr(x), ptr(w), ptr(mean), ptr(rstd), ptr(dres), ptr(dx), ptr(part), rows,
                  Cdim, code_of(x), _stream())
    else:
        _lib.call("vpu_layernorm_bwd2", ptr(dy), ptr(dy2), ptr(x), ptr(w), ptr(mean), ptr(rstd), ptr(dres), ptr(dx),
                  ptr(part), rows, Cdim, code_of(x), _stream())


def edt(mask_u8, zero_border=True):
    B, H, W = mask_u8.shape
    mask_u8 = mask_u8.contiguous()
    scratch = torch.empty(B, H, W, device=mask_u8.device, dtype=torch.int32)
    dist = torch.empty(B, H, W, device=mask_u8.device, dtype=torch.float32)
    _lib.call("vpu_edt", ptr(mask_u8), ptr(scratch), ptr(dist), B, H, W, int(zero_border), _stream())
    return dist


def chamfer5(mask_u8, zero_border=True):
    B, H, W = mask_u8.shape
    mask_u8 = mask_u8.contiguous()
    scratch = torch.empty(B, H + 2, W + 2, device=mask_u8.device, dtype=torch.int32)
    dist = torch.empty(B, H, W, device=mask_u8.device, dtype=torch.float32)
    _lib.call("vpu_chamfer5", ptr(mask_u8), ptr(scratch), ptr(dist), B, H, W, int(zero_border), _stream())
    return dist


def cc_roots(mask_u8):
    B, H, W = mask_u8.shape
    mask_u8 = mask_u8.contiguous()
    roots = torch.empty(B, H, W, device=mask_u8.device, dtype=torch.int32)
    _lib.call("vpu_cc_roots", ptr(mask_u8), ptr(roots), B, H, W, _stream())
    return roots


def cc_table(roots, kmax=4096):
    B, H, W = roots.shape
    slots = torch.empty(B, H, W, device=roots.device, dtype=torch.int32)
    table = torch.empty(kmax * 6 + 1, device=roots.device, dtype=torch.int32)
    _lib.call("vpu_cc_table", ptr(roots), ptr(slots), ptr(table), kmax, B, H, W, _stream())
    return table


def colsum_batched(jobs):
    for i in range(0, len(jobs), 64):
        chunk = jobs[i:i + 64]
        arr = (_lib.ColsumJob * len(chunk))()
        for j, job in zip(arr, chunk):
            inp, out, rows, Cdim = job[:4]
            j.inp, j.out, j.nrows, j.ncols = ptr(inp), ptr(out), rows, Cdim
            j.row_len, j.out_ld = (job[4], job[5]) if len(job) > 4 and job[4] and job[5] != job[4] else (0, 0)
        _lib.call("vpu_colsum_batched", arr, len(chunk), _stream())


def colsum_f32(inp, out, rows, Cdim, beta=0.0):
    _lib.call("vpu_colsum_f32", ptr(inp), ptr(out), rows, Cdim, beta, _stream())


def colsum(inp, ld, out, part, rows, Cdim, beta=0.0):
    _lib.call("vpu_colsum", ptr(inp), ld, ptr(out), ptr(part), rows, Cdim, beta, code_of(inp[0] if isinstance(inp, tuple) else inp),
              _stream())


def softmax_fwd(S, lds, P, ldp, rows, ncols):
    _lib.call("vpu_softmax_fwd", ptr(S), lds, ptr(P), ldp, rows, ncols, code_of(P), _stream())


def softmax_bwd(P, ldp, dP, lddp, dS, rows, ncols, scale):
    _lib.call("vpu_softmax_bwd", ptr(P), ldp, ptr(dP), lddp, ptr(dS), rows, ncols, scale, code_of(P), _stream())


def l2norm_fwd(x, y, inv, rows, Cdim):
    _lib.call("vpu_l2norm_fwd", ptr(x), ptr(y), ptr(inv), rows, Cdim, code_of(x), _stream())


def l2norm_bwd(dy, y, inv, dx, rows, Cdim):
    _lib.call("vpu_l2norm_bwd", ptr(dy), ptr(y), ptr(inv), ptr(dx), rows, Cdim, code_of(y), _stream())


def attn_fwd(q, k, v, out, lse, nb, H, n, hd, ld, ldo, scale):
    _lib.call("vpu_attn_fwd", ptr(q), ptr(k), ptr(v), ptr(out), ptr(lse), nb, H, n, hd, ld, ldo, scale, _stream())


def xattn_fwd(q, k, v, out, lse, nb, H, nq, nk, hd, ldq, ldk, ldo, scale):
    _lib.call("vpu_xattn_fwd", ptr(q), ptr(k), ptr(v), ptr(out), ptr(lse), nb, H, nq, nk, hd, ldq, ldk, ldo, scale,
              _stream())


def xattn_bwd(q, k, v, o, d_o, lse, delta, dq, dk, dv, nb, H, nq, nk, hd, ldq, ldk, ldo, ldgq, ldgk, scale):
    _lib.call("vpu_xattn_bwd", ptr(q), ptr(k), ptr(v), ptr(o), ptr(d_o), ptr(lse), ptr(delta), ptr(dq), ptr(dk),
              ptr(dv), nb, H, nq, nk, hd, ldq, ldk, ldo, ldgq, ldgk, scale, _stream())


def xattn_fwd_split(q, k, v, out, lse, nb, H, nq, nk, hd, ldq, ldk, ldo, scale, qdiv, kdiv):
    _lib.call("vpu_xattn_fwd_split", ptr(q), ptr(k), ptr(v), ptr(out), ptr(lse), nb, H, nq, nk, hd, ldq, ldk, ldo, scale,
              int(qdiv), int(kdiv), _stream())


def xattn_bwd_split(q, k, v, o, d_o, lse, delta, dq, dk, dv, nb, H, nq, nk, hd, ldq, ldk, ldo, ldgq, ldgk, scale, qdiv, kdiv):
    _lib.call("vpu_xattn_bwd_split", ptr(q), ptr(k), ptr(v), ptr(o), ptr(d_o), ptr(lse), ptr(delta), ptr(dq), ptr(dk),
              ptr(dv), nb, H, nq, nk, hd, ldq, ldk, ldo, ldgq, ldgk, scale, int(qdiv), int(kdiv), _stream())


def attn_combine(o_s, lse_s, out, lse, nb, H, nq, hd, S, ld_s, ldo):
    _lib.call("vpu_attn_combine", ptr(o_s), ptr(lse_s), ptr(out), ptr(lse), nb, H, nq, hd, S, ld_s, ldo, _stream())


def sum_groups(inp, out, G, S, n):
    _lib.call("vpu_sum_groups", ptr(inp), ptr(out), G, S, n, code_of(inp), _stream())


def attn_bwd(q, k, v, o, d_o, lse, delta, dq, dk, dv, nb, H, n, hd, ld, ldo, ldg, scale):
    _lib.call("vpu_attn_bwd", ptr(q), ptr(k), ptr(v), ptr(o), ptr(d_o), ptr(lse), ptr(delta), ptr(dq), ptr(dk),
              ptr(dv), nb, H, n, hd, ld, ldo, ldg, scale, _stream())


def add_bcast(a, b, out, n, period):
    _lib.call("vpu_add_bcast", ptr(a), ptr(b), ptr(out), n, period, code_of(a), _stream())


def add4(a, b, c, d, out, n):
    _lib.call("vpu_add4", ptr(a), ptr(b), ptr(c), ptr(d), ptr(out), n, code_of(a), _stream())


def fanout_add(src, dsts, accum, n):
    arr = (C.c_void_p * len(dsts))(*[ptr(t) for t in dsts])
    acc = (C.c_int32 * len(dsts))(*[int(bool(a)) for a in accum])
    _lib.call("vpu_fanout_add", ptr(src), arr, acc, len(dsts), n, code_of(src), _stream())


def cast2d(src, ld_src, dst, ld_dst, rows, cols, cols_pad=None):
    s = src[0] if isinstance(src, tuple) else src
    d = dst[0] if isinstance(dst, tuple) else dst
    _lib.call("vpu_cast2d", ptr(src), code_of(s), ld_src, ptr(dst), code_of(d), ld_dst, rows, cols,
              cols if cols_pad is None else cols_pad, _stream())


def cast2d_batched(jobs):
    arr = (_lib.CastJob * len(jobs))()
    for j, q in zip(arr, jobs):
        d = q["dst"][0] if isinstance(q["dst"], tuple) else q["dst"]
        j.src, j.src2, j.dst = ptr(q["src"]), ptr(q.get("src2")), ptr(q["dst"])
        j.ld_src, j.ld_dst, j.rows = q["ld_src"], q["ld_dst"], q["rows"]
        j.cols, j.cols_pad, j.dst_dtype = q["cols"], q.get("cols_pad", q["cols"]), code_of(d)
        j.perm_g, j.perm_wg = q.get("perm", (0, 0))
    _lib.call("vpu_cast2d_batched", arr, len(jobs), _stream())


def act_bwd(dy, ld_dy, aux, ld_aux, dz, ld_dz, rows, cols, kind, dtype):
    _lib.call("vpu_act_bwd", ptr(dy), ld_dy, ptr(aux), ld_aux, ptr(dz), ld_dz, rows, cols, kind, dtype, _stream())


def sigmoid_to_channel(logits, out, B, HW, channels, channel):
    _lib.call("vpu_sigmoid_to_channel", ptr(logits), ptr(out), B, HW, channels, channel, _stream())


def debug_spin(sink, wgs, cycles):
    _lib.call("vpu_debug_spin", ptr(sink), int(wgs), int(cycles), _stream())


_drop_state = {}


def _drop_key(device):
    key = torch.device(device)
    if key.type == "cuda" and key.index is None:
        key = torch.device("cuda", torch.cuda.current_device())
    return key


def _drop_entry(key, seed=None):
    if key not in _drop_state:
        sd = int(torch.initial_seed() if seed is None else seed) & (2 ** 63 - 1)
        _drop_state[key] = torch.tensor([0, sd], dtype=torch.int64, device=key)
    return _drop_state[key]


def dropout_mask(B, channels, keep, device, seed=None):
    key = _drop_key(device)
    state = _drop_entry(key, seed)
    out = torch.empty(B, channels, device=key, dtype=torch.float32)
    _lib.call("vpu_dropout_mask", ptr(out), B * channels, float(keep), 0, ptr(state), _stream())
    return out


def dropout_seed(device, seed):
    set_dropout_state(device, {"seed": int(seed) & (2 ** 63 - 1), "calls": 0})


def dropout_state(device):
    st = _drop_entry(_drop_key(device)).cpu()
    return {"seed": int(st[1]), "calls": int(st[0])}


def set_dropout_state(device, d):
    st = _drop_entry(_drop_key(device))
    st.copy_(torch.tensor([int(d["calls"]), int(d["seed"]) & (2 ** 63 - 1)], dtype=torch.int64))


def zero_(t):
    nbytes = t.numel() * t.element_size()
    assert t.is_contiguous() and nbytes % 4 == 0
    _lib.call("vpu_fill_f32", ptr(t), 0.0, nbytes // 4, _stream())
    return t


def zero_ranges_(t, ranges):
    assert t.dtype == torch.float32 and t.is_contiguous()
    for i in range(0, len(ranges), 160):
        chunk = ranges[i:i + 160]
        offs = (C.c_int64 * len(chunk))(*[int(o) for o, _ in chunk])
        lens = (C.c_int64 * len(chunk))(*[int(n) for _, n in chunk])
        _lib.call("vpu_fill_ranges_f32", ptr(t), offs, lens, len(chunk), 0.0, _stream())
    return t


def fill_f32(t, v, n=None):
    _lib.call("vpu_fill_f32", ptr(t), v, t.numel() if n is None else n, _stream())


def pue_encode(points, boxes, lut, out, out64, B, n, num_max, img, ld):
    _lib.call("vpu_pue_encode", ptr(points), ptr(boxes), ptr(lut), ptr(out), ptr(out64), B, n, num_max, img, ld,
              code_of(out), _stream())


def pue_scribble_rows(points, vec64, out, out64, B, n, num_max, img, ld):
    _lib.call("vpu_pue_scribble_rows", ptr(points), ptr(vec64), ptr(out), ptr(out64), B, n, num_max, img, ld, code_of(out),
              _stream())


def draw_polyline(curve_i32, disks, B, P, H, W):
    _lib.call("vpu_draw_polyline", ptr(curve_i32), ptr(disks), B, P, H, W, _stream())


def pue_encode_rows(points, kinds_i32, boxes, vec64, lut, out, out64, B, n, num_max, img, ld):
    _lib.call("vpu_pue_encode_rows", ptr(points), ptr(kinds_i32), ptr(boxes), ptr(vec64), ptr(lut), ptr(out), ptr(out64),
              B, n, num_max, img, ld, code_of(out), _stream())


def draw_prompt_rows(kinds_i32, boxes, curve_i32, counts_i32, disks, B, Pmax, n, H, W):
    _lib.call("vpu_draw_prompt_rows", ptr(kinds_i32), ptr(boxes), ptr(curve_i32), ptr(counts_i32), ptr(disks), B, Pmax, n,
              H, W, _stream())


def mask_bbox(prob, thr, pos_clicks=None):
    B, H, W = prob.shape
    out = torch.empty(B, 5, device=prob.device, dtype=torch.int32)
    n = 0 if pos_clicks is None else int(pos_clicks.shape[0])
    _lib.call("vpu_mask_bbox", ptr(prob), float(thr), ptr(pos_clicks) if n else None, n, ptr(out), B, H, W, _stream())
    return out


def error_masks(pred_u8, gt_u8, valid_u8):
    H, W = gt_u8.shape
    out = torch.empty(2, H, W, device=gt_u8.device, dtype=torch.uint8)
    _lib.call("vpu_error_masks", ptr(pred_u8), ptr(gt_u8), ptr(valid_u8), ptr(out), H, W, _stream())
    return out


def masked_argmax(dist, keep_u8):
    P, H, W = dist.shape
    out = torch.empty(P, device=dist.device, dtype=torch.int64)
    _lib.call("vpu_masked_argmax", ptr(dist), ptr(keep_u8), ptr(out), P, H, W, _stream())
    return out
# ... 290 lines not shown
```

Measured before the change: 1022.

## Fuse split cross-attention partial reduction into kernels via last-arriver counters

Result: no change. 1025, median of 6 (+0.4%).

```diff
diff --git a/include/vpu_hip.h b/include/vpu_hip.h
--- a/include/vpu_hip.h
+++ b/include/vpu_hip.h
@@ -109,6 +109,13 @@
 int vpu_attn_combine(const void* o_s, const float* lse_s, void* out, float* lse, int32_t nb, int32_t H, int32_t nq, int32_t hd,
                      int32_t S, int32_t ld_s, int32_t ldo, void* stream);
 int vpu_sum_groups(const void* in, void* out, int64_t G, int32_t S, int64_t n, int32_t dtype, void* stream);
+int vpu_xattn_fwd_fused(const void* q, const void* k, const void* v, void* out, float* lse, float* part, float* part_lse,
+                        int32_t* counters, int32_t nb, int32_t H, int32_t nq, int32_t nk, int32_t hd, int32_t ldq, int32_t ldk,
+                        int32_t ldo, float scale, int32_t S, void* stream);
+int vpu_xattn_bwd_fused(const void* q, const void* k, const void* v, const void* o, const void* d_o, const float* lse,
+                        float* delta, void* dq, void* dk, void* dv, float* part, int32_t* counters, int32_t nb, int32_t H,
+                        int32_t nq, int32_t nk, int32_t hd, int32_t ldq, int32_t ldk, int32_t ldo, int32_t ldgq, int32_t ldgk,
+                        float scale, int32_t S, int32_t long_q, void* stream);
 
 int vpu_add_bcast(const void* a, const void* b, void* out, int64_t n, int64_t period_b, int32_t dtype, void* stream);
 int vpu_add4(const void* a, const void* b, const void* c, const void* d, void* out, int64_t n, int32_t dtype,
diff --git a/pvpuformer_amd/_lib.py b/pvpuformer_amd/_lib.py
--- a/pvpuformer_amd/_lib.py
+++ b/pvpuformer_amd/_lib.py
@@ -97,6 +97,8 @@
     "vpu_xattn_bwd_split": [_P, _P, _P, _P, _P, _P, _P, _P, _P, _P, _I, _I, _I, _I, _I, _I, _I, _I, _I, _I, _F, _I, _I, _P],
     "vpu_attn_combine": [_P, _P, _P, _P, _I, _I, _I, _I, _I, _I, _I, _P],
     "vpu_sum_groups": [_P, _P, _L, _I, _L, _I, _P],
+    "vpu_xattn_fwd_fused": [_P, _P, _P, _P, _P, _P, _P, _P, _I, _I, _I, _I, _I, _I, _I, _I, _F, _I, _P],
+    "vpu_xattn_bwd_fused": [_P, _P, _P, _P, _P, _P, _P, _P, _P, _P, _P, _P, _I, _I, _I, _I, _I, _I, _I, _I, _I, _I, _F, _I, _I, _P],
     "vpu_add_bcast": [_P, _P, _P, _L, _L, _I, _P],
     "vpu_add4": [_P, _P, _P, _P, _P, _L, _I, _P],
     "vpu_cast2d": [_P, _I, _L, _P, _I, _L, _L, _I, _I, _P],
diff --git a/pvpuformer_amd/csrc/attention.hip b/pvpuformer_amd/csrc/attention.hip
--- a/pvpuformer_amd/csrc/attention.hip
+++ b/pvpuformer_amd/csrc/attention.hip
@@ -3,6 +3,7 @@
 #include <string.h>
 #include <atomic>
 #include "vpu_common.h"
+#include "last_arriver.h"
 #include "../../include/vpu_hip.h"
 
 namespace {
@@ -102,6 +103,8 @@
     float scale;
     int gx, nbh;
     int qdiv, kdiv;
+    float *part, *part2, *part_lse;
+    int* cnt;
 };
 
 template <int HD, int NS, int QT>
@@ -462,7 +465,7 @@
 
 constexpr float RESCALE_TH = 8.0f;
 
-template <int HD, int QT, int HC>
+template <int HD, int QT, int HC, bool FZ = false>
 #ifndef VPU_ATTN_FWD_OCC
 #define VPU_ATTN_FWD_OCC 4
 #endif
@@ -472,8 +475,14 @@
     __shared__ __attribute__((aligned(16))) char ldsK[2][CH * HD * 2];
     __shared__ __attribute__((aligned(16))) char ldsV[2][CH * HD * 2];
     const int tid = threadIdx.x, lane = tid & 63, wave = tid >> 6, g = lane >> 4, c = lane & 15;
-    int bh, xb;
-    wg_problem(a.gx, a.nbh, bh, xb);
+    int bh, xb, tile = 0;
+    if constexpr (FZ) {
+        int sp;
+        wg_problem(a.qdiv, a.nbh, tile, sp);
+        xb = tile % a.gx;
+        const int bh0 = tile / a.gx;
+        bh = ((bh0 / a.H) * a.qdiv + sp) * a.H + bh0 % a.H;
+    } else wg_problem(a.gx, a.nbh, bh, xb);
     const int bw = bh / a.H, h = bh % a.H, nq = a.nq, nk = a.nk, hd = a.hd;
     const int bwq = bw / max(a.qdiv, 1), bwk = bw / max(a.kdiv, 1);
     const int64_t rbq = (int64_t)bwq * nq, rbk = (int64_t)bwk * nk, rbqo = (int64_t)bw * nq, rbko = (int64_t)bw * nk;
@@ -603,7 +612,46 @@
         if (i < nch) { stage(i); scores(i); }
     }
     __syncthreads();
-    {
+    if constexpr (FZ) {
+        const int S = a.qdiv;
+        const __amdgpu_buffer_rsrc_t rsP = __builtin_amdgcn_make_buffer_rsrc(a.part, 0, 0x7FFFFFFF, 0x00020000);
+#pragma unroll
+        for (int u = 0; u < QT; ++u) {
+            const float l = accl[u][0], il = __builtin_amdgcn_rcpf(l);
+            const int qq = q0 + 16 * u + c;
+            if (qq < nq) {
+                if (g == 0) vpu_publish_store(a.part_lse + (int64_t)bh * nq + qq, (mref[u] + __builtin_amdgcn_logf(l)) * LN2);
+                const int off = (((bh * nq + qq) * hd) + 4 * g) * 4;
+#pragma unroll
+                for (int dt = 0; dt < DT; ++dt)
+                    if (dt * 16 < hd) vpu_publish_store16(rsP, off + dt * 64, acc[u][dt] * il);
+            }
+        }
+        if (!vpu_arrive_last(a.cnt + tile, S, reinterpret_cast<int*>(&ldsK[0][0]))) return;
+        const int cpr = hd / 8, qb = xb * (64 * QT), rows = min(64 * QT, nq - qb);
+        for (int idx = tid; idx < rows * cpr; idx += 256) {
+            const int qq = qb + idx / cpr, ck = idx % cpr;
+            float ls[8], m = -INFINITY;
+            for (int sp = 0; sp < S; ++sp) {
+                ls[sp] = a.part_lse[((int64_t)(bwq * S + sp) * a.H + h) * nq + qq];
+                m = fmaxf(m, ls[sp]);
+            }
+            float tot = 0.f, o8[8] = {0.f, 0.f, 0.f, 0.f, 0.f, 0.f, 0.f, 0.f};
+            for (int sp = 0; sp < S; ++sp) {
+                const float w = __expf(ls[sp] - m);
+                tot += w;
+                float v8[8];
+                load8(a.part + (((int64_t)(bwq * S + sp) * a.H + h) * nq + qq) * hd + ck * 8, v8);
+#pragma unroll
+                for (int j = 0; j < 8; ++j) o8[j] += w * v8[j];
+            }
+            const float inv = 1.f / tot;
+#pragma unroll
+            for (int j = 0; j < 8; ++j) o8[j] *= inv;
+            store8(a.out + ((int64_t)bwq * nq + qq) * a.ldo + h * hd + ck * 8, o8);
+            if (ck == 0) a.lse[(int64_t)bhq * nq + qq] = m + __logf(tot);
+        }
+    } else {
         typedef __bf16 bf16x4o_t __attribute__((ext_vector_type(4)));
         constexpr int RB = HD * 2, NCHK = HD / 8, SW = NCHK >= 8 ? 7 : NCHK - 1;
         char* const stg = (wave < 2 ? &ldsK[0][0] : &ldsV[0][0]) + (wave & 1) * (CH * HD * 2);
@@ -632,14 +680,20 @@
     }
 }
 
-template <int HD, int QT, int HC>
+template <int HD, int QT, int HC, bool FZ = false>
 __global__ __launch_bounds__(256) void attn_bwd_dq_lean_kernel(const AttnArgs a) {
     constexpr int KS = HC / 32, DT = HC / 16;
     using S = Stg<HD>;
     __shared__ __attribute__((aligned(16))) char ldsKr[2][CH * HD * 2], ldsKt[2][CH * HD * 2], ldsVr[2][CH * HD * 2];
     const int tid = threadIdx.x, lane = tid & 63, wave = tid >> 6, g = lane >> 4, c = lane & 15;
-    int bh, xb;
-    wg_problem(a.gx, a.nbh, bh, xb);
+    int bh, xb, tile = 0;
+    if constexpr (FZ) {
+        int sp;
+        wg_problem(a.qdiv, a.nbh, tile, sp);
+        xb = tile % a.gx;
+        const int bh0 = tile / a.gx;
+        bh = ((bh0 / a.H) * a.qdiv + sp) * a.H + bh0 % a.H;
+    } else wg_problem(a.gx, a.nbh, bh, xb);
     const int bw = bh / a.H, h = bh % a.H, nq = a.nq, nk = a.nk, hd = a.hd;
     const int bwq = bw / max(a.qdiv, 1), bwk = bw / max(a.kdiv, 1);
     const int64_t rbq = (int64_t)bwq * nq, rbk = (int64_t)bwk * nk, rbqo = (int64_t)bw * nq, rbko = (int64_t)bw * nk;
@@ -737,6 +791,35 @@
             for (int u = 0; u < QT; ++u) adq[u][dt] = __builtin_amdgcn_mfma_f32_16x16x32_bf16(dsf[u], ktf, adq[u][dt], 0, 0, 0);
         }
     }
+    if constexpr (FZ) {
+        const int S = a.qdiv;
+#pragma unroll
+        for (int u = 0; u < QT; ++u)
+#pragma unroll
+            for (int r = 0; r < 4; ++r) {
+                const int qq = q0 + 16 * u + 4 * g + r;
+                if (qq < nq) {
+                    float* pr = a.part + ((int64_t)bh * nq + qq) * hd + c;
+#pragma unroll
+                    for (int dt = 0; dt < DT; ++dt)
+                        if (dt * 16 < hd) vpu_publish_store(pr + dt * 16, adq[u][dt][r]);
+                }
+            }
+        if (!vpu_arrive_last(a.cnt + tile, S, reinterpret_cast<int*>(&ldsKr[0][0]))) return;
+        const int cpr = hd / 8, qb = xb * (64 * QT), rows = min(64 * QT, nq - qb);
+        for (int idx = tid; idx < rows * cpr; idx += 256) {
+            const int qq = qb + idx / cpr, ck = idx % cpr;
+            float o8[8] = {0.f, 0.f, 0.f, 0.f, 0.f, 0.f, 0.f, 0.f};
+            for (int sp = 0; sp < S; ++sp) {
+                float v8[8];
+                load8(a.part + (((int64_t)(bwq * S + sp) * a.H + h) * nq + qq) * hd + ck * 8, v8);
+#pragma unroll
+                for (int j = 0; j < 8; ++j) o8[j] += v8[j];
+            }
+            store8(a.dq + ((int64_t)bwq * nq + qq) * a.ldgq + h * hd + ck * 8, o8);
+        }
+        return;
+    }
 #pragma unroll
     for (int u = 0; u < QT; ++u)
 #pragma unroll
@@ -756,15 +839,21 @@
         }
 }
 
-template <int HD, int KT, int HC>
+template <int HD, int KT, int HC, bool FZ = false>
 __global__ __launch_bounds__(256, 3) void attn_bwd_dkdv_lean_kernel(const AttnArgs a) {
     constexpr int KS = HC / 32, DT = HC / 16;
     using S = Stg<HD>;
     __shared__ __attribute__((aligned(16))) char ldsQr[2][CH * HD * 2], ldsQt[2][CH * HD * 2];
     __shared__ __attribute__((aligned(16))) char ldsOr[2][CH * HD * 2], ldsOt[2][CH * HD * 2];
     const int tid = threadIdx.x, lane = tid & 63, wave = tid >> 6, g = lane >> 4, c = lane & 15;
-    int bh, xb;
-    wg_problem(a.gx, a.nbh, bh, xb);
+    int bh, xb, tile = 0;
+    if constexpr (FZ) {
+        int sp;
+        wg_problem(a.kdiv, a.nbh, tile, sp);
+        xb = tile % a.gx;
+        const int bh0 = tile / a.gx;
+        bh = ((bh0 / a.H) * a.kdiv + sp) * a.H + bh0 % a.H;
+    } else wg_problem(a.gx, a.nbh, bh, xb);
     const int bw = bh / a.H, h = bh % a.H, nq = a.nq, nk = a.nk, hd = a.hd;
     const int bwq = bw / max(a.qdiv, 1), bwk = bw / max(a.kdiv, 1);
     const int64_t rbq = (int64_t)bwq * nq, rbk = (int64_t)bwk * nk, rbqo = (int64_t)bw * nq, rbko = (int64_t)bw * nk;
@@ -851,6 +940,40 @@
                 adk[u][dt] = __builtin_amdgcn_mfma_f32_16x16x32_bf16(dsf[u], qtf, adk[u][dt], 0, 0, 0);
             }
         }
+    }
+    if constexpr (FZ) {
+        const int S = a.kdiv;
+#pragma unroll
+        for (int u = 0; u < KT; ++u)
+#pragma unroll
+            for (int r = 0; r < 4; ++r) {
+                const int kk = key0 + 16 * u + 4 * g + r;
+                if (kk < nk) {
+                    const int64_t o = ((int64_t)bh * nk + kk) * hd + c;
+#pragma unroll
+                    for (int dt = 0; dt < DT; ++dt)
+                        if (dt * 16 < hd) {
+                            vpu_publish_store(a.part + o + dt * 16, adk[u][dt][r]);
+                            vpu_publish_store(a.part2 + o + dt * 16, adv[u][dt][r]);
+                        }
+                }
+            }
+        if (!vpu_arrive_last(a.cnt + tile, S, reinterpret_cast<int*>(&ldsQr[0][0]))) return;
+        const int cpr = hd / 8, kb0 = xb * (64 * KT), rows = min(64 * KT, nk - kb0);
+        for (int idx = tid; idx < 2 * rows * cpr; idx += 256) {
+            const int which = idx / (rows * cpr), i2 = idx - which * rows * cpr;
+            const int kk = kb0 + i2 / cpr, ck = i2 % cpr;
+            const float* src = which ? a.part2 : a.part;
+            float o8[8] = {0.f, 0.f, 0.f, 0.f, 0.f, 0.f, 0.f, 0.f};
+            for (int sp = 0; sp < S; ++sp) {
+                float v8[8];
+                load8(src + (((int64_t)(bwk * S + sp) * a.H + h) * nk + kk) * hd + ck * 8, v8);
+#pragma unroll
+                for (int j = 0; j < 8; ++j) o8[j] += v8[j];
+            }
+            store8((which ? a.dv : a.dk) + ((int64_t)bwk * nk + kk) * a.ldgk + h * hd + ck * 8, o8);
+        }
+        return;
     }
 #pragma unroll
     for (int u = 0; u < KT; ++u)
@@ -1812,6 +1935,37 @@
     return vpu_check_launch("vpu_attn_combine");
 }
 
+static void launch_dq_lean(const AttnArgs& a, dim3 gq, bool q2, hipStream_t s) {
+    const int hd = a.hd;
+    switch (hd_image(hd) * 4 + (q2 ? 2 : 1)) {
+        case 128 * 4 + 2:
+            if (hd <= 96) attn_bwd_dq_lean_kernel<128, 2, 96><<<gq, 256, 0, s>>>(a);
+            else attn_bwd_dq_lean_kernel<128, 2, 128><<<gq, 256, 0, s>>>(a);
+            break;
+        case 32 * 4 + 2: attn_bwd_dq_lean_kernel<32, 2, 32><<<gq, 256, 0, s>>>(a); break;
+        case 32 * 4 + 1: attn_bwd_dq_lean_kernel<32, 1, 32><<<gq, 256, 0, s>>>(a); break;
+        case 64 * 4 + 2: attn_bwd_dq_lean_kernel<64, 2, 64><<<gq, 256, 0, s>>>(a); break;
+        case 64 * 4 + 1: attn_bwd_dq_lean_kernel<64, 1, 64><<<gq, 256, 0, s>>>(a); break;
+        default:
+            if (hd <= 96) attn_bwd_dq_lean_kernel<128, 1, 96><<<gq, 256, 0, s>>>(a);
+            else attn_bwd_dq_lean_kernel<128, 1, 128><<<gq, 256, 0, s>>>(a);
+            break;
+    }
+}
+static void launch_dkdv_lean(const AttnArgs& ak, dim3 gk, bool k2, hipStream_t s) {
+    const int hd = ak.hd;
+    switch (hd_image(hd) * 4 + (k2 ? 2 : 1)) {
+        case 32 * 4 + 2: attn_bwd_dkdv_lean_kernel<32, 2, 32><<<gk, 256, 0, s>>>(ak); break;
+        case 32 * 4 + 1: attn_bwd_dkdv_lean_kernel<32, 1, 32><<<gk, 256, 0, s>>>(ak); break;
+        case 64 * 4 + 2: attn_bwd_dkdv_lean_kernel<64, 2, 64><<<gk, 256, 0, s>>>(ak); break;
+        case 64 * 4 + 1: attn_bwd_dkdv_lean_kernel<64, 1, 64><<<gk, 256, 0, s>>>(ak); break;
+        default:
+            if (hd <= 96) attn_bwd_dkdv_lean_kernel<128, 1, 96><<<gk, 256, 0, s>>>(ak);
+            else attn_bwd_dkdv_lean_kernel<128, 1, 128><<<gk, 256, 0, s>>>(ak);
+            break;
+    }
+}
+
 static int xattn_bwd_impl(const void* q, const void* k, const void* v, const void* o, const void* d_o,
                           const float* lse, float* delta, void* dq, void* dk, void* dv, int32_t nb, int32_t H,
                           int32_t nq, int32_t nk, int32_t hd, int32_t ldq, int32_t ldk, int32_t ldo, int32_t ldgq,
@@ -1889,30 +2043,8 @@
         if (xcd_map_enabled() && gk.x > 1) { ak.gx = gk.x; ak.nbh = nb * H; gk = dim3(gk.x * gk.y); }
         snprintf(g_last_attn, sizeof(g_last_attn), "attn_bwd_dq_lean_kernel<%d, %d, %d> attn_bwd_dkdv_lean_kernel<%d, %d, %d>",
                  hd_image(hd), q2 ? 2 : 1, hd_computed(hd), hd_image(hd), k2 ? 2 : 1, hd_computed(hd));
-        switch (hd_image(hd) * 4 + (q2 ? 2 : 1)) {
-            case 128 * 4 + 2:
-                if (hd <= 96) attn_bwd_dq_lean_kernel<128, 2, 96><<<gq, 256, 0, s>>>(a);
-                else attn_bwd_dq_lean_kernel<128, 2, 128><<<gq, 256, 0, s>>>(a);
-                break;
-            case 32 * 4 + 2: attn_bwd_dq_lean_kernel<32, 2, 32><<<gq, 256, 0, s>>>(a); break;
-            case 32 * 4 + 1: attn_bwd_dq_lean_kernel<32, 1, 32><<<gq, 256, 0, s>>>(a); break;
-            case 64 * 4 + 2: attn_bwd_dq_lean_kernel<64, 2, 64><<<gq, 256, 0, s>>>(a); break;
-            case 64 * 4 + 1: attn_bwd_dq_lean_kernel<64, 1, 64><<<gq, 256, 0, s>>>(a); break;
-            default:
-                if (hd <= 96) attn_bwd_dq_lean_kernel<128, 1, 96><<<gq, 256, 0, s>>>(a);
-                else attn_bwd_dq_lean_kernel<128, 1, 128><<<gq, 256, 0, s>>>(a);
-                break;
-        }
-        switch (hd_image(hd) * 4 + (k2 ? 2 : 1)) {
-            case 32 * 4 + 2: attn_bwd_dkdv_lean_kernel<32, 2, 32><<<gk, 256, 0, s>>>(ak); break;
-            case 32 * 4 + 1: attn_bwd_dkdv_lean_kernel<32, 1, 32><<<gk, 256, 0, s>>>(ak); break;
-            case 64 * 4 + 2: attn_bwd_dkdv_lean_kernel<64, 2, 64><<<gk, 256, 0, s>>>(ak); break;
-            case 64 * 4 + 1: attn_bwd_dkdv_lean_kernel<64, 1, 64><<<gk, 256, 0, s>>>(ak); break;
-            default:
-                if (hd <= 96) attn_bwd_dkdv_lean_kernel<128, 1, 96><<<gk, 256, 0, s>>>(ak);
-                else attn_bwd_dkdv_lean_kernel<128, 1, 128><<<gk, 256, 0, s>>>(ak);
-                break;
-        }
+        launch_dq_lean(a, gq, q2, s);
+        launch_dkdv_lean(ak, gk, k2, s);
         return vpu_check_launch("vpu_xattn_bwd");
     }
     dim3 gk((nk + 63) / 64, nb * H), gq((nq + 63) / 64, nb * H);
@@ -1947,6 +2079,91 @@
     return xattn_bwd_impl(q, k, v, o, d_o, lse, delta, dq, dk, dv, nb, H, nq, nk, hd, ldq, ldk, ldo, ldgq, ldgk, scale, qdiv, kdiv, stream);
 }
 
+#define VPU_FZ_LAUNCH(KERN_, grid_, a_)                                                   \
+    switch (hd_image(hd)) {                                                               \
+        case 32: KERN_<32, 1, 32, true><<<grid_, 256, 0, s>>>(a_); break;                 \
+        case 64: KERN_<64, 1, 64, true><<<grid_, 256, 0, s>>>(a_); break;                 \
+        default:                                                                          \
+            if (hd <= 96) KERN_<128, 1, 96, true><<<grid_, 256, 0, s>>>(a_);              \
+            else KERN_<128, 1, 128, true><<<grid_, 256, 0, s>>>(a_);                      \
+            break;                                                                        \
+    }
+
+extern "C" int vpu_xattn_fwd_fused(const void* q, const void* k, const void* v, void* out, float* lse, float* part,
+                                   float* part_lse, int32_t* counters, int32_t nb, int32_t H, int32_t nq, int32_t nk, int32_t hd,
+                                   int32_t ldq, int32_t ldk, int32_t ldo, float scale, int32_t S, void* stream) {
+    vpu_clear_stale_error();
+    if (!lean_enabled() || S < 2 || S > 8 || nb <= 0 || H <= 0 || nq <= 0 || nq > 64 || nk <= 0 || nk % S || hd <= 0 || hd > 128 ||
+        hd % 16 || ldq % 8 || ldk % 8 || ldo % 8 || !ok16(q) || !ok16(k) || !ok16(v) || !ok16(out) || !ok16(part) || !lse || !part ||
+        !part_lse || !counters || (int64_t)(nk / S) * ldk >= (1 << 29) || (int64_t)nb * S * H * nq * hd * 4 >= 0x7FFFFFF0LL) {
+        vpu_set_error("xattn_fwd_fused: the lean kernels, 2 <= S <= 8, nk % S == 0, nq <= 64, head dim a multiple of 16 up to 128, "
+                      "16-byte aligned slices and scratch, row strides % 8 == 0");
+        return VPU_ERR_ARG;
+    }
+    AttnArgs a{};
+    a.q = (const bf16_t*)q; a.k = (const bf16_t*)k; a.v = (const bf16_t*)v; a.out = (bf16_t*)out; a.lse = lse;
+    a.nq = nq; a.nk = nk / S; a.H = H; a.hd = hd; a.ldq = ldq; a.ldk = ldk; a.ldo = ldo; a.scale = scale;
+    a.qdiv = S; a.kdiv = 1; a.gx = 1; a.nbh = nb * H;
+    a.part = part; a.part_lse = part_lse; a.cnt = counters;
+    hipStream_t s = reinterpret_cast<hipStream_t>(stream);
+    const dim3 grid((unsigned)(nb * H * S));
+    snprintf(g_last_attn, sizeof(g_last_attn), "attn_fwd_lean_kernel<%d, 1, %d, true>", hd_image(hd), hd_computed(hd));
+    VPU_FZ_LAUNCH(attn_fwd_lean_kernel, grid, a)
+    return vpu_check_launch("vpu_xattn_fwd_fused");
+}
+
+extern "C" int vpu_xattn_bwd_fused(const void* q, const void* k, const void* v, const void* o, const void* d_o, const float* lse,
+                                   float* delta, void* dq, void* dk, void* dv, float* part, int32_t* counters, int32_t nb,
+                                   int32_t H, int32_t nq, int32_t nk, int32_t hd, int32_t ldq, int32_t ldk, int32_t ldo,
+                                   int32_t ldgq, int32_t ldgk, float scale, int32_t S, int32_t long_q, void* stream) {
+    vpu_clear_stale_error();
+    bool ok = lean_enabled() && S >= 2 && S <= 8 && nb > 0 && H > 0 && nq > 0 && nk > 0 && hd > 0 && hd <= 128 && hd % 16 == 0 &&
+              ldq % 8 == 0 && ldk % 8 == 0 && ldo % 8 == 0 && ldgq % 8 == 0 && ldgk % 8 == 0 && ok16(q) && ok16(k) && ok16(v) &&
+              ok16(o) && ok16(d_o) && ok16(dq) && ok16(dk) && ok16(dv) && ok16(part) && lse && delta && part && counters &&
+              (int64_t)nb * S * H * (long_q ? nk : nq) * hd * 4 < 0x7FFFFFF0LL;
+    if (ok && long_q) ok = nq % (4 * S) == 0 && nk <= 64;
+    else if (ok) ok = nk % S == 0 && nq <= 64 && nq % 4 == 0;
+    const int nqe = long_q ? nq / S : nq, nke = long_q ? nk : nk / S;
+    ok = ok && (int64_t)nke * ldk < (1 << 29) && (int64_t)nqe * ldq < (1 << 29) && (int64_t)nqe * ldo < (1 << 29);
+    if (!ok) {
+        vpu_set_error("xattn_bwd_fused: the lean kernels, 2 <= S <= 8, the long side a multiple of S (of 4 S: queries), the short "
+                      "side <= 64 rows (queries % 4 == 0), head dim a multiple of 16 up to 128, 16-byte aligned slices and scratch, "
+                      "row strides % 8 == 0");
+        return VPU_ERR_ARG;
+    }
+    AttnArgs a{};
+    a.q = (const bf16_t*)q; a.k = (const bf16_t*)k; a.v = (const bf16_t*)v; a.o = (const bf16_t*)o;
+    a.d_o = (const bf16_t*)d_o; a.lse = const_cast<float*>(lse); a.delta = delta;
+    a.dq = (bf16_t*)dq; a.dk = (bf16_t*)dk; a.dv = (bf16_t*)dv;
+    a.nq = nqe; a.nk = nke; a.H = H; a.hd = hd; a.ldq = ldq; a.ldk = ldk; a.ldo = ldo; a.ldgq = ldgq; a.ldgk = ldgk;
+    a.scale = scale; a.qdiv = long_q ? 1 : S; a.kdiv = long_q ? S : 1;
+    hipStream_t s = reinterpret_cast<hipStream_t>(stream);
+    const int nbe = nb * S;
+    AttnArgs af = a;
+    af.gx = 1; af.nbh = nb * H; af.cnt = counters; af.part = part;
+    af.part2 = part + (int64_t)nbe * H * nk * hd;
+    const dim3 gf((unsigned)(nb * H * S));
+    if (long_q) {
+        const bool q2 = nqe > 64 && (hd_image(hd) <= 64 || wide_two());
+        dim3 gq(q2 ? (nqe + 127) / 128 : (nqe + 63) / 64, nbe * H);
+        if (xcd_map_enabled() && gq.x > 1) { a.gx = gq.x; a.nbh = nbe * H; gq = dim3(gq.x * gq.y); }
+        snprintf(g_last_attn, sizeof(g_last_attn), "attn_bwd_dq_lean_kernel<%d, %d, %d> attn_bwd_dkdv_lean_kernel<%d, 1, %d, true>",
+                 hd_image(hd), q2 ? 2 : 1, hd_computed(hd), hd_image(hd), hd_computed(hd));
+        launch_dq_lean(a, gq, q2, s);
+        VPU_FZ_LAUNCH(attn_bwd_dkdv_lean_kernel, gf, af)
+    } else {
+        const bool k2 = nke > 64 && hd_image(hd) <= 64;
+        dim3 gk(k2 ? (nke + 127) / 128 : (nke + 63) / 64, nbe * H);
+        if (xcd_map_enabled() && gk.x > 1) { a.gx = gk.x; a.nbh = nbe * H; gk = dim3(gk.x * gk.y); }
+        snprintf(g_last_attn, sizeof(g_last_attn), "attn_bwd_dq_lean_kernel<%d, 1, %d, true> attn_bwd_dkdv_lean_kernel<%d, %d, %d>",
+                 hd_image(hd), hd_computed(hd), hd_image(hd), k2 ? 2 : 1, hd_computed(hd));
+        VPU_FZ_LAUNCH(attn_bwd_dq_lean_kernel, gf, af)
+        launch_dkdv_lean(a, gk, k2, s);
+    }
+    return vpu_check_launch("vpu_xattn_bwd_fused");
+}
+#undef VPU_FZ_LAUNCH
+
 extern "C" int vpu_attn_fwd(const void* q, const void* k, const void* v, void* out, float* lse, int32_t nb, int32_t H,
                             int32_t n, int32_t hd, int32_t ld, int32_t ldo, float scale, void* stream) {
     return vpu_xattn_fwd(q, k, v, out, lse, nb, H, n, n, hd, ld, ld, ldo, scale, stream);
diff --git a/pvpuformer_amd/csrc/gemm.hip b/pvpuformer_amd/csrc/gemm.hip
--- a/pvpuformer_amd/csrc/gemm.hip
+++ b/pvpuformer_amd/csrc/gemm.hip
@@ -2123,8 +2123,11 @@
     const int left = (v - r) & ~7;
     return left >= 64 ? left : v;
 }
+#ifndef VPU_GEMM_INLAUNCH_DEFAULT
+#define VPU_GEMM_INLAUNCH_DEFAULT 0
+#endif
 inline int inlaunch_env0() {
-    static const int v = [] { const char* e = vpu_lab_getenv("VPU_GEMM_INLAUNCH"); return e ? atoi(e) : 0; }();
+    static const int v = [] { const char* e = vpu_lab_getenv("VPU_GEMM_INLAUNCH"); return e ? atoi(e) : VPU_GEMM_INLAUNCH_DEFAULT; }();
     return v;
 }
 constexpr int64_t CNT_BYTES = 256 << 10;
diff --git a/pvpuformer_amd/csrc/last_arriver.h b/pvpuformer_amd/csrc/last_arriver.h
--- /dev/null
+++ b/pvpuformer_amd/csrc/last_arriver.h
@@ -0,0 +1,29 @@
+#pragma once
+#include <hip/hip_runtime.h>
+
+typedef float vpu_f32x4_t __attribute__((ext_vector_type(4)));
+typedef unsigned vpu_u32x4_t __attribute__((ext_vector_type(4)));
+
+__device__ __forceinline__ void vpu_publish_store(float* p, float v) {
+    __hip_atomic_store(p, v, __ATOMIC_RELAXED, __HIP_MEMORY_SCOPE_AGENT);
+}
+__device__ __forceinline__ void vpu_publish_store16(__amdgpu_buffer_rsrc_t r, int off, vpu_f32x4_t v) {
+    __builtin_amdgcn_raw_buffer_store_b128(__builtin_bit_cast(vpu_u32x4_t, v), r, off, 0, 16);
+}
+
+__device__ __forceinline__ bool vpu_arrive_last(int* __restrict__ counter, int parts, int* lds_flag) {
+    asm volatile("s_waitcnt vmcnt(0)" ::: "memory");
+    __syncthreads();
+    if (threadIdx.x == 0) {
+        const int seen = __hip_atomic_fetch_add(counter, 1, __ATOMIC_RELAXED, __HIP_MEMORY_SCOPE_AGENT);
+        const bool last = seen == parts - 1;
+        if (last) {
+            __hip_atomic_store(counter, 0, __ATOMIC_RELAXED, __HIP_MEMORY_SCOPE_AGENT);
+            __builtin_amdgcn_fence(__ATOMIC_ACQUIRE, "agent");
+            asm volatile("s_waitcnt vmcnt(0)" ::: "memory");
+        }
+        *lds_flag = last ? 1 : 0;
+    }
+    __syncthreads();
+    return *lds_flag != 0;
+}
diff --git a/pvpuformer_amd/engine.py b/pvpuformer_amd/engine.py
--- a/pvpuformer_amd/engine.py
+++ b/pvpuformer_amd/engine.py
@@ -10,6 +10,10 @@
 from . import ops
 from ._lib import (BF16, F32, EPI_BIAS, EPI_PREACT, EPI_GELU, EPI_RELU, EPI_DGELU, EPI_DRELU, EPI_RESID, EPI_AFFINE,
                    EPI_ACCUM, EPI_OUT_F32, EPI_SAVE_DGELU, EPI_MULAUX)
+
+
+XATTN_SPLIT_DEFAULT = 4
+XATTN_SPLIT_FWD = False
 
 
 class Tape:
@@ -133,7 +137,9 @@
         self.wgrad_tn = 256 if self.k4_wgrad else 128
         self.unify_wgrad = True
         self.lazy_zero = True
-        self.xattn_split = max(1, int(os.environ.get("VPU_XATTN_SPLIT", "1")))
+        self.xattn_split = max(1, int(os.environ.get("VPU_XATTN_SPLIT", str(XATTN_SPLIT_DEFAULT))))
+        self._xcnt, self._xcnt_at = None, 0
+        self.xattn_split_fwd = XATTN_SPLIT_FWD
         self.neck_lanes = int(os.environ.get("VPU_NECK_LANES", "0"))
         self._tok_stream = None
         self._in_lanes = False
@@ -631,16 +637,17 @@
 
     def cross_attention(self, Qp, Kp, Vp, O, nb, H, nq, nk, hd, ld, scale):
         S = self.xattn_split
-        long_q = S > 1 and nq >= 4 * nk and nq % (4 * S) == 0 and nq // S >= 64
-        long_k = S > 1 and not long_q and nk >= 4 * nq and nk % S == 0 and nk // S >= 64 and nq % 4 == 0
+        long_q = 1 < S <= 8 and nq >= 4 * nk and nq % (4 * S) == 0 and nq // S >= 64 and nk <= 64
+        long_k = 1 < S <= 8 and not long_q and nk >= 4 * nq and nk % S == 0 and nk // S >= 64 and nq % 4 == 0 and nq <= 64
         if long_q:
             lse = self._new(nb * S * H, nq // S, dtype=torch.float32)
             ops.xattn_fwd_split(Qp.t, Kp.t, Vp.t, O.t, lse, nb * S, H, nq // S, nk, hd, ld, ld, ld, scale, 1, S)
-        elif long_k:
+        elif long_k and self.xattn_split_fwd:
             lse = self._new(nb * H, nq, dtype=torch.float32)
-            o_s, lse_s = self._new(nb * S * nq, ld), self._new(nb * S * H, nq, dtype=torch.float32)
-            ops.xattn_fwd_split(Qp.t, Kp.t, Vp.t, o_s, lse_s, nb * S, H, nq, nk // S, hd, ld, ld, ld, scale, S, 1)
-            ops.attn_combine(o_s, lse_s, O.t, lse, nb, H, nq, hd, S, ld, ld)
+            part = self._new(nb * S * H, nq, hd, dtype=torch.float32)
+            part_lse = self._new(nb * S * H, nq, dtype=torch.float32)
+            ops.xattn_fwd_fused(Qp.t, Kp.t, Vp.t, O.t, lse, part, part_lse, self._xattn_counters(nb * H), nb, H, nq, nk, hd,
+                                ld, ld, ld, scale, S)
         else:
             lse = self._new(nb * H, nq, dtype=torch.float32)
             ops.xattn_fwd(Qp.t, Kp.t, Vp.t, O.t, lse, nb, H, nq, nk, hd, ld, ld, ld, scale)
@@ -653,22 +660,28 @@
                     var.g = torch.empty_like(var.t)
                 if long_q:
                     delta = self._new(nb * S * H, nq // S, dtype=torch.float32)
-                    dkp, dvp = self._new(nb * S * nk, ld), self._new(nb * S * nk, ld)
-                    ops.xattn_bwd_split(Qp.t, Kp.t, Vp.t, O.t, O.g, lse, delta, Qp.g, dkp, dvp, nb * S, H, nq // S, nk, hd, ld, ld,
-                                        ld, ld, ld, scale, 1, S)
-                    ops.sum_groups(dkp, Kp.g, nb, S, nk * ld)
-                    ops.sum_groups(dvp, Vp.g, nb, S, nk * ld)
+                    part = self._new(2, nb * S * H, nk, hd, dtype=torch.float32)
+                    ops.xattn_bwd_fused(Qp.t, Kp.t, Vp.t, O.t, O.g, lse, delta, Qp.g, Kp.g, Vp.g, part, self._xattn_counters(nb * H),
+                                        nb, H, nq, nk, hd, ld, ld, ld, ld, ld, scale, S, True)
                 elif long_k:
                     delta = self._new(nb * H, nq, dtype=torch.float32)
-                    dqp = self._new(nb * S * nq, ld)
-                    ops.xattn_bwd_split(Qp.t, Kp.t, Vp.t, O.t, O.g, lse, delta, dqp, Kp.g, Vp.g, nb * S, H, nq, nk // S, hd, ld, ld,
-                                        ld, ld, ld, scale, S, 1)
-                    ops.sum_groups(dqp, Qp.g, nb, S, nq * ld)
+                    part = self._new(nb * S * H, nq, hd, dtype=torch.float32)
+                    ops.xattn_bwd_fused(Qp.t, Kp.t, Vp.t, O.t, O.g, lse, delta, Qp.g, Kp.g, Vp.g, part, self._xattn_counters(nb * H),
+                                        nb, H, nq, nk, hd, ld, ld, ld, ld, ld, scale, S, False)
                 else:
                     delta = self._new(nb * H, nq, dtype=torch.float32)
                     ops.xattn_bwd(Qp.t, Kp.t, Vp.t, O.t, O.g, lse, delta, Qp.g, Kp.g, Vp.g, nb, H, nq, nk, hd, ld, ld, ld,
                                   ld, ld, scale)
             self.tape.append(bwd)
+
+    def _xattn_counters(self, n):
+        if self._xcnt is None:
+            self._xcnt = torch.zeros(1 << 16, device=self.dev, dtype=torch.int32)
+        if self._xcnt_at + n > self._xcnt.numel():
+            self._xcnt_at = 0
+        at = self._xcnt_at
+        self._xcnt_at = at + (n + 31) // 32 * 32
+        return self._xcnt[at:at + n]
 
     def add_pe(self, x, pe, n, period, pe_var=None):
         y = Var(torch.empty_like(x.t))
@@ -1489,6 +1502,8 @@
 
     def abort_pass(self):
         self._wq, self._csq, self._gq = [], [], []
+        if self._xcnt is not None:
+            self._xcnt.zero_()
         self._lazy_finish()
         self._gq_out, self._frozen = set(), set()
         self._pending_reports, self._reporting = [], False
diff --git a/pvpuformer_amd/ops.py b/pvpuformer_amd/ops.py
--- a/pvpuformer_amd/ops.py
+++ b/pvpuformer_amd/ops.py
@@ -244,6 +244,17 @@
     _lib.call("vpu_sum_groups", ptr(inp), ptr(out), G, S, n, code_of(inp), _stream())
 
 
+def xattn_fwd_fused(q, k, v, out, lse, part, part_lse, counters, nb, H, nq, nk, hd, ldq, ldk, ldo, scale, S):
+    _lib.call("vpu_xattn_fwd_fused", ptr(q), ptr(k), ptr(v), ptr(out), ptr(lse), ptr(part), ptr(part_lse), ptr(counters), nb, H,
+              nq, nk, hd, ldq, ldk, ldo, scale, int(S), _stream())
+
+
+def xattn_bwd_fused(q, k, v, o, d_o, lse, delta, dq, dk, dv, part, counters, nb, H, nq, nk, hd, ldq, ldk, ldo, ldgq, ldgk, scale,
+                    S, long_q):
+    _lib.call("vpu_xattn_bwd_fused", ptr(q), ptr(k), ptr(v), ptr(o), ptr(d_o), ptr(lse), ptr(delta), ptr(dq), ptr(dk), ptr(dv),
+              ptr(part), ptr(counters), nb, H, nq, nk, hd, ldq, ldk, ldo, ldgq, ldgk, scale, int(S), 1 if long_q else 0, _stream())
+
+
 def attn_bwd(q, k, v, o, d_o, lse, delta, dq, dk, dv, nb, H, n, hd, ld, ldo, ldg, scale):
     _lib.call("vpu_attn_bwd", ptr(q), ptr(k), ptr(v), ptr(o), ptr(d_o), ptr(lse), ptr(delta), ptr(dq), ptr(dk),
               ptr(dv), nb, H, n, hd, ld, ldo, ldg, scale, _stream())
```
